# joesound212985/Deepfake-Detection-using-CLIP-Based-SigLIP-2-Vision-Transformers

Hardware: AMD Instinct MI355X
Metric: images/sec (train fwd+bwd) SigLIP-2-so400m@384 bf16 (higher is better)
Workload: dtype bf16; 1 GPU; so400m-patch14-384 encoder+pool-head train fwd+bwd, 384x384, per-GPU batch 128, seeded random weights; global_batch=128, parallelism=dp1

## Files before the change

### deepfake-detection-using-clip-based-siglip-2-vision-transformers_amd/csrc/attention.hip

```cpp
#include <stdlib.h>

#include "common.hip.h"
#include "kernels.h"

namespace sgl {

hipError_t attn_f32_fwd(const float*, const float*, const float*, float*, float*, int, int, int, int, int, int, hipStream_t);
hipError_t attn_f32_bwd(const float*, const float*, const float*, const float*, const float*, const float*, float*,
                        float*, int, int, int, int, int, int, hipStream_t);
hipError_t attn_ref_fwd(const float*, const float*, const float*, float*, float*, int, int, int, int, int, int, hipStream_t);
hipError_t attn_ref_bwd(const float*, const float*, const float*, const float*, const float*, const float*, float*,
                        float*, int, int, int, int, int, int, hipStream_t);

template <int DP>
struct AttnCfg {
  static constexpr int KS = DP / 16;
  static constexpr int DT = (DP + 31) / 32;
  static constexpr int CPR = DP / 8;
  static constexpr int RSTR = DP * 2 + 16;
  static constexpr int TSTR = 192;
  static constexpr int DSTR = 208;
};

__device__ __forceinline__ u32x4 a_ldg(__amdgpu_buffer_rsrc_t r, uint32_t off) {
// ... 336 lines not shown
      dP = MFMA32(da[ks], vfr[ks], dP);
    }
    if constexpr (C::KS == 5) {
      __builtin_amdgcn_sched_group_barrier(0x100, 4, 0);
#pragma unroll
      for (int i = 0; i < 6; ++i) {
        __builtin_amdgcn_sched_group_barrier(0x008, 1, 0);
        __builtin_amdgcn_sched_group_barrier(0x100, 1, 0);
      }
      __builtin_amdgcn_sched_group_barrier(0x008, 4, 0);
    }
    __builtin_amdgcn_sched_barrier(0);
    constexpr int NF = 2 * 2 * C::DT;
    lo_x8<T> fr[NF];
    auto frag = [&](int i) {
      const int which = i & 1, kk = (i >> 1) & 1, dt = i >> 2;
      return lds_trfrag<T>(which ? qimg : dimg, C::DSTR, kk, dt * 32, lane);
    };
    constexpr int PRE = NF < 2 ? NF : 2;
#pragma unroll
    for (int i = 0; i < PRE; ++i) fr[i] = frag(i);
    __builtin_amdgcn_sched_barrier(0);
#pragma unroll
    for (int g4 = 0; g4 < 4; ++g4) {
      const f32x4 A0 = *reinterpret_cast<const f32x4*>(ld + 2 * (8 * g4 + 4 * hh));
      const f32x4 A1 = *reinterpret_cast<const f32x4*>(ld + 2 * (8 * g4 + 4 * hh) + 4);
      const float L4[4] = {A0[0], A0[2], A1[0], A1[2]};
      const float D4[4] = {A0[1], A0[3], A1[1], A1[3]};
#pragma unroll
      for (int r3 = 0; r3 < 4; ++r3) {
        const int r = 4 * g4 + r3;
        const float p = fast_exp2(fmaf(S[r], c, L4[r3]));
        S[r] = p;
        dP[r] = p * fmaf(dP[r], scale, D4[r3]);
      }
    }
    lo_x8<T> pb[2], dsb[2];
    pb[0] = pack8<T>(S, 0);
    pb[1] = pack8<T>(S, 8);
    dsb[0] = pack8<T>(dP, 0);
    dsb[1] = pack8<T>(dP, 8);
    __builtin_amdgcn_sched_barrier(0);
#pragma unroll
    for (int i = 0; i < NF; ++i) {
      if (i + PRE < NF) fr[i + PRE] = frag(i + PRE);
      const int which = i & 1, kk = (i >> 1) & 1, dt = i >> 2;
      if (which) dk[dt] = MFMA32(fr[i], dsb[kk], dk[dt]);
      else dv[dt] = MFMA32(fr[i], pb[kk], dv[dt]);
      if (i % 3 == 1) issue1(i / 3, st_next);
      __builtin_amdgcn_sched_barrier(0);
    }
#pragma unroll
    for (int j = (NF + 1) / 3; j < 4; ++j) issue1(j, st_next);
  }
  asm volatile("s_waitcnt vmcnt(0)" ::: "memory");
  const int key = key0 + li;
  if (key < N) {
    T* krow = dqkv + ((size_t)b * N + key) * (3 * (size_t)D) + D + hd * dh;
    T* vrow = krow + D;
#pragma unroll
    for (int dt = 0; dt < C::DT; ++dt)
#pragma unroll
      for (int g4 = 0; g4 < 4; ++g4) {
        const int d = dt * 32 + 8 * g4 + 4 * hh;
        if (d < dh) {
          lo_x4<T> a, g;
#pragma unroll
          for (int r = 0; r < 4; ++r) {
            a[r] = (T)dk[dt][4 * g4 + r];
            g[r] = (T)dv[dt][4 * g4 + r];
          }
          *reinterpret_cast<lo_x4<T>*>(krow + d) = a;
          *reinterpret_cast<lo_x4<T>*>(vrow + d) = g;
        }
      }
  }
}

template <typename T, int DP, bool TOK>
__global__ __launch_bounds__(256, 2) void attn_bwd_q_kernel(const T* __restrict__ Q, const T* __restrict__ K,
                                                            const T* __restrict__ V, const T* __restrict__ O,
                                                            const T* __restrict__ dO, const float* __restrict__ lse,
                                                            float* __restrict__ aux, T* __restrict__ dqkv,
                                                            int B, int H, int N, int dh, int ld, float c, float scale) {
  using C = AttnCfg<DP>;
  constexpr int KT = 32;
  constexpr int SCK = C::DSTR / 16, SCV = C::RSTR / 16;
  constexpr int NIK = (KT * SCK + 63) / 64, NIV = (KT * SCV + 63) / 64;
  constexpr int KIMG = NIK * 1024, VIMG = NIV * 1024, STAGE = KIMG + VIMG;
  constexpr int NSLOT = NIK + NIV;
  static_assert(NSLOT <= 16, "at most four DMA slots per wave");
  constexpr float LOG2E = 1.4426950408889634f;
  extern __shared__ __attribute__((aligned(16))) char smem[];
  const int t = threadIdx.x, lane = t & 63;
  const int w = __builtin_amdgcn_readfirstlane(t >> 6);
  int bh, xb;
  if (!head_block((N + 127) / 128, B * H, bh, xb)) return;
  const int b = bh / H, hd = bh - b * H;
  const int D = H * dh;
  const int q0 = xb * 128 + w * 32;
  HeadSrc src = head_src(TOK ? ld : 0, b, hd, H, N, dh, DP);
  if constexpr (!TOK) {
    src.rowbytes = (uint32_t)DP * 2u;
    src.nc = (uint32_t)DP / 8u;
  }
  const __amdgpu_buffer_rsrc_t rq = make_rsrc(Q + src.base, src.bytes);
  const T* dOb = dO + (size_t)b * N * D + hd * dh;
  const __amdgpu_buffer_rsrc_t rdo = make_rsrc(dOb, (uint32_t)(((size_t)(N - 1) * D + dh) * 2));
  const u32x4 dk_ = att_desc(K + src.base, src.bytes);
  const u32x4 dv_ = att_desc(V + src.base, src.bytes);
  const uint32_t lds0 = (uint32_t)(size_t)((SGL_LDS char*)smem);

  const int li = lane & 31, hh = lane >> 5;
  const int q = q0 + li;
  lo_x8<T> qf[C::KS], dof[C::KS];
#pragma unroll
  for (int ks = 0; ks < C::KS; ++ks) {
    const int col = 16 * ks + 8 * hh;
    qf[ks] = as_x8<T>(a_ldg(rq, (q < N && (uint32_t)(col >> 3) < src.nc) ? (uint32_t)q * src.rowbytes + (uint32_t)col * 2u
                                                                           : SGL_OOB));
    dof[ks] = as_x8<T>(a_ldg(rdo, (q < N && col < dh) ? (uint32_t)(((size_t)q * D + col) * 2) : SGL_OOB));
  }
  float dl = 0.f;
  {
    const __amdgpu_buffer_rsrc_t ro = make_rsrc(O + (size_t)b * N * D + hd * dh, (uint32_t)(((size_t)(N - 1) * D + dh) * 2));
#pragma unroll
    for (int ks = 0; ks < C::KS; ++ks) {
      const int col = 16 * ks + 8 * hh;
      const lo_x8<T> of = as_x8<T>(a_ldg(ro, (q < N && col < dh) ? (uint32_t)(((size_t)q * D + col) * 2) : SGL_OOB));
#pragma unroll
      for (int j = 0; j < 8; ++j) dl = fmaf((float)of[j], (float)dof[ks][j], dl);
    }
    dl += __shfl_xor(dl, 32, 64);
  }
  const float Lq = (q < N) ? -lse[(size_t)bh * N + q] * LOG2E : -INFINITY;
  const float Dq = (q < N) ? -dl * scale : 0.f;
  if (q < N && hh == 0) *reinterpret_cast<float2*>(aux + 2 * ((size_t)bh * N + q)) = make_float2(Lq, Dq);

  uint32_t voff[4];
  u32x4 dsc[4];
  uint32_t ldst[4];
#pragma unroll
  for (int j = 0; j < 4; ++j) {
    const int sl = w + 4 * j;
    if (sl < NIK) {
      voff[j] = att_chunk_off(sl * 64 + lane, KT, SCK, (int)src.nc, src.rowbytes);
      dsc[j] = dk_;
      ldst[j] = (uint32_t)sl * 1024u;
    } else {
      voff[j] = att_chunk_off((sl - NIK) * 64 + lane, KT, SCV, (int)src.nc, src.rowbytes);
      dsc[j] = dv_;
      ldst[j] = (uint32_t)(KIMG + (sl - NIK) * 1024);
    }
  }
  auto issue1 = [&](int j, int stage) {
    if (w + 4 * j < NSLOT) att_dma16(dsc[j], lds0 + (uint32_t)(stage * STAGE) + ldst[j], voff[j]);
    voff[j] += (uint32_t)KT * src.rowbytes;
  };

  f32x16 dq[C::DT];
#pragma unroll
  for (int dt = 0; dt < C::DT; ++dt)
#pragma unroll
    for (int r = 0; r < 16; ++r) dq[dt][r] = 0.f;

  const int ntiles = (N + KT - 1) / KT;
#pragma unroll
// ... 5 lines not shown
#pragma unroll
  for (int j = 0; j < 4; ++j) issue1(j, 1);
  int st = 0;
  for (int kt = 0; kt < ntiles; ++kt) {
    const int nw = (NSLOT - w + 3) / 4;
    if (nw >= 4) SGL_ATT_WAIT_BARRIER(4);
    else if (nw == 3) SGL_ATT_WAIT_BARRIER(3);
    else if (nw == 2) SGL_ATT_WAIT_BARRIER(2);
    else SGL_ATT_WAIT_BARRIER(1);
    const int st_next = (st == 0) ? 2 : st - 1;
    const char* kimg = smem + st * STAGE;
    const char* vimg = kimg + KIMG;
    st = (st == 2) ? 0 : st + 1;
    f32x16 S, dP;
#pragma unroll
    for (int r = 0; r < 16; ++r) { S[r] = 0.f; dP[r] = 0.f; }
    lo_x8<T> ka[C::KS], va[C::KS];
#pragma unroll
    for (int ks = 0; ks < C::KS; ++ks) {
      ka[ks] = lds_row8<T>(kimg + li * C::DSTR + (16 * ks + 8 * hh) * 2);
      va[ks] = lds_row8<T>(vimg + li * C::RSTR + (16 * ks + 8 * hh) * 2);
    }
#pragma unroll
    for (int ks = 0; ks < C::KS; ++ks) {
      S = MFMA32(ka[ks], qf[ks], S);
      dP = MFMA32(va[ks], dof[ks], dP);
    }
    if constexpr (C::KS == 5) {
      __builtin_amdgcn_sched_group_barrier(0x100, 6, 0);
#pragma unroll
      for (int i = 0; i < 4; ++i) {
        __builtin_amdgcn_sched_group_barrier(0x008, 1, 0);
        __builtin_amdgcn_sched_group_barrier(0x100, 1, 0);
      }
      __builtin_amdgcn_sched_group_barrier(0x008, 6, 0);
    }
    __builtin_amdgcn_sched_barrier(0);
    lo_x8<T> kt_frag[C::DT][2];
#pragma unroll
    for (int dt = 0; dt < C::DT; ++dt)
#pragma unroll
      for (int kk = 0; kk < 2; ++kk) kt_frag[dt][kk] = lds_trfrag<T>(kimg, C::DSTR, kk, dt * 32, lane);
    __builtin_amdgcn_sched_barrier(0);
#pragma unroll
    for (int r = 0; r < 16; ++r) {
      const float p = fast_exp2(fmaf(S[r], c, Lq));
      dP[r] = p * fmaf(dP[r], scale, Dq);
    }
    if (kt == ntiles - 1) {
#pragma unroll
      for (int r = 0; r < 16; ++r) {
        const int key = kt * KT + (r & 3) + 8 * (r >> 2) + 4 * hh;
        if (key >= N) dP[r] = 0.f;
      }
    }
    lo_x8<T> dsb[2];
    dsb[0] = pack8<T>(dP, 0);
    dsb[1] = pack8<T>(dP, 8);
#pragma unroll
    for (int i = 0; i < 2 * C::DT; ++i) {
      dq[i >> 1] = MFMA32(kt_frag[i >> 1][i & 1], dsb[i & 1], dq[i >> 1]);
      if (i < 4) issue1(i, st_next);
      __builtin_amdgcn_sched_barrier(0);
    }
#pragma unroll
    for (int j = 2 * C::DT; j < 4; ++j) issue1(j, st_next);
  }
  asm volatile("s_waitcnt vmcnt(0)" ::: "memory");
  if (q < N) {
    T* qrow = dqkv + ((size_t)b * N + q) * (3 * (size_t)D) + hd * dh;
#pragma unroll
    for (int dt = 0; dt < C::DT; ++dt)
#pragma unroll
      for (int g4 = 0; g4 < 4; ++g4) {
        const int d = dt * 32 + 8 * g4 + 4 * hh;
        if (d < dh) {
          lo_x4<T> a;
#pragma unroll
          for (int r = 0; r < 4; ++r) a[r] = (T)dq[dt][4 * g4 + r];
          *reinterpret_cast<lo_x4<T>*>(qrow + d) = a;
        }
      }
  }
}

template <typename T, int DP>
static hipError_t fwd_launch(const T* q, const T* k, const T* v, T* out, float* lse, int B, int H, int N,
                             int dh, int ld, hipStream_t s) {
  using C = AttnCfg<DP>;
  constexpr int smem = 2 * (64 * C::RSTR + 64 * C::TSTR);
  const float scale = 1.0f / sqrtf((float)dh);
  if (ld > 0)
    hipLaunchKernelGGL((attn_fwd_kernel<T, DP, true>), head_grid((N + 127) / 128, B * H), dim3(256), smem, s, q, k, v, out, lse,
                       B, H, N, dh, ld, scale * 1.4426950408889634f, scale);
  else
    hipLaunchKernelGGL((attn_fwd_kernel<T, DP, false>), head_grid((N + 127) / 128, B * H), dim3(256), smem, s, q, k, v, out,
                       lse, B, H, N, dh, 0, scale * 1.4426950408889634f, scale);
  return hipGetLastError();
}

template <typename T, int DP>
static hipError_t bwd_launch(const T* q, const T* k, const T* v, const T* out, const T* dout,
                             const float* lse, T* dqkv, float* delta, int B, int H, int N, int dh, int ld,
                             hipStream_t s) {
  using C = AttnCfg<DP>;
  const float scale = 1.0f / sqrtf((float)dh);
  const float c = scale * 1.4426950408889634f;
  constexpr int smem_kv = 3 * (2 * ((32 * (C::DSTR / 16) + 63) / 64) * 1024 + 32 * 8);
  constexpr int smem_q = 3 * (((32 * (C::DSTR / 16) + 63) / 64) + ((32 * (C::RSTR / 16) + 63) / 64)) * 1024;
  const dim3 grid = head_grid((N + 127) / 128, B * H), block(256);
  if (ld > 0)
    hipLaunchKernelGGL((attn_bwd_q_kernel<T, DP, true>), grid, block, smem_q, s, q, k, v, out, dout, lse, delta, dqkv, B, H, N,
                       dh, ld, c, scale);
  else
    hipLaunchKernelGGL((attn_bwd_q_kernel<T, DP, false>), grid, block, smem_q, s, q, k, v, out, dout, lse, delta, dqkv, B, H, N,
                       dh, 0, c, scale);
  hipError_t e = hipGetLastError();
  if (e != hipSuccess) return e;
  if (ld > 0)
    hipLaunchKernelGGL((attn_bwd_kv_kernel<T, DP, true>), grid, block, smem_kv, s, q, k, v, dout, delta, dqkv, B, H, N, dh, ld, c,
                       scale);
  else
    hipLaunchKernelGGL((attn_bwd_kv_kernel<T, DP, false>), grid, block, smem_kv, s, q, k, v, dout, delta, dqkv, B, H, N, dh, 0,
                       c, scale);
  return hipGetLastError();
}

static bool attn_shape_ok(int N, int dh, int DP, int H, int ld) {
  if (dh % 8 || DP != ((dh + 15) / 16) * 16) return false;
  if (DP != 16 && DP != 32 && DP != 48 && DP != 64 && DP != 80 && DP != 96) return false;
  if (ld < 0 || (ld > 0 && (ld % 8 || ld < H * dh))) return false;
  if ((size_t)N * (ld > 0 ? ld : DP) * 2 >= (1ull << 31)) return false;
  if ((size_t)N * H * dh * 2 >= (1ull << 31)) return false;
  return true;
}

hipError_t attn_fwd(const void* q, const void* k, const void* v, int dtype, void* out, float* lse, int B, int H, int N,
                    int dh, int DP, int ld, hipStream_t s) {
  if (B * H == 0 || N == 0) return hipSuccess;
  if (dtype == DT_F32)
    return attn_ref_fwd((const float*)q, (const float*)k, (const float*)v, (float*)out, lse, B, H, N, dh, DP, ld, s);
  if (dtype == DT_F32_MFMA)
    return attn_f32_fwd((const float*)q, (const float*)k, (const float*)v, (float*)out, lse, B, H, N, dh, DP, ld, s);
  if (!attn_shape_ok(N, dh, DP, H, ld)) return hipErrorInvalidValue;
  if ((((uintptr_t)q) | ((uintptr_t)k) | ((uintptr_t)v)) & 15) return hipErrorInvalidValue;
#define SGL_F(T, DPV) \
  case DPV: return fwd_launch<T, DPV>((const T*)q, (const T*)k, (const T*)v, (T*)out, lse, B, H, N, dh, ld, s);
  if (dtype == DT_F16) {
    switch (DP) {
      SGL_F(f16, 16) SGL_F(f16, 32) SGL_F(f16, 48) SGL_F(f16, 64) SGL_F(f16, 80) SGL_F(f16, 96)
    }
    return hipErrorInvalidValue;
  }
  switch (DP) {
    SGL_F(bf16, 16) SGL_F(bf16, 32) SGL_F(bf16, 48) SGL_F(bf16, 64) SGL_F(bf16, 80) SGL_F(bf16, 96)
  }
#undef SGL_F
  return hipErrorInvalidValue;
}

hipError_t attn_bwd(const void* q, const void* k, const void* v, const void* out, const void* dout, const float* lse,
                    int dtype, void* dqkv, float* delta, float* , int B, int H, int N, int dh, int DP,
                    int ld, hipStream_t s) {
  if (B * H == 0 || N == 0) return hipSuccess;
  if (dtype == DT_F32)
    return attn_ref_bwd((const float*)q, (const float*)k, (const float*)v, (const float*)out, (const float*)dout, lse,
                        (float*)dqkv, delta, B, H, N, dh, DP, ld, s);
  if (dtype == DT_F32_MFMA)
    return attn_f32_bwd((const float*)q, (const float*)k, (const float*)v, (const float*)out, (const float*)dout, lse,
                        (float*)dqkv, delta, B, H, N, dh, DP, ld, s);
  if (!attn_shape_ok(N, dh, DP, H, ld)) return hipErrorInvalidValue;
  if ((((uintptr_t)q) | ((uintptr_t)k) | ((uintptr_t)v)) & 15) return hipErrorInvalidValue;
#define SGL_B(T, DPV)                                                                                  \
  case DPV:                                                                                            \
    return bwd_launch<T, DPV>((const T*)q, (const T*)k, (const T*)v, (const T*)out, (const T*)dout, lse, \
                              (T*)dqkv, delta, B, H, N, dh, ld, s);
  if (dtype == DT_F16) {
    switch (DP) {
      SGL_B(f16, 16) SGL_B(f16, 32) SGL_B(f16, 48) SGL_B(f16, 64) SGL_B(f16, 80) SGL_B(f16, 96)
    }
    return hipErrorInvalidValue;
  }
  switch (DP) {
    SGL_B(bf16, 16) SGL_B(bf16, 32) SGL_B(bf16, 48) SGL_B(bf16, 64) SGL_B(bf16, 80) SGL_B(bf16, 96)
  }
#undef SGL_B
  return hipErrorInvalidValue;
}

}
```

### deepfake-detection-using-clip-based-siglip-2-vision-transformers_amd/csrc/elementwise.hip

```cpp
#include "common.hip.h"
#include "shadow_tile.hip.h"
#include "kernels.h"

namespace sgl {

template <typename T>
__global__ __launch_bounds__(256) void im2col_kernel(const float* __restrict__ pix, int channels_last,
                                                     T* __restrict__ out, int B, int H, int W, int P, int gh, int gw,
                                                     int Kp) {
  const size_t total = (size_t)B * gh * gw * Kp;
  const int K = 3 * P * P;
  for (size_t idx = (size_t)blockIdx.x * 256 + threadIdx.x; idx < total; idx += (size_t)gridDim.x * 256) {
    const int k = (int)(idx % Kp);
    const size_t m = idx / Kp;
    float v = 0.f;
    if (k < K) {
      const int gx = (int)(m % gw);
      const int gy = (int)((m / gw) % gh);
      const int b = (int)(m / ((size_t)gw * gh));
      const int c = k / (P * P);
      const int r = k - c * P * P;
      const int ky = r / P, kx = r - ky * P;
      const int yy = gy * P + ky, xx = gx * P + kx;
      const size_t src = channels_last ? (((size_t)b * H + yy) * W + xx) * 3 + c
// ... 215 lines not shown
}
void cast_job_add_vec(CastJob& job, const float* src, int n, float* dst, int np) {
  job.vsrc[job.nvec] = src; job.vdst[job.nvec] = dst; job.vn[job.nvec] = n; job.vnp[job.nvec] = np;
  ++job.nvec;
}
hipError_t cast_job_run(const CastJob& job, int dst_dtype, hipStream_t s) {
  if (job.ntiles == 0 && job.nvec == 0) return hipSuccess;
  const dim3 grid((unsigned)(job.ntiles + (job.nvec ? 1 : 0)));
  if (dst_dtype == DT_BF16)
    hipLaunchKernelGGL(cast_job_kernel<bf16>, grid, dim3(256), 0, s, job);
  else if (dst_dtype == DT_F16)
    hipLaunchKernelGGL(cast_job_kernel<f16>, grid, dim3(256), 0, s, job);
  else
    hipLaunchKernelGGL(cast_job_kernel<float>, grid, dim3(256), 0, s, job);
  return hipGetLastError();
}

int colsum_chunks(int M) {
  int c = (M + 511) / 512;
  return c < 1 ? 1 : (c > 256 ? 256 : c);
}

template <typename T>
__global__ __launch_bounds__(256) void colsum_kernel(const T* __restrict__ in, int ld, int M, int N, int rows_per,
                                                     float* __restrict__ partial) {
  __shared__ float red[8][257];
  const int cg = threadIdx.x & 31, rl = threadIdx.x >> 5;
  const int col0 = blockIdx.x * 256 + cg * 8;
  const int r_begin = blockIdx.y * rows_per;
  const int r_end = (r_begin + rows_per < M) ? r_begin + rows_per : M;
  float acc[8] = {0, 0, 0, 0, 0, 0, 0, 0};
  if (col0 < N) {
    for (int r = r_begin + rl; r < r_end; r += 8) {
      float v[8];
      Vec<T, 8>::ld(in + (size_t)r * ld + col0, v);
#pragma unroll
      for (int j = 0; j < 8; ++j) acc[j] += v[j];
    }
  }
#pragma unroll
  for (int j = 0; j < 8; ++j) red[rl][cg * 8 + j] = acc[j];
  __syncthreads();
  const int c = threadIdx.x;
  if (blockIdx.x * 256 + c < N) {
    float s = 0.f;
#pragma unroll
    for (int r = 0; r < 8; ++r) s += red[r][c];
    partial[(size_t)blockIdx.y * N + blockIdx.x * 256 + c] = s;
  }
}

hipError_t colsum(const void* in, int dtype, int ld, int M, int N, int n_out, float* partial, float* out,
                  int accumulate, hipStream_t s) {
  if (N % 8 || ld % 8) return hipErrorInvalidValue;
  if (N == 0) return hipSuccess;
  const int chunks = colsum_chunks(M);
  const int rows_per = (M + chunks - 1) / chunks;
  dim3 grid((N + 255) / 256, chunks), block(256);
  if (dtype == DT_BF16)
    hipLaunchKernelGGL(colsum_kernel<bf16>, grid, block, 0, s, (const bf16*)in, ld, M, N, rows_per, partial);
  else if (dtype == DT_F16)
    hipLaunchKernelGGL(colsum_kernel<f16>, grid, block, 0, s, (const f16*)in, ld, M, N, rows_per, partial);
  else
    hipLaunchKernelGGL(colsum_kernel<float>, grid, block, 0, s, (const float*)in, ld, M, N, rows_per, partial);
  hipError_t e = hipGetLastError();
  if (e != hipSuccess) return e;
  return reduce_partials(partial, chunks, N, out, n_out < N ? n_out : N, accumulate, s);
}

__global__ __launch_bounds__(256) void batch_sum_kernel(const float* __restrict__ in, int B, size_t n,
                                                        float* __restrict__ out, int accumulate) {
  const size_t j = (size_t)blockIdx.x * 256 + threadIdx.x;
  if (j >= n) return;
  float s = 0.f;
  for (int b = 0; b < B; ++b) s += in[(size_t)b * n + j];
  out[j] = accumulate ? out[j] + s : s;
}
hipError_t batch_sum(const float* in, int B, size_t n, float* out, int accumulate, hipStream_t s) {
  if (n == 0) return hipSuccess;
  hipLaunchKernelGGL(batch_sum_kernel, dim3((unsigned)((n + 255) / 256)), dim3(256), 0, s, in, B, n, out, accumulate);
  return hipGetLastError();
}

constexpr int VECMAT_CHUNKS = 16;
__global__ __launch_bounds__(256) void vecmat_f32_kernel(const float* __restrict__ v, const float* __restrict__ W, int rows,
                                                         int cols, float* __restrict__ partial) {
  __shared__ float part[4][64];
  const int jj = threadIdx.x & 63, rg = threadIdx.x >> 6;
  const int j = blockIdx.x * 64 + jj;
  const int per = (rows + VECMAT_CHUNKS - 1) / VECMAT_CHUNKS;
  const int r0 = blockIdx.y * per, r1 = (r0 + per < rows) ? r0 + per : rows;
  float s = 0.f;
  if (j < cols)
    for (int i = r0 + rg; i < r1; i += 4) s = fmaf(v[i], W[(size_t)i * cols + j], s);
  part[rg][jj] = s;
  __syncthreads();
  if (rg == 0 && j < cols) partial[(size_t)blockIdx.y * cols + j] = (part[0][jj] + part[1][jj]) + (part[2][jj] + part[3][jj]);
}
hipError_t vecmat_f32(const float* v, const float* W, int rows, int cols, float* scratch, float* out, int accumulate,
                      hipStream_t s) {
  if (rows <= 0 || cols <= 0) return hipSuccess;
  hipLaunchKernelGGL(vecmat_f32_kernel, dim3((unsigned)((cols + 63) / 64), VECMAT_CHUNKS), dim3(256), 0, s, v, W, rows, cols,
                     scratch);
  hipError_t e = hipGetLastError();
  if (e != hipSuccess) return e;
  return reduce_partials(scratch, VECMAT_CHUNKS, cols, out, cols, accumulate, s);
}

__device__ __forceinline__ void cubic_coeffs(float t, float* w) {
  const float A = -0.75f;
  float x = t + 1.0f;
  w[0] = ((A * x - 5.0f * A) * x + 8.0f * A) * x - 4.0f * A;
  x = t;
  w[1] = ((A + 2.0f) * x - (A + 3.0f)) * x * x + 1.0f;
  x = 1.0f - t;
  w[2] = ((A + 2.0f) * x - (A + 3.0f)) * x * x + 1.0f;
  x = 2.0f - t;
  w[3] = ((A * x - 5.0f * A) * x + 8.0f * A) * x - 4.0f * A;
}
__device__ __forceinline__ void cubic_taps(int o, int n_in, int n_out, int* idx, float* w) {
  const float scale = (float)n_in / (float)n_out;
  const float src = scale * ((float)o + 0.5f) - 0.5f;
  const float fl = floorf(src);
  cubic_coeffs(src - fl, w);
  const int i0 = (int)fl;
#pragma unroll
  for (int k = 0; k < 4; ++k) {
    int i = i0 - 1 + k;
    idx[k] = i < 0 ? 0 : (i > n_in - 1 ? n_in - 1 : i);
  }
}

__global__ __launch_bounds__(256) void pos_resize_kernel(const float* __restrict__ table, int g0,
                                                         float* __restrict__ out, int gh, int gw, int D) {
  const size_t total = (size_t)gh * gw * D;
  const size_t idx = (size_t)blockIdx.x * 256 + threadIdx.x;
  if (idx >= total) return;
  const int d = (int)(idx % D);
  const int o = (int)(idx / D);
  const int oy = o / gw, ox = o - oy * gw;
  int iy[4], ix[4];
  float wy[4], wx[4];
  cubic_taps(oy, g0, gh, iy, wy);
  cubic_taps(ox, g0, gw, ix, wx);
  float acc = 0.f;
#pragma unroll
  for (int a = 0; a < 4; ++a) {
    float rowv = 0.f;
#pragma unroll
    for (int b = 0; b < 4; ++b) rowv += wx[b] * table[((size_t)iy[a] * g0 + ix[b]) * D + d];
    acc += wy[a] * rowv;
  }
  out[idx] = acc;
}
hipError_t pos_resize(const float* table, int g0, float* out, int gh, int gw, int D, hipStream_t s) {
  const size_t total = (size_t)gh * gw * D;
  if (total == 0) return hipSuccess;
  hipLaunchKernelGGL(pos_resize_kernel, dim3((unsigned)((total + 255) / 256)), dim3(256), 0, s, table, g0, out, gh, gw,
                     D);
  return hipGetLastError();
}

__device__ __forceinline__ void tap_range(int i, int g0, int gout, int& lo, int& hi) {
  const float inv = (float)gout / (float)g0;
  lo = (int)floorf(((float)i - 3.0f + 0.5f) * inv - 0.5f) - 1;
  hi = (int)ceilf(((float)i + 3.0f + 0.5f) * inv - 0.5f) + 1;
  if (i == 0) lo = 0;
  if (i == g0 - 1) hi = gout - 1;
  if (lo < 0) lo = 0;
  if (hi > gout - 1) hi = gout - 1;
}
__global__ __launch_bounds__(256) void pos_resize_bwd_kernel(const float* __restrict__ dout, int gh, int gw,
                                                             float* __restrict__ dtable, int g0, int D) {
  const size_t total = (size_t)g0 * g0 * D;
  const size_t idx = (size_t)blockIdx.x * 256 + threadIdx.x;
  if (idx >= total) return;
  const int d = (int)(idx % D);
  const int e = (int)(idx / D);
  const int ty = e / g0, tx = e - ty * g0;
  int ylo, yhi, xlo, xhi;
  tap_range(ty, g0, gh, ylo, yhi);
  tap_range(tx, g0, gw, xlo, xhi);
  float acc = 0.f;
  for (int oy = ylo; oy <= yhi; ++oy) {
    int iy[4];
    float wy[4];
    cubic_taps(oy, g0, gh, iy, wy);
// ... 299 lines not shown
```

### deepfake-detection-using-clip-based-siglip-2-vision-transformers_amd/csrc/encoder.hip

```cpp
#include <hip/hip_runtime.h>
#include <string.h>

#include <algorithm>
#include <new>
#include <vector>

#include "kernels.h"
#include "siglip_hip.h"

using namespace sgl;

namespace {

inline size_t align256(size_t x) { return (x + 255) & ~(size_t)255; }
inline char* at(void* base, size_t off) { return reinterpret_cast<char*>(base) + off; }
inline const char* at(const void* base, size_t off) { return reinterpret_cast<const char*>(base) + off; }
inline bool mfma16(int dt) { return dt == DT_BF16 || dt == DT_F16; }
inline int round_up(int x, int m) { return (x + m - 1) / m * m; }

struct Bump {
  size_t off = 0;
  size_t take(size_t bytes) {
    const size_t o = off;
    off += align256(bytes);
    return o;
  }
};

struct ShadowLayer {
  size_t wqkv, wqkv_t, wo, wo_t, w1, w1_t, w2, w2_t, bqkv, b1;
  size_t wqkv_s, wo_s, w1_s, w2_s;
};

}

struct sgl_ctx {
  sgl_config cfg;
  int D, I, Ip, L, H, dh, DP, P, K0, Kp, g0, dt;
  size_t es;
  int split = 0;
  int mx = 0;
  int Dp = 0;
  int recompute = 0;
  int last_hip = 0;
  size_t sh_wpatch = 0;
  std::vector<ShadowLayer> sh_layers;
  size_t sh_hwkv = 0, sh_hwkv_t = 0, sh_hwo = 0, sh_hwo_t = 0, sh_hw1 = 0, sh_hw1_t = 0, sh_hw2 = 0, sh_hw2_t = 0,
         sh_hb1 = 0;
  size_t sh_total = 0;
};

namespace {

constexpr int kMaxLayers = 128;

constexpr size_t kSplitWsBytes = (size_t)256 * 256 * 256 * 4;
static_assert(tn_plan_is(93312, 1152, 1152, kSplitWsBytes, 384, 12), "out_proj dW in the encoder's workspace");
static_assert(tn_plan_is(93312, 3456, 1152, kSplitWsBytes, 384, 4), "QKV dW in the encoder's workspace");

inline size_t head_bytes(const sgl_ctx* c, int B, int N) { return (size_t)B * c->H * N * c->DP * c->es; }

struct Layout {
  int B = 0, gh = 0, gw = 0, N = 0, M = 0;
  bool train = false;
  size_t a_im2col = 0, a_pos = 0;
  size_t a_layer0 = 0, a_layer_stride = 0;
  size_t r_stats1 = 0, r_h1 = 0, r_qkv = 0, r_attn = 0, r_lse = 0, r_xmid = 0, r_stats2 = 0, r_h2 = 0, r_u = 0, r_a = 0,
         r_attq = 0;
  size_t a_pstats = 0, a_lastlp = 0, a_kvh = 0, a_qp = 0, a_probs = 0, a_ao = 0, a_h0 = 0, a_hstats = 0, a_hl = 0, a_hu = 0,
         a_ha = 0;
  size_t a_spa = 0, a_spb = 0, w_spa = 0, w_spb = 0;
  size_t act_total = 0;
  size_t w_dx = 0, w_g = 0, w_du = 0, w_dh = 0, w_dqkv = 0, w_delta = 0, w_splitws = 0, w_lnpart = 0, w_cspart = 0,
         w_dlast = 0, w_gsum = 0, w_csum = 0;
  size_t w_hg = 0, w_hdu = 0, w_hdh = 0, w_hdao = 0, w_hdqpart = 0, w_hdqp = 0, w_hdh0 = 0;
  size_t ws_bwd_total = 0;
  size_t saved_total = 0, ws_total = 0, ws_act_off = 0;
  bool rc = false;
  size_t w_blk = 0;

  Layout() = default;
  Layout(const sgl_ctx* c, int B_, int Himg, int Wimg, bool train_) {
    B = B_;
    train = train_;
    rc = train && c->recompute;
    gh = Himg / c->P;
    gw = Wimg / c->P;
    N = gh * gw;
    M = B * N;
    const size_t es = c->es, D = c->D, Ip = c->Ip, Mz = (size_t)M;
    Bump a;
    a_im2col = a.take(Mz * c->Kp * es);
    a_pos = a.take((size_t)N * D * 4);
    Bump r;
    const size_t Dp = c->Dp;
    const bool mx = c->mx;
    r_stats1 = r.take(Mz * 2 * 4);
    r_h1 = r.take(mx ? Mz * Dp + Mz * Dp / 32 : Mz * D * es);
    r_qkv = r.take(3 * head_bytes(c, B, N));
    r_attn = r.take(Mz * D * es);
    r_lse = r.take((size_t)B * c->H * N * 4);
    r_xmid = r.take(Mz * D * 4);
    r_stats2 = r.take(Mz * 2 * 4);
    r_h2 = r.take(mx ? Mz * Dp + Mz * Dp / 32 : Mz * D * es);
    r_u = r.take(mx ? 0 : Mz * Ip * es);
    r_a = r.take(mx ? Mz * Ip + Mz * Ip / 32 : Mz * Ip * es);
    r_attq = r.take(mx ? Mz * Dp + Mz * Dp / 32 : 0);
    a_layer_stride = (train && !rc) ? r.off : 0;
    a_layer0 = a.take(rc ? 0 : train ? r.off * (size_t)c->L : r.off);
    a_pstats = a.take(Mz * 2 * 4);
    a_lastlp = a.take(Mz * D * es);
    a_kvh = a.take(2 * head_bytes(c, B, N));
    a_qp = a.take(D * 4);
    a_probs = a.take((size_t)B * c->H * N * 4);
    a_ao = a.take((size_t)B * D * es);
    a_h0 = a.take((size_t)B * D * 4);
    a_hstats = a.take((size_t)B * 2 * 4);
    a_hl = a.take((size_t)B * D * es);
    a_hu = a.take((size_t)B * Ip * es);
    a_ha = a.take((size_t)B * Ip * es);
    const size_t widest = std::max(Ip, 3 * D), Kp = (size_t)c->Kp;
    const size_t Wd = (size_t)round_up((int)std::max(widest, Kp), 8);
    const size_t sp_act = 3 * std::max(Mz, (size_t)B) * Wd * 2;
    const size_t sp_wgt = 3 * Wd * (size_t)round_up((int)std::max(D, Kp), 8) * 2;
    const size_t sp_bytes = std::max(sp_act, sp_wgt);
    if (c->split && !rc) {
      a_spa = a.take(sp_bytes);
      a_spb = a.take(sp_bytes);
    }
    act_total = a.off;

    Bump w;
    if (train) {
      w_dx = w.take(Mz * D * 4);
      w_g = w.take(Mz * D * es);
      w_du = w.take(Mz * Ip * es);
      w_dh = w.take(Mz * D * es);
      w_dqkv = w.take(Mz * 3 * D * es);
      w_delta = w.take((size_t)B * c->H * N * 8);
      w_splitws = w.take(kSplitWsBytes);
      w_lnpart = w.take((size_t)layernorm_bwd_blocks(M) * 3 * D * 4);
      w_gsum = w.take(D * 4);
      w_csum = w.take((size_t)((M + 127) / 128) * widest * 4);
      w_cspart = w.take((size_t)std::max(colsum_chunks(M), 16) * widest * 4);
      w_dlast = w.take(Mz * D * 4);
      w_hg = w.take((size_t)B * D * es);
      w_hdu = w.take((size_t)B * Ip * es);
      w_hdh = w.take((size_t)B * D * es);
      w_hdao = w.take((size_t)B * D * 4);
      w_hdqpart = w.take((size_t)B * D * 4);
      w_hdqp = w.take(D * 4);
      w_hdh0 = w.take((size_t)B * D * 4);
      if (c->split) {
        w_spa = w.take(sp_bytes);
        w_spb = w.take(sp_bytes);
      }
      if (rc) w_blk = w.take(r.off);
    }
    ws_bwd_total = w.off;
    if (train) {
      saved_total = act_total;
      ws_act_off = 0;
      ws_total = ws_bwd_total;
    } else {
      saved_total = 0;
      ws_act_off = ws_bwd_total;
      ws_total = ws_bwd_total + act_total;
    }
    if (ws_total == 0) ws_total = 256;
  }
  size_t layer_base(int l) const { return a_layer0 + a_layer_stride * (size_t)l; }
};

#define CK(expr)                        \
  do {                                  \
    hipError_t e_ = (expr);             \
    if (e_ != hipSuccess) {             \
      ctx->last_hip = (int)e_;          \
      return SGL_ERR_HIP;               \
    }                                   \
  } while (0)

#define RET(expr)                 \
  do {                            \
    int r_ = (expr);              \
    if (r_ != SGL_OK) return r_;  \
  } while (0)

EpiParams epi_store(void* out, int ldo) {
  EpiParams p;
  p.out = out;
  p.ldo = ldo;
  return p;
}
EpiParams epi_f32(float* out, int ldo, const float* bias = nullptr) {
  EpiParams p;
  p.out = out;
  p.ldo = ldo;
  p.bias = bias;
  return p;
}
EpiParams epi_f32_acc(float* out, int ldo, int accumulate) {
  EpiParams p;
  p.out = out;
  p.ldo = ldo;
  p.accumulate = accumulate;
  return p;
}
EpiParams epi_res_f32(float* out, const float* bias, const float* res, int ld) {
  EpiParams p;
  p.out = out;
  p.ldo = ld;
  p.bias = bias;
  p.res = res;
  p.ldr = ld;
  return p;
}
EpiParams epi_pos_f32(float* out, int ldo, const float* bias, const float* pos, int pos_rows) {
  EpiParams p;
  p.out = out;
  p.ldo = ldo;
  p.bias = bias;
  p.pos = pos;
  p.pos_rows = pos_rows;
  return p;
}
// ... 26 lines not shown
    p.colsum_ld = ld;
  }
  return p;
}

int tn_splits(int N1, int N2, int rows) {
  const int tiles = ((N1 + 127) / 128) * ((N2 + 127) / 128);
  return std::min({(512 + tiles - 1) / tiles, std::max(rows / 512, 1), 16});
}

struct Call {
  sgl_ctx* ctx = nullptr;
  Layout lay;
  hipStream_t s = nullptr;
  const void* shadow = nullptr;
  char* act = nullptr;
  void* ws = nullptr;
  void* sp_a = nullptr;
  void* sp_b = nullptr;

  char* wsp(size_t off) const { return at(ws, off); }
  float* wsf(size_t off) const { return reinterpret_cast<float*>(at(ws, off)); }
  float* actf(size_t off) const { return reinterpret_cast<float*>(act + off); }
  const char* sh(size_t off) const { return at(shadow, off); }
  const float* shf(size_t off) const { return reinterpret_cast<const float*>(at(shadow, off)); }
  size_t head_bytes() const { return ::head_bytes(ctx, lay.B, lay.N); }
  char* block(int l) const { return lay.rc ? wsp(lay.w_blk) : act + lay.layer_base(l); }

  EpiParams epi_qkv(void* out, const float* bias) const {
    EpiParams p;
    p.out = out;
    p.bias = bias;
    p.tokens = lay.N;
    p.heads = ctx->H;
    p.head_dim = ctx->dh;
    p.head_dim_pad = ctx->DP;
    p.batch = lay.B;
    return p;
  }

  hipError_t gemm_nt(const void* A, int lda, const void* B, int ldb, int M, int N, int K, int epi, int out_dt,
                     const EpiParams& p) const {
    if (ctx->dt == DT_BF16) return gemm_nt_bf16(A, lda, B, ldb, M, N, K, epi, out_dt, p, s);
    if (ctx->dt == DT_F16) return gemm_nt_f16(A, lda, B, ldb, M, N, K, epi, out_dt, p, s);
    if (ctx->split && M > 0 && N > 0) {
      const int Ks = round_up(K, 8);
      hipError_t e = split3_rows((const float*)A, M, K, lda, sp_a, Ks, 0, s);
      if (e != hipSuccess) return e;
      e = split3_rows((const float*)B, N, K, ldb, sp_b, Ks, 1, s);
      if (e != hipSuccess) return e;
      return gemm_nt_bf16(sp_a, 3 * Ks, sp_b, 3 * Ks, M, N, 3 * Ks, epi, out_dt, p, s);
    }
    return gemm_f32_generic((const float*)A, lda, 1, (const float*)B, ldb, 1, M, N, K, epi, out_dt, p, s);
  }

  hipError_t gemm_tn(const void* A, int lda, const void* B, int ldb, int Mred, int N1, int N2, float* out, int ldo,
                     int accumulate, bool split_slabs) const {
    const EpiParams p = epi_f32_acc(out, ldo, accumulate);
    float* slabs = split_slabs ? wsf(lay.w_splitws) : nullptr;
    const size_t slab_bytes = split_slabs ? kSplitWsBytes : 0;
    if (ctx->dt == DT_F16)
      return gemm_tn_f16(A, lda, B, ldb, Mred, N1, N2, tn_splits(N1, N2, Mred), p, s, slabs, slab_bytes);
    if (ctx->dt == DT_BF16)
      return gemm_tn_bf16(A, lda, B, ldb, Mred, N1, N2, tn_splits(N1, N2, Mred), p, s, slabs, slab_bytes);
    if (ctx->split && Mred > 0 && N1 > 0 && N2 > 0) {
      const int l1 = round_up(N1, 8), l2 = round_up(N2, 8);
      hipError_t e = split3_stack((const float*)A, Mred, N1, lda, sp_a, l1, 0, s);
      if (e != hipSuccess) return e;
      e = split3_stack((const float*)B, Mred, N2, ldb, sp_b, l2, 1, s);
      if (e != hipSuccess) return e;
      return gemm_tn_bf16(sp_a, l1, sp_b, l2, 3 * Mred, N1, N2, tn_splits(N1, N2, 3 * Mred), p, s, slabs, slab_bytes);
    }
    return gemm_f32_generic((const float*)A, 1, lda, (const float*)B, 1, ldb, N1, N2, Mred, EPI_F32, DT_F32, p, s);
  }

  int bias_grad(const void* in, int ld, int M, int N, int n_out, float* out, int accumulate) const {
    if (!out) return SGL_OK;
    CK(colsum(in, ctx->dt, ld, M, N, n_out, wsf(lay.w_cspart), out, accumulate, s));
    return SGL_OK;
  }

  int ln_backward(const void* dy, int dy_dt, const float* x, const float* stats, int rows, const float* gamma,
                  const float* dres, float* dx, void* dx_lp, float* dgamma, float* dbeta, int accumulate,
                  float* colsum_out = nullptr) const {
    const int D = ctx->D;
    const bool want = dgamma || dbeta || colsum_out;
    const int nblk = layernorm_bwd_blocks(rows);
    float* part = wsf(lay.w_lnpart);
    CK(layernorm_bwd(dy, dy_dt, D, x, stats, stats + rows, gamma, dres, dx, dx_lp, ctx->dt, want ? part : nullptr, nblk,
                     rows, D, s));
    CK(reduce_partials3(part, nblk, 3 * D, dgamma, dbeta, colsum_out, D, accumulate, accumulate, 0, s));
    return SGL_OK;
  }
};

int mx_block(const Call& c, const sgl_layer_weights& lw, const ShadowLayer& sl, char* lb, const float* x, float* xo) {
  sgl_ctx* ctx = c.ctx;
  const Layout& lay = c.lay;
  hipStream_t s = c.s;
  const int D = ctx->D, Ip = ctx->Ip, Dp = ctx->Dp, M = lay.M;
  const float eps = ctx->cfg.layer_norm_eps;
  const size_t Mz = (size_t)M;
  char* h1 = lb + lay.r_h1;
  char* q = lb + lay.r_qkv;
  char* aq = lb + lay.r_attq;
  float* xmid = reinterpret_cast<float*>(lb + lay.r_xmid);
  char* h2 = lb + lay.r_h2;
  char* ua = lb + lay.r_a;
  CK(layernorm_fwd_mx(x, lw.ln1_w, lw.ln1_b, h1, h1 + Mz * Dp, M, D, Dp, eps, s));
  CK(gemm_nt_mx(h1, h1 + Mz * Dp, c.sh(sl.wqkv), c.sh(sl.wqkv_s), M, 3 * D, Dp, EPI_QKV, c.epi_qkv(q, c.shf(sl.bqkv)),
                nullptr, s));
  CK(attn_fwd(q, q + c.head_bytes(), q + 2 * c.head_bytes(), DT_BF16, lb + lay.r_attn,
              reinterpret_cast<float*>(lb + lay.r_lse), lay.B, ctx->H, lay.N, ctx->dh, ctx->DP, 0, s));
  CK(quantize_mx(lb + lay.r_attn, DT_BF16, D, M, D, Dp, aq, aq + Mz * Dp, s));
  CK(gemm_nt_mx(aq, aq + Mz * Dp, c.sh(sl.wo), c.sh(sl.wo_s), M, D, Dp, EPI_RES_F32, epi_res_f32(xmid, lw.o_b, x, D),
                nullptr, s));
  CK(layernorm_fwd_mx(xmid, lw.ln2_w, lw.ln2_b, h2, h2 + Mz * Dp, M, D, Dp, eps, s));
  CK(gemm_nt_mx(h2, h2 + Mz * Dp, c.sh(sl.w1), c.sh(sl.w1_s), M, Ip, Dp, EPI_BIAS_GELU,
                epi_bias_gelu_mx(ua, Ip, c.shf(sl.b1)), ua + Mz * Ip, s));
  CK(gemm_nt_mx(ua, ua + Mz * Ip, c.sh(sl.w2), c.sh(sl.w2_s), M, D, Ip, EPI_RES_F32, epi_res_f32(xo, lw.fc2_b, xmid, D),
                nullptr, s));
  return SGL_OK;
}

int block_to_fc1(const Call& c, const sgl_layer_weights& lw, const ShadowLayer& sl, char* lb, const float* x, bool want_u) {
  sgl_ctx* ctx = c.ctx;
  const Layout& lay = c.lay;
  hipStream_t s = c.s;
  const int D = ctx->D, Ip = ctx->Ip, M = lay.M, dt = ctx->dt;
  const float eps = ctx->cfg.layer_norm_eps;
  float* st1 = reinterpret_cast<float*>(lb + lay.r_stats1);
  float* st2 = reinterpret_cast<float*>(lb + lay.r_stats2);
  char* q = lb + lay.r_qkv;
  float* xmid = reinterpret_cast<float*>(lb + lay.r_xmid);
  CK(layernorm_fwd(x, lw.ln1_w, lw.ln1_b, lb + lay.r_h1, dt, D, st1, st1 + M, M, D, eps, s));
  CK(c.gemm_nt(lb + lay.r_h1, D, c.sh(sl.wqkv), D, M, 3 * D, D, EPI_QKV, dt, c.epi_qkv(q, c.shf(sl.bqkv))));
  CK(attn_fwd(q, q + c.head_bytes(), q + 2 * c.head_bytes(), ctx->split ? DT_F32_MFMA : dt, lb + lay.r_attn,
              reinterpret_cast<float*>(lb + lay.r_lse), lay.B, ctx->H, lay.N, ctx->dh, ctx->DP, 0, s));
  CK(c.gemm_nt(lb + lay.r_attn, D, c.sh(sl.wo), D, M, D, D, EPI_RES_F32, DT_F32, epi_res_f32(xmid, lw.o_b, x, D)));
  CK(layernorm_fwd(xmid, lw.ln2_w, lw.ln2_b, lb + lay.r_h2, dt, D, st2, st2 + M, M, D, eps, s));
  CK(c.gemm_nt(lb + lay.r_h2, D, c.sh(sl.w1), D, M, Ip, D, EPI_BIAS_GELU, dt,
               epi_bias_gelu(want_u ? lb + lay.r_u : nullptr, lb + lay.r_a, Ip, c.shf(sl.b1), mfma16(dt))));
  return SGL_OK;
}

int embed_forward(const Call& c, const sgl_weights* w, const float* pixels, int channels_last, int H, int W, float* out) {
  sgl_ctx* ctx = c.ctx;
  const Layout& lay = c.lay;
  hipStream_t s = c.s;
  const int D = ctx->D, Kp = ctx->Kp, M = lay.M;
  char* cols = c.act + lay.a_im2col;
  if (channels_last == 2) {
    CK(hipMemcpyAsync(cols, pixels, (size_t)M * Kp * ctx->es, hipMemcpyDeviceToDevice, s));
  } else {
    CK(im2col(pixels, channels_last, cols, ctx->dt, lay.B, H, W, ctx->P, Kp, s));
  }
  const float* pos = w->pos;
  if (!(lay.gh == ctx->g0 && lay.gw == ctx->g0)) {
    float* pr = c.actf(lay.a_pos);
    CK(pos_resize(w->pos, ctx->g0, pr, lay.gh, lay.gw, D, s));
    pos = pr;
  }
  CK(c.gemm_nt(cols, Kp, c.sh(ctx->sh_wpatch), Kp, M, D, Kp, EPI_POS_F32, DT_F32,
               epi_pos_f32(out, D, w->patch_b, pos, lay.N)));
  return SGL_OK;
}

int head_forward(const Call& c, const sgl_weights* w, const float* last_hidden, float* pooled) {
  sgl_ctx* ctx = c.ctx;
  const Layout& lay = c.lay;
  hipStream_t s = c.s;
  const int D = ctx->D, Ip = ctx->Ip, M = lay.M, B = lay.B, dt = ctx->dt;
  char* act = c.act;
// ... 387 lines not shown
  float* pst = c.actf(lay.a_pstats);
  CK(layernorm_fwd(hs_slots[ctx->L], w->post_ln_w, w->post_ln_b, last_hidden, DT_F32, ctx->D, pst, pst + lay.M, lay.M,
                   ctx->D, ctx->cfg.layer_norm_eps, c.s));
  if (ctx->cfg.use_head && pooled) RET(head_forward(c, w, last_hidden, pooled));
  return SGL_OK;
}

namespace {

int head_backward(const Call& c, const sgl_weights* w, const sgl_grads* g, const float* d_pooled,
                  const float* d_last_hidden, float* dlast) {
  sgl_ctx* ctx = c.ctx;
  const Layout& lay = c.lay;
  hipStream_t s = c.s;
  const int D = ctx->D, I = ctx->I, Ip = ctx->Ip, M = lay.M, B = lay.B, dt = ctx->dt;
  const int acc = g->accumulate;
  const char* act = c.act;
  const char* kv = act + lay.a_kvh;
  const float* qp = c.actf(lay.a_qp);
  void* hg = c.wsp(lay.w_hg);
  void* hdu = c.wsp(lay.w_hdu);
  void* hdh = c.wsp(lay.w_hdh);
  float* hdao = c.wsf(lay.w_hdao);
  CK(cast_f32(d_pooled, hg, dt, (size_t)B * D, s));
  CK(c.gemm_nt(hg, D, c.sh(ctx->sh_hw2_t), D, B, Ip, D, EPI_GELU_BWD, dt, epi_gelu_bwd(hdu, act + lay.a_hu, Ip, 0)));
  if (g->head_fc2_w) CK(c.gemm_tn(hg, D, act + lay.a_ha, Ip, B, D, I, g->head_fc2_w, I, acc, false));
  RET(c.bias_grad(hg, D, B, D, D, g->head_fc2_b, acc));
  CK(c.gemm_nt(hdu, Ip, c.sh(ctx->sh_hw1_t), Ip, B, D, Ip, EPI_STORE, dt, epi_store(hdh, D)));
  if (g->head_fc1_w) CK(c.gemm_tn(hdu, Ip, act + lay.a_hl, D, B, I, D, g->head_fc1_w, D, acc, false));
  RET(c.bias_grad(hdu, Ip, B, Ip, I, g->head_fc1_b, acc));
  RET(c.ln_backward(hdh, dt, c.actf(lay.a_h0), c.actf(lay.a_hstats), B, w->head_ln_w, d_pooled, c.wsf(lay.w_hdh0), hg,
                    g->head_ln_w, g->head_ln_b, acc));
  CK(c.gemm_nt(hg, D, c.sh(ctx->sh_hwo_t), D, B, D, D, EPI_F32, DT_F32, epi_f32(hdao, D)));
  if (g->out_proj_w) CK(c.gemm_tn(hg, D, act + lay.a_ao, D, B, D, D, g->out_proj_w, D, acc, false));
  RET(c.bias_grad(hg, D, B, D, D, g->out_proj_b, acc));
  void* dkv = c.wsp(lay.w_dqkv);
  float* dqpart = c.wsf(lay.w_hdqpart);
  float* dqp = c.wsf(lay.w_hdqp);
  CK(pool_attn_bwd(qp, kv, kv + c.head_bytes(), dt, c.actf(lay.a_probs), hdao, dkv, dqpart, B, ctx->H, lay.N, ctx->dh,
                   ctx->DP, s));
  if (g->probe || g->in_proj_w || g->in_proj_b) {
    CK(batch_sum(dqpart, B, (size_t)D, dqp, 0, s));
    if (g->in_proj_w)
      CK(gemm_f32_generic(dqp, 1, 1, w->probe, 1, 1, D, D, 1, EPI_F32, DT_F32, epi_f32_acc(g->in_proj_w, D, acc), s));
    if (g->in_proj_b) CK(batch_sum(dqp, 1, (size_t)D, g->in_proj_b, acc, s));
    if (g->probe)
      CK(gemm_f32_generic(dqp, D, 1, w->in_proj_w, 1, D, 1, D, D, EPI_F32, DT_F32, epi_f32_acc(g->probe, D, acc), s));
  }
  if (d_last_hidden) CK(copy_f32(d_last_hidden, dlast, (size_t)M * D, s));
  CK(c.gemm_nt(dkv, 2 * D, c.sh(ctx->sh_hwkv_t), 2 * D, M, D, 2 * D, EPI_F32, DT_F32,
               epi_f32_acc(dlast, D, d_last_hidden ? 1 : 0)));
  if (g->in_proj_w)
    CK(c.gemm_tn(dkv, 2 * D, act + lay.a_lastlp, D, M, 2 * D, D, g->in_proj_w + (size_t)D * D, D, acc, true));
  if (g->in_proj_b) RET(c.bias_grad(dkv, 2 * D, M, 2 * D, 2 * D, g->in_proj_b + D, acc));
  return SGL_OK;
}

int zero_dead_grads(const Call& c, const sgl_grads* g, bool no_head_grad, bool no_post_ln_grad) {
  sgl_ctx* ctx = c.ctx;
  hipStream_t s = c.s;
  if (g->accumulate) return SGL_OK;
  auto zero = [&](float* p, size_t n) { return p ? hipMemsetAsync(p, 0, n * 4, s) : hipSuccess; };
  const size_t Dz = (size_t)ctx->D, Iz = (size_t)ctx->I;
  if (ctx->cfg.use_head && no_head_grad) {
    CK(zero(g->probe, Dz));
    CK(zero(g->in_proj_w, 3 * Dz * Dz));
    CK(zero(g->in_proj_b, 3 * Dz));
    CK(zero(g->out_proj_w, Dz * Dz));
    CK(zero(g->out_proj_b, Dz));
    CK(zero(g->head_ln_w, Dz));
    CK(zero(g->head_ln_b, Dz));
    CK(zero(g->head_fc1_w, Iz * Dz));
    CK(zero(g->head_fc1_b, Iz));
    CK(zero(g->head_fc2_w, Dz * Iz));
    CK(zero(g->head_fc2_b, Dz));
  }
  if (no_post_ln_grad) {
    CK(zero(g->post_ln_w, Dz));
    CK(zero(g->post_ln_b, Dz));
  }
  return SGL_OK;
}

int mlp_backward(const Call& c, const sgl_layer_weights& lw, const sgl_layer_grads& lg, const ShadowLayer& sl,
                 const char* lb, int acc) {
  sgl_ctx* ctx = c.ctx;
  const Layout& lay = c.lay;
  hipStream_t s = c.s;
  const int D = ctx->D, I = ctx->I, Ip = ctx->Ip, M = lay.M, dt = ctx->dt;
  float* dx = c.wsf(lay.w_dx);
  void* gbuf = c.wsp(lay.w_g);
  void* du = c.wsp(lay.w_du);
  void* dhb = c.wsp(lay.w_dh);
  float* gsum = c.wsf(lay.w_gsum);
  float* csum = c.wsf(lay.w_csum);
  const bool fuse_cs = mfma16(dt) && lg.fc1_b;
  if (fuse_cs) CK(hipMemsetAsync(csum, 0, (size_t)((M + 127) / 128) * Ip * 4, s));
  CK(c.gemm_nt(gbuf, D, c.sh(sl.w2_t), D, M, Ip, D, EPI_GELU_BWD, dt,
               epi_gelu_bwd(du, lb + lay.r_u, Ip, mfma16(dt), fuse_cs ? csum : nullptr)));
  if (lg.fc2_w) CK(c.gemm_tn(gbuf, D, lb + lay.r_a, Ip, M, D, I, lg.fc2_w, I, acc, true));
  if (lg.fc2_b) CK(batch_sum(gsum, 1, (size_t)D, lg.fc2_b, acc, s));
  CK(c.gemm_nt(du, Ip, c.sh(sl.w1_t), Ip, M, D, Ip, EPI_STORE, dt, epi_store(dhb, D)));
  if (lg.fc1_w) CK(c.gemm_tn(du, Ip, lb + lay.r_h2, D, M, I, D, lg.fc1_w, D, acc, true));
  if (fuse_cs)
    CK(reduce_partials(csum, (M + 127) / 128, Ip, lg.fc1_b, I, acc, s));
  else
    RET(c.bias_grad(du, Ip, M, Ip, I, lg.fc1_b, acc));
  RET(c.ln_backward(dhb, dt, reinterpret_cast<const float*>(lb + lay.r_xmid),
                    reinterpret_cast<const float*>(lb + lay.r_stats2), M, lw.ln2_w, dx, dx, gbuf, lg.ln2_w, lg.ln2_b, acc,
                    (lg.o_b || lg.v_b) ? gsum : nullptr));
  if (lg.o_b) CK(batch_sum(gsum, 1, (size_t)D, lg.o_b, acc, s));
  return SGL_OK;
}

int attn_backward(const Call& c, const sgl_layer_weights& lw, const sgl_layer_grads& lg, const ShadowLayer& sl,
                  const char* lb, int acc) {
  sgl_ctx* ctx = c.ctx;
  const Layout& lay = c.lay;
  hipStream_t s = c.s;
  const int D = ctx->D, M = lay.M, dt = ctx->dt;
  void* gbuf = c.wsp(lay.w_g);
  void* dattn = c.wsp(lay.w_dh);
  void* dqkv = c.wsp(lay.w_dqkv);
  float* gsum = c.wsf(lay.w_gsum);
  const char* q = lb + lay.r_qkv;
  CK(c.gemm_nt(gbuf, D, c.sh(sl.wo_t), D, M, D, D, EPI_STORE, dt, epi_store(dattn, D)));
  if (lg.o_w) CK(c.gemm_tn(gbuf, D, lb + lay.r_attn, D, M, D, D, lg.o_w, D, acc, true));
  CK(attn_bwd(q, q + c.head_bytes(), q + 2 * c.head_bytes(), lb + lay.r_attn, dattn,
              reinterpret_cast<const float*>(lb + lay.r_lse), ctx->split ? DT_F32_MFMA : dt, dqkv, c.wsf(lay.w_delta),
              nullptr, lay.B, ctx->H, lay.N, ctx->dh, ctx->DP, 0, s));
  float* gw[3] = {lg.q_w, lg.k_w, lg.v_w};
  float* gb[3] = {lg.q_b, lg.k_b, lg.v_b};
  const bool w_adj = gw[0] && gw[1] == gw[0] + (size_t)D * D && gw[2] == gw[1] + (size_t)D * D;
  if (w_adj) CK(c.gemm_tn(dqkv, 3 * D, lb + lay.r_h1, D, M, 3 * D, D, gw[0], D, acc, true));
  for (int j = 0; j < 3; ++j) {
    const char* aj = reinterpret_cast<const char*>(dqkv) + (size_t)j * D * ctx->es;
    if (!w_adj && gw[j]) CK(c.gemm_tn(aj, 3 * D, lb + lay.r_h1, D, M, D, D, gw[j], D, acc, true));
  }
  if (gb[0]) RET(c.bias_grad(dqkv, 3 * D, M, D, D, gb[0], acc));
  if (gb[1] && !acc) CK(hipMemsetAsync(gb[1], 0, (size_t)D * 4, s));
  if (gb[2]) CK(vecmat_f32(gsum, lw.o_w, D, D, c.wsf(lay.w_cspart), gb[2], acc, s));
  return SGL_OK;
}

int ln1_backward(const Call& c, const sgl_layer_weights& lw, const sgl_layer_grads& lg, const ShadowLayer& sl,
                 const char* lb, const float* x_in, int acc) {
  sgl_ctx* ctx = c.ctx;
  const Layout& lay = c.lay;
  const int D = ctx->D, M = lay.M, dt = ctx->dt;
  float* dx = c.wsf(lay.w_dx);
  void* dh1 = c.wsp(lay.w_dh);
  CK(c.gemm_nt(c.wsp(lay.w_dqkv), 3 * D, c.sh(sl.wqkv_t), 3 * D, M, D, 3 * D, EPI_STORE, dt, epi_store(dh1, D)));
  RET(c.ln_backward(dh1, dt, x_in, reinterpret_cast<const float*>(lb + lay.r_stats1), M, lw.ln1_w, dx, dx,
                    c.wsp(lay.w_g), lg.ln1_w, lg.ln1_b, acc, c.wsf(lay.w_gsum)));
  return SGL_OK;
}

}

int sgl_backward_begin(sgl_ctx* ctx, const sgl_weights* w, const void* shadow, const sgl_grads* g, int B, int H, int W,
                       const float* hidden_states, const float* d_last_hidden, const float* d_pooled,
                       const float* d_tap_last, const void* saved, size_t saved_bytes, void* ws, size_t ws_bytes,
                       sgl_stream stream) {
  if (!ctx || !hidden_states) return SGL_ERR_NULL;
  if (!train_shape_ok(ctx, B, H, W)) return SGL_ERR_BAD_SHAPE;
  const size_t stride = (size_t)B * (H / ctx->P) * (W / ctx->P) * ctx->D;
  return sgl_backward_begin_p(ctx, w, shadow, g, B, H, W, hidden_states + (size_t)ctx->L * stride, d_last_hidden, d_pooled,
                              d_tap_last, saved, saved_bytes, ws, ws_bytes, stream);
}

int sgl_backward_begin_p(sgl_ctx* ctx, const sgl_weights* w, const void* shadow, const sgl_grads* g, int B, int H, int W,
                         const float* hs_last, const float* d_last_hidden, const float* d_pooled,
                         const float* d_tap_last, const void* saved, size_t saved_bytes, void* ws, size_t ws_bytes,
                         sgl_stream stream) {
  if (!ctx || !w || !shadow || !g || !hs_last) return SGL_ERR_NULL;
  Call c;
  RET(begin_call(c, BACKWARD, ctx, shadow, B, H, W, saved, saved_bytes, ws, ws_bytes, stream));
  const Layout& lay = c.lay;
  hipStream_t s = c.s;
  const int D = ctx->D, M = lay.M;
  float* dx = c.wsf(lay.w_dx);
  void* gbuf = c.wsp(lay.w_g);
  float* gsum = c.wsf(lay.w_gsum);
  const float* dlast = d_last_hidden;
  if (ctx->cfg.use_head && d_pooled) {
    float* dlast_buf = c.wsf(lay.w_dlast);
    RET(head_backward(c, w, g, d_pooled, d_last_hidden, dlast_buf));
    dlast = dlast_buf;
  }
  RET(zero_dead_grads(c, g, !d_pooled, !dlast));
  if (dlast) {
    RET(c.ln_backward(dlast, DT_F32, hs_last, c.actf(lay.a_pstats), M, w->post_ln_w, d_tap_last, dx, gbuf, g->post_ln_w,
                      g->post_ln_b, g->accumulate, gsum));
  } else if (d_tap_last) {
    CK(copy_f32(d_tap_last, dx, (size_t)M * D, s));
    CK(cast_f32(d_tap_last, gbuf, ctx->dt, (size_t)M * D, s));
    CK(colsum(gbuf, ctx->dt, D, M, D, D, c.wsf(lay.w_cspart), gsum, 0, s));
  } else {
    CK(hipMemsetAsync(dx, 0, (size_t)M * D * 4, s));
    CK(hipMemsetAsync(gbuf, 0, (size_t)M * D * ctx->es, s));
    CK(hipMemsetAsync(gsum, 0, (size_t)D * 4, s));
  }
  return SGL_OK;
}

int sgl_backward_layer(sgl_ctx* ctx, const sgl_weights* w, const void* shadow, const sgl_grads* g, int layer, int B,
                       int H, int W, const float* hidden_states, const float* d_tap, int need_dx, const void* saved,
                       size_t saved_bytes, void* ws, size_t ws_bytes, sgl_stream stream) {
  if (!ctx || !hidden_states) return SGL_ERR_NULL;
  if (layer < 0 || layer >= ctx->L || !train_shape_ok(ctx, B, H, W)) return SGL_ERR_BAD_SHAPE;
  const size_t stride = (size_t)B * (H / ctx->P) * (W / ctx->P) * ctx->D;
  return sgl_backward_layer_p(ctx, w, shadow, g, layer, B, H, W, hidden_states + (size_t)layer * stride, d_tap, need_dx,
                              saved, saved_bytes, ws, ws_bytes, stream);
}

int sgl_backward_layer_p(sgl_ctx* ctx, const sgl_weights* w, const void* shadow, const sgl_grads* g, int layer, int B,
                         int H, int W, const float* hs_in, const float* d_tap, int need_dx, const void* saved,
                         size_t saved_bytes, void* ws, size_t ws_bytes, sgl_stream stream) {
  if (!ctx || !w || !shadow || !g || !hs_in || !g->layers || !w->layers) return SGL_ERR_NULL;
  if (layer < 0 || layer >= ctx->L) return SGL_ERR_BAD_SHAPE;
  Call c;
  RET(begin_call(c, BACKWARD, ctx, shadow, B, H, W, saved, saved_bytes, ws, ws_bytes, stream));
  const int acc = g->accumulate;
  const sgl_layer_weights& lw = w->layers[layer];
// ... 130 lines not shown
  return SGL_OK;
}

int sgl_op_layernorm_fwd_mx(const float* x, const float* gamma, const float* beta, void* q, void* scales, int M, int D,
                            int Kp, float eps, sgl_stream stream) {
  if (!x || !gamma || !beta || !q || !scales) return SGL_ERR_NULL;
  CKV(layernorm_fwd_mx(x, gamma, beta, q, scales, M, D, Kp, eps, (hipStream_t)stream));
  return SGL_OK;
}

int sgl_op_gemm_nt_mx(const void* A, const void* As, const void* B, const void* Bs, int M, int N, int Kp, int epi,
                      void* out, int ldo, void* out_scales, const float* bias, const float* res, int ldr, int tokens,
                      int heads, int head_dim, int head_dim_pad, int batch, sgl_stream stream) {
  if (!A || !As || !B || !Bs || !out || !bias) return SGL_ERR_NULL;
  EpiParams p;
  p.out = out; p.ldo = ldo; p.bias = bias; p.res = res; p.ldr = ldr;
  p.tokens = tokens > 0 ? tokens : 1; p.heads = heads > 0 ? heads : 1; p.head_dim = head_dim > 0 ? head_dim : 8;
  p.head_dim_pad = head_dim_pad > 0 ? head_dim_pad : 8; p.batch = batch > 0 ? batch : 1;
  CKV(gemm_nt_mx(A, As, B, Bs, M, N, Kp, epi, p, out_scales, (hipStream_t)stream));
  return SGL_OK;
}

int sgl_op_layernorm_bwd(const void* dy, int dy_dtype, const float* x, const float* mean, const float* rstd,
                         const float* gamma, const float* dres, float* dx, void* dx_lp, int lp_dtype, float* dgamma,
                         float* dbeta, float* scratch, size_t scratch_bytes, int M, int D, sgl_stream stream) {
  const int nblk = layernorm_bwd_blocks(M);
  if (scratch_bytes < (size_t)nblk * 3 * D * 4) return SGL_ERR_WORKSPACE;
  hipStream_t s = (hipStream_t)stream;
  CKV(layernorm_bwd(dy, dy_dtype, D, x, mean, rstd, gamma, dres, dx, dx_lp, lp_dtype, scratch, nblk, M, D, s));
  if (dgamma) CKV(reduce_partials(scratch, nblk, 3 * D, dgamma, D, 0, s));
  if (dbeta) CKV(reduce_partials(scratch + D, nblk, 3 * D, dbeta, D, 0, s));
  return SGL_OK;
}

int sgl_op_gemm_nt(int dtype, const void* A, int lda, const void* B, int ldb, int M, int N, int K, int epi, void* out,
                   int ldo, void* out2, int ldo2, const float* bias, const float* res, int ldr, const void* aux,
                   int ldaux, const float* pos, int pos_rows, int tokens, int heads, int head_dim, int head_dim_pad,
                   int batch, sgl_stream stream) {
  EpiParams p;
  p.out = out; p.ldo = ldo; p.out2 = out2; p.ldo2 = ldo2; p.bias = bias; p.res = res; p.ldr = ldr;
  p.aux = aux; p.ldaux = ldaux; p.pos = pos; p.pos_rows = pos_rows > 0 ? pos_rows : 1;
  p.tokens = tokens > 0 ? tokens : 1; p.heads = heads > 0 ? heads : 1; p.head_dim = head_dim > 0 ? head_dim : 8;
  p.head_dim_pad = head_dim_pad > 0 ? head_dim_pad : 8; p.batch = batch > 0 ? batch : 1;
  const bool f32_out = (epi == EPI_RES_F32 || epi == EPI_POS_F32 || epi == EPI_F32);
  const int out_dt = f32_out ? DT_F32 : dtype;
  if (dtype == DT_BF16)
    CKV(gemm_nt_bf16(A, lda, B, ldb, M, N, K, epi, out_dt, p, (hipStream_t)stream));
  else if (dtype == DT_F16)
    CKV(gemm_nt_f16(A, lda, B, ldb, M, N, K, epi, out_dt, p, (hipStream_t)stream));
  else
    CKV(gemm_f32_generic((const float*)A, lda, 1, (const float*)B, ldb, 1, M, N, K, epi, out_dt, p,
                         (hipStream_t)stream));
  return SGL_OK;
}

int sgl_op_gemm_tn(int dtype, const void* A, int lda, const void* B, int ldb, int Mred, int N1, int N2, int splits,
                   float* out, int ldo, int accumulate, sgl_stream stream) {
  return sgl_op_gemm_tn_ws(dtype, A, lda, B, ldb, Mred, N1, N2, splits, out, ldo, accumulate, nullptr, 0, stream);
}

int sgl_op_gemm_tn_ws(int dtype, const void* A, int lda, const void* B, int ldb, int Mred, int N1, int N2, int splits,
                      float* out, int ldo, int accumulate, float* scratch, size_t scratch_bytes, sgl_stream stream) {
  EpiParams p;
  p.out = out; p.ldo = ldo; p.accumulate = accumulate;
  if (dtype == DT_BF16)
    CKV(gemm_tn_bf16(A, lda, B, ldb, Mred, N1, N2, splits, p, (hipStream_t)stream, scratch, scratch_bytes));
  else if (dtype == DT_F16)
    CKV(gemm_tn_f16(A, lda, B, ldb, Mred, N1, N2, splits, p, (hipStream_t)stream, scratch, scratch_bytes));
  else
    CKV(gemm_f32_generic((const float*)A, 1, lda, (const float*)B, 1, ldb, N1, N2, Mred, EPI_F32, DT_F32, p,
                         (hipStream_t)stream));
  return SGL_OK;
}

int sgl_op_attn_fwd(int dtype, const void* q, const void* k, const void* v, void* out, float* lse, int B, int H, int N,
                    int head_dim, int head_dim_pad, int ld_qkv, sgl_stream stream) {
  CKV(attn_fwd(q, k, v, dtype, out, lse, B, H, N, head_dim, head_dim_pad, ld_qkv, (hipStream_t)stream));
  return SGL_OK;
}

int sgl_op_attn_bwd(int dtype, const void* q, const void* k, const void* v, const void* out, const void* dout,
                    const float* lse, void* dqkv, float* delta_scratch, int B, int H, int N, int head_dim,
                    int head_dim_pad, int ld_qkv, sgl_stream stream) {
  CKV(attn_bwd(q, k, v, out, dout, lse, dtype, dqkv, delta_scratch, nullptr, B, H, N, head_dim, head_dim_pad, ld_qkv,
               (hipStream_t)stream));
  return SGL_OK;
}

int sgl_op_colsum(int dtype, const void* in, int ld, int M, int N, float* out, int accumulate, float* scratch,
                  size_t scratch_bytes, sgl_stream stream) {
  if (scratch_bytes < (size_t)colsum_chunks(M) * N * 4) return SGL_ERR_WORKSPACE;
  CKV(colsum(in, dtype, ld, M, N, N, scratch, out, accumulate, (hipStream_t)stream));
  return SGL_OK;
}

int sgl_op_im2col(const float* pixels, int channels_last, void* out, int out_dtype, int B, int H, int W, int P, int Kp,
                  sgl_stream stream) {
  CKV(im2col(pixels, channels_last, out, out_dtype, B, H, W, P, Kp, (hipStream_t)stream));
  return SGL_OK;
}

int sgl_op_col2im(const float* d_cols, int B, int H, int W, int P, int Kp, float* d_pixels, int channels_last,
                  sgl_stream stream) {
  if (!d_cols || !d_pixels) return SGL_ERR_NULL;
  CKV(col2im(d_cols, B, H, W, P, Kp, d_pixels, channels_last, (hipStream_t)stream));
  return SGL_OK;
}

int sgl_op_pos_resize(const float* table, int native_grid, float* out, int gh, int gw, int D, sgl_stream stream) {
  CKV(pos_resize(table, native_grid, out, gh, gw, D, (hipStream_t)stream));
  return SGL_OK;
}

static bool lo_dtype_ok(int dt) { return dt == DT_F32 || dt == DT_BF16 || dt == DT_F16; }
static bool aligned16(const void* p) { return (((uintptr_t)p) & 15) == 0; }

int sgl_op_pool_attn_fwd(int dtype, const float* q, const void* K, const void* V, void* out, float* probs, int B, int H,
                         int N, int head_dim, int head_dim_pad, sgl_stream stream) {
  if (!q || !K || !V || !out || !probs) return SGL_ERR_NULL;
  if (B <= 0 || H <= 0 || N <= 0 || head_dim <= 0 || head_dim % 8 || head_dim_pad % 8 || head_dim > head_dim_pad)
    return SGL_ERR_BAD_SHAPE;
  if (!lo_dtype_ok(dtype) || !aligned16(K) || !aligned16(V)) return SGL_ERR_UNSUPPORTED;
  CKV(pool_attn_fwd(q, K, V, dtype, out, probs, B, H, N, head_dim, head_dim_pad, (hipStream_t)stream));
  return SGL_OK;
}

int sgl_op_pool_attn_bwd(int dtype, const float* q, const void* K, const void* V, const float* probs, const float* dout,
                         void* dkv, float* dq_partial, int B, int H, int N, int head_dim, int head_dim_pad,
                         sgl_stream stream) {
  if (!q || !K || !V || !probs || !dout || !dkv || !dq_partial) return SGL_ERR_NULL;
  if (B <= 0 || H <= 0 || N <= 0 || head_dim <= 0 || head_dim % 8 || head_dim_pad % 8 || head_dim > head_dim_pad)
    return SGL_ERR_BAD_SHAPE;
  if (!lo_dtype_ok(dtype) || !aligned16(K) || !aligned16(V) || !aligned16(dkv)) return SGL_ERR_UNSUPPORTED;
  CKV(pool_attn_bwd(q, K, V, dtype, probs, dout, dkv, dq_partial, B, H, N, head_dim, head_dim_pad, (hipStream_t)stream));
  return SGL_OK;
}

int sgl_op_pos_resize_bwd(const float* dout, int gh, int gw, float* dtable, int native_grid, int D, sgl_stream stream) {
  if (!dout || !dtable) return SGL_ERR_NULL;
  if (gh <= 0 || gw <= 0 || native_grid <= 0 || D <= 0) return SGL_ERR_BAD_SHAPE;
  CKV(pos_resize_bwd(dout, gh, gw, dtable, native_grid, D, (hipStream_t)stream));
  return SGL_OK;
}

int sgl_op_cast_pad(const float* src, int R, int C, int lds, void* dst, int dst_dtype, int Rp, int Cp, int ldd,
                    sgl_stream stream) {
  if (!src || !dst) return SGL_ERR_NULL;
  if (R < 0 || C < 0 || Rp < R || Cp < C || lds < C || ldd < Cp) return SGL_ERR_BAD_SHAPE;
  if (!lo_dtype_ok(dst_dtype)) return SGL_ERR_UNSUPPORTED;
  CKV(cast_pad(src, R, C, lds, dst, dst_dtype, Rp, Cp, ldd, (hipStream_t)stream));
  return SGL_OK;
}

int sgl_op_cast_job(const sgl_cast_mat* mats, int nmat, const sgl_cast_vec* vecs, int nvec, int dst_dtype,
                    sgl_stream stream) {
  if ((nmat > 0 && !mats) || (nvec > 0 && !vecs)) return SGL_ERR_NULL;
  if (nmat < 0 || nmat > 6 || nvec < 0 || nvec > 4) return SGL_ERR_BAD_SHAPE;
  for (int k = 0; k < nmat; ++k)
    if (!mats[k].src || (!mats[k].dst && !mats[k].dst_t)) return SGL_ERR_NULL;
  for (int k = 0; k < nvec; ++k)
    if (!vecs[k].src || !vecs[k].dst) return SGL_ERR_NULL;
  for (int k = 0; k < nmat; ++k) {
    const sgl_cast_mat& m = mats[k];
    if (m.R <= 0 || m.C <= 0 || m.Rp < m.R || m.Cp < m.C || m.lds < m.C || (m.dst && m.ldd < m.Cp) ||
        (m.dst_t && m.ldt < m.Rp))
      return SGL_ERR_BAD_SHAPE;
  }
  for (int k = 0; k < nvec; ++k)
    if (vecs[k].n < 0 || vecs[k].np < vecs[k].n) return SGL_ERR_BAD_SHAPE;
// ... 79 lines not shown
```

### deepfake-detection-using-clip-based-siglip-2-vision-transformers_amd/csrc/epilogue.hip.h

```cpp
#pragma once
#include <type_traits>

#include "common.hip.h"
#include "kernels.h"

namespace sgl {

template <int NV>
__device__ __forceinline__ void epi_res_f32(float* v, const float* bias, const float* r, float* dst) {
#pragma unroll
  for (int j = 0; j < NV; ++j) v[j] = r[j] + (v[j] + bias[j]);
  Vec<float, NV>::st_nt(dst, v);
}
template <typename TOut, int NV>
__device__ __forceinline__ void epi_bias_gelu(const EpiParams& p, float* v, const float* bias, TOut* dst_u, TOut* dst_act) {
  float a[NV];
  if (p.out && p.gelu_grad_form) {
#pragma unroll
    for (int j = 0; j < NV; ++j) gelu_tanh_both(v[j] + bias[j], a[j], v[j]);
  } else {
#pragma unroll
    for (int j = 0; j < NV; ++j) {
      v[j] += bias[j];
      a[j] = gelu_tanh(v[j]);
    }
  }
  if (p.out) Vec<TOut, NV>::st_nt(dst_u, v);
  Vec<TOut, NV>::st_nt(dst_act, a);
}
__device__ __forceinline__ void qkv_split_row(int row, int tokens, int& b, int& n) {
  b = (int)((float)row * __builtin_amdgcn_rcpf((float)tokens));
  n = row - b * tokens;
  if (n < 0) { b -= 1; n += tokens; }
  else if (n >= tokens) { b += 1; n -= tokens; }
}
template <typename TOut, int NV>
__device__ __forceinline__ void epi_qkv(float* v, const float* bias, TOut* dst, int pad_chunks) {
#pragma unroll
  for (int j = 0; j < NV; ++j) v[j] += bias[j];
  Vec<TOut, NV>::st_nt(dst, v);
  if (pad_chunks) {
    float z[NV];
#pragma unroll
    for (int j = 0; j < NV; ++j) z[j] = 0.f;
    for (int k = 1; k <= pad_chunks; ++k) Vec<TOut, NV>::st_nt(dst + k * NV, z);
  }
}
template <typename TOut, int NV>
__device__ __forceinline__ void epi_gelu_bwd(const EpiParams& p, float* v, const float* u, TOut* dst) {
  if (p.gelu_grad_form) {
#pragma unroll
    for (int j = 0; j < NV; ++j) v[j] *= u[j];
  } else {
#pragma unroll
    for (int j = 0; j < NV; ++j) v[j] *= gelu_tanh_grad(u[j]);
  }
  Vec<TOut, NV>::st_nt(dst, v);
}

__device__ __forceinline__ void lds_barrier() {
  asm volatile("s_waitcnt lgkmcnt(0)" ::: "memory");
  __builtin_amdgcn_s_barrier();
  asm volatile("" ::: "memory");
}

template <int NT, int BN, int NV>
__device__ __forceinline__ void epi_colsum_fold(float* ct, const float (&csum)[NV], int t, int m0, int n0, int N,
                                                const EpiParams& p) {
  constexpr int CPR = BN / NV, GROUPS = NT / CPR;
  static_assert(NT % CPR == 0 && BN <= NT, "one fixed column set per thread, one thread per column");
  if (!p.colsum) return;
  lds_barrier();
#pragma unroll
  for (int j = 0; j < NV; ++j) ct[(t / CPR) * BN + (t % CPR) * NV + j] = csum[j];
  lds_barrier();
  if (t < BN && n0 + t < N) {
    float s = 0.f;
#pragma unroll
    for (int gI = 0; gI < GROUPS; ++gI) s += ct[gI * BN + t];
    if (p.colsum_ld > 0)
      p.colsum[(size_t)(m0 >> 7) * p.colsum_ld + n0 + t] = s;
    else
      atomicAdd(p.colsum + n0 + t, s);
  }
}

template <int EPI, typename TOut, int NV>
__device__ __forceinline__ void epi_apply(const EpiParams& p, int row, int col, int N, float* v) {
  if constexpr (EPI == EPI_STORE) {
#pragma unroll
    for (int j = 0; j < NV; ++j) v[j] *= p.alpha;
    if (p.bias) {
      float b[NV];
      Vec<float, NV>::ld(p.bias + col, b);
#pragma unroll
      for (int j = 0; j < NV; ++j) v[j] += b[j];
    }
    Vec<TOut, NV>::st_nt(reinterpret_cast<TOut*>(p.out) + (size_t)row * p.ldo + col, v);
  } else if constexpr (EPI == EPI_BIAS_GELU) {
    float b[NV];
    Vec<float, NV>::ld(p.bias + col, b);
    epi_bias_gelu<TOut, NV>(p, v, b, reinterpret_cast<TOut*>(p.out) + (size_t)row * p.ldo + col,
                            reinterpret_cast<TOut*>(p.out2) + (size_t)row * p.ldo2 + col);
  } else if constexpr (EPI == EPI_RES_F32) {
    float b[NV], r[NV];
    Vec<float, NV>::ld(p.bias + col, b);
    Vec<float, NV>::ld(p.res + (size_t)row * p.ldr + col, r);
    epi_res_f32<NV>(v, b, r, reinterpret_cast<float*>(p.out) + (size_t)row * p.ldo + col);
  } else if constexpr (EPI == EPI_QKV) {
    const int dm = p.heads * p.head_dim;
    const int which = col / dm;
    const int hc = col - which * dm;
    const int h = hc / p.head_dim;
    const int d = hc - h * p.head_dim;
    int b, n;
    qkv_split_row(row, p.tokens, b, n);
    float bb[NV];
    Vec<float, NV>::ld(p.bias + col, bb);
    TOut* dst = reinterpret_cast<TOut*>(p.out) +
                ((((size_t)which * p.batch + b) * p.heads + h) * p.tokens + n) * p.head_dim_pad + d;
    epi_qkv<TOut, NV>(v, bb, dst, (d + NV == p.head_dim) ? (p.head_dim_pad - p.head_dim) / NV : 0);
  } else if constexpr (EPI == EPI_GELU_BWD) {
    float u[NV];
    Vec<TOut, NV>::ld(reinterpret_cast<const TOut*>(p.aux) + (size_t)row * p.ldaux + col, u);
    epi_gelu_bwd<TOut, NV>(p, v, u, reinterpret_cast<TOut*>(p.out) + (size_t)row * p.ldo + col);
  } else if constexpr (EPI == EPI_POS_F32) {
    float b[NV], e[NV];
    Vec<float, NV>::ld(p.bias + col, b);
    Vec<float, NV>::ld(p.pos + (size_t)(row % p.pos_rows) * N + col, e);
#pragma unroll
    for (int j = 0; j < NV; ++j) v[j] = (v[j] + b[j]) + e[j];
    Vec<float, NV>::st(reinterpret_cast<float*>(p.out) + (size_t)row * p.ldo + col, v);
  } else {
    float* dst = reinterpret_cast<float*>(p.out) + (size_t)row * p.ldo + col;
    const int nv = (col + NV <= N) ? NV : (N - col);
#pragma unroll
    for (int j = 0; j < NV; ++j) v[j] *= p.alpha;
    if (p.bias) {
      for (int j = 0; j < nv; ++j) v[j] += p.bias[col + j];
    }
    if (p.atomic) {
      for (int j = 0; j < nv; ++j) atomicAdd(dst + j, v[j]);
    } else if (nv == NV && (p.ldo % NV) == 0) {
      if (p.accumulate) {
        float o[NV];
        Vec<float, NV>::ld(dst, o);
#pragma unroll
        for (int j = 0; j < NV; ++j) v[j] += o[j];
      }
      Vec<float, NV>::st(dst, v);
    } else {
      for (int j = 0; j < nv; ++j) dst[j] = p.accumulate ? dst[j] + v[j] : v[j];
    }
  }
}

template <int EPI, typename TOut>
struct EpiTag {
  static constexpr int epi = EPI;
  using out = TOut;
};
template <typename TLo = bf16, typename Launch>
hipError_t dispatch_epilogue(int epi, int out_dtype, Launch&& launch) {
  const bool b16 = out_dtype == (std::is_same<TLo, f16>::value ? DT_F16 : DT_BF16);
  switch (epi) {
// ... 13 lines not shown
```

### deepfake-detection-using-clip-based-siglip-2-vision-transformers_amd/csrc/gemm_bf16.hip

```cpp
#include <stdlib.h>

#include "common.hip.h"
#include "epilogue.hip.h"
#include "kernels.h"

namespace sgl {

constexpr int G_BM = 128, G_BN = 128, G_BK = 64;
constexpr int G_STAGE = (G_BM + G_BN) * G_BK * 2;
constexpr int G_CT_LD = 132;
constexpr int G_LDS = (2 * G_STAGE > G_BM * G_CT_LD * 4) ? 2 * G_STAGE : G_BM * G_CT_LD * 4;

__device__ __forceinline__ u32x4 ldg128(__amdgpu_buffer_rsrc_t r, uint32_t voff) {
  return __builtin_amdgcn_raw_buffer_load_b128(r, voff, 0, 0);
}

template <int EPI, typename TOut>
__device__ __forceinline__ void store_tile(char* smem, f32x4 (&acc)[4][4], int wr, int wc, int lane, int t, int m0,
                                           int n0, int M, int N, const EpiParams& p) {
  float* ct = reinterpret_cast<float*>(smem);
  __syncthreads();
  const int g = lane >> 4, c16 = lane & 15;
#pragma unroll
  for (int i = 0; i < 4; ++i)
#pragma unroll
    for (int j = 0; j < 4; ++j)
#pragma unroll
      for (int r = 0; r < 4; ++r)
        ct[(wr * 64 + i * 16 + g * 4 + r) * G_CT_LD + wc * 64 + j * 16 + c16] = acc[i][j][r];
  __syncthreads();
  if constexpr (EPI == EPI_F32) {
    if (p.atomic) {
      float* outp = reinterpret_cast<float*>(p.out);
      const int w = t >> 6;
#pragma unroll 4
      for (int rr = 0; rr < 32; ++rr) {
        const int row = w + rr * 4;
        const int grow = m0 + row;
        if (grow >= M) continue;
#pragma unroll
        for (int h = 0; h < 2; ++h) {
          const int col = lane + 64 * h;
          if (n0 + col < N) atomicAdd(outp + (size_t)grow * p.ldo + n0 + col, ct[row * G_CT_LD + col] * p.alpha);
        }
      }
      return;
    }
  }
  constexpr int NV = (sizeof(TOut) == 4) ? 4 : 8;
  constexpr int CPR = G_BN / NV;
  float csum[NV];
#pragma unroll
  for (int j = 0; j < NV; ++j) csum[j] = 0.f;
#pragma unroll
  for (int q = 0; q < (G_BM * CPR) / 256; ++q) {
    const int c = t + q * 256;
    const int row = c / CPR, col = (c % CPR) * NV;
    const int grow = m0 + row, gcol = n0 + col;
    if (grow < M && gcol < N) {
      float v[NV];
      Vec<float, NV>::ld(ct + row * G_CT_LD + col, v);
      epi_apply<EPI, TOut, NV>(p, grow, gcol, N, v);
      if constexpr (EPI == EPI_GELU_BWD) {
#pragma unroll
        for (int j = 0; j < NV; ++j) csum[j] += v[j];
      }
    }
  }
  if constexpr (EPI == EPI_GELU_BWD) epi_colsum_fold<256, G_BN, NV>(ct, csum, t, m0, n0, N, p);
}

template <int EPI, typename TOut, typename TIn>
__global__ __launch_bounds__(256, 2) void gemm_nt_kernel(const TIn* __restrict__ A, int lda,
                                                         const TIn* __restrict__ B, int ldb, int M, int N, int K,
                                                         EpiParams p) {
  extern __shared__ __attribute__((aligned(16))) char smem[];
  const int t = threadIdx.x, lane = t & 63, wave = t >> 6;
  const int wr = wave >> 1, wc = wave & 1;
  const int tiles_n = (N + G_BN - 1) / G_BN;
  const int tile_m = blockIdx.x / tiles_n, tile_n = blockIdx.x - tile_m * tiles_n;
  const int m0 = tile_m * G_BM, n0 = tile_n * G_BN;
  const int rows_a = (M - m0 < G_BM) ? M - m0 : G_BM;
  const int rows_b = (N - n0 < G_BN) ? N - n0 : G_BN;
  const __amdgpu_buffer_rsrc_t ra = make_rsrc(A + (size_t)m0 * lda, (uint32_t)(((size_t)(rows_a - 1) * lda + K) * 2));
  const __amdgpu_buffer_rsrc_t rb = make_rsrc(B + (size_t)n0 * ldb, (uint32_t)(((size_t)(rows_b - 1) * ldb + K) * 2));

  const int srow = t >> 3, skc = t & 7;
  uint32_t a_off[4], b_off[4], l_off[4];
#pragma unroll
  for (int q = 0; q < 4; ++q) {
    const int row = srow + q * 32;
    a_off[q] = (row < rows_a) ? (uint32_t)(row * lda + skc * 8) * 2u : SGL_OOB;
    b_off[q] = (row < rows_b) ? (uint32_t)(row * ldb + skc * 8) * 2u : SGL_OOB;
    l_off[q] = (uint32_t)(row * 128 + ((skc ^ (row & 7)) << 4));
  }
  const int frow = lane & 15, fg = lane >> 4;
  uint32_t fa_row[4], fb_row[4];
#pragma unroll
  for (int i = 0; i < 4; ++i) {
    fa_row[i] = (uint32_t)((wr * 64 + i * 16 + frow) * 128);
    fb_row[i] = (uint32_t)(G_BM * 128 + (wc * 64 + i * 16 + frow) * 128);
  }
  const int fsw = frow & 7;

  f32x4 acc[4][4];
#pragma unroll
  for (int i = 0; i < 4; ++i)
#pragma unroll
    for (int j = 0; j < 4; ++j) acc[i][j] = f32x4{0.f, 0.f, 0.f, 0.f};

  const int nk = (K + G_BK - 1) / G_BK;
  u32x4 sa[4], sb[4];
  auto load_tile = [&](int kt) {
    const int k0 = kt * G_BK;
    const bool kok = (k0 + skc * 8) < K;
#pragma unroll
    for (int q = 0; q < 4; ++q) {
      sa[q] = ldg128(ra, kok ? a_off[q] + (uint32_t)k0 * 2u : SGL_OOB);
      sb[q] = ldg128(rb, kok ? b_off[q] + (uint32_t)k0 * 2u : SGL_OOB);
    }
  };
  auto store_stage = [&](int stage) {
    char* base = smem + stage * G_STAGE;
#pragma unroll
    for (int q = 0; q < 4; ++q) {
      *reinterpret_cast<u32x4*>(base + l_off[q]) = sa[q];
      *reinterpret_cast<u32x4*>(base + G_BM * 128 + l_off[q]) = sb[q];
    }
  };

  load_tile(0);
  store_stage(0);
  __syncthreads();
  for (int kt = 0; kt < nk; ++kt) {
    const int cur = kt & 1;
    if (kt + 1 < nk) load_tile(kt + 1);
    const char* base = smem + cur * G_STAGE;
#pragma unroll
    for (int s = 0; s < 2; ++s) {
      const uint32_t coff = (uint32_t)(((4 * s + fg) ^ fsw) << 4);
      lo_x8<TIn> af[4], bfr[4];
#pragma unroll
      for (int i = 0; i < 4; ++i) {
        af[i] = *reinterpret_cast<const lo_x8<TIn>*>(base + fa_row[i] + coff);
        bfr[i] = *reinterpret_cast<const lo_x8<TIn>*>(base + fb_row[i] + coff);
      }
#pragma unroll
      for (int i = 0; i < 4; ++i)
#pragma unroll
        for (int j = 0; j < 4; ++j)
          acc[i][j] = mfma_16x16x32(af[i], bfr[j], acc[i][j]);
    }
// ... 220 lines not shown
```

### deepfake-detection-using-clip-based-siglip-2-vision-transformers_amd/csrc/gemm_bf16_v2.hip

```cpp
#include <stdlib.h>
#ifdef SGL_TIMELINE
#include <stdio.h>
#include <string.h>
#endif

#include "common.hip.h"
#include "epilogue.hip.h"
#include "kernels.h"

namespace sgl {

constexpr int T_BK = 64;

template <int BM_, int BN_, int MI_, int MJ_>
struct NtTileShape {
  static constexpr int BM = BM_, BN = BN_, MI = MI_, MJ = MJ_;
  static constexpr int WM = 16 * MI, WN = 16 * MJ;
  static constexpr int NWR = BM / WM, NWC = BN / WN;
  static constexpr int OPA = BM * T_BK * 2;
  static constexpr int STAGE = (BM + BN) * T_BK * 2;
  static constexpr int LDS = 2 * STAGE;
  static constexpr int PA = BM / 128, PB = BN / 64, NI = 2 * PA + PB;
  static constexpr int CT_LD = BN + 4;
  static_assert(NWR * WM == BM && NWC * WN == BN && NWR * NWC == 8, "8 waves = 512 threads cover the tile");
// ... 79 lines not shown
        const void* src = (EPI == EPI_RES_F32)
                              ? (const void*)(p.res + (size_t)grow * p.ldr + gcol[h])
                              : (const void*)(reinterpret_cast<const TOut*>(p.aux) + (size_t)grow * p.ldaux + gcol[h]);
        dst[q] = (grow < M && col_ok[h]) ? *reinterpret_cast<const PreT*>(src) : PreT{0u, 0u, 0u, 0u};
      }
    }
  };
  load_pre(0, pre[0]);
#pragma unroll
  for (int pass = 0; pass < NPASS; ++pass) {
    if (pass + 1 < NPASS) load_pre(pass + 1, pre[(pass + 1) & 1]);
    lds_barrier();
#pragma unroll
    for (int i2 = 0; i2 < BLK; ++i2)
#pragma unroll
      for (int j = 0; j < G::MJ; ++j)
#pragma unroll
        for (int r = 0; r < 4; ++r)
          ct[(wr * WR_ROWS + i2 * 16 + g * 4 + r) * CT_LD + wc * G::WN + j * 16 + c16] = acc[BLK * pass + i2][j][r];
    lds_barrier();
    if constexpr (EPI == EPI_F32) {
      if (p.atomic) {
        float* outp = reinterpret_cast<float*>(p.out);
        const int w = t >> 6;
#pragma unroll 2
        for (int rr = 0; rr < 8; ++rr) {
          const int row = w + rr * 8;
          const int grow = grow_of(pass, row);
          if (grow >= M) continue;
#pragma unroll
          for (int h = 0; h < G::BN / 64; ++h) {
            const int col = lane + 64 * h;
            if (n0 + col < N) atomicAdd(outp + (size_t)grow * p.ldo + n0 + col, ct[row * CT_LD + col] * p.alpha);
          }
        }
        continue;
      }
    }
#pragma unroll
    for (int q = 0; q < QN; ++q) {
      const int h = q % P;
      const int row = (t + 512 * q) / CPR;
      const int grow = grow_of(pass, row);
      if (grow < M && col_ok[h]) {
        float v[NV];
        Vec<float, NV>::ld(ct + row * CT_LD + tcol[h], v);
        if constexpr (EPI == EPI_RES_F32) {
          const f32x4 r = __builtin_bit_cast(f32x4, pre[pass & 1][q]);
          float rf[NV];
#pragma unroll
          for (int j = 0; j < NV; ++j) rf[j] = r[j];
          epi_res_f32<NV>(v, bias[h], rf, reinterpret_cast<float*>(p.out) + (size_t)grow * p.ldo + gcol[h]);
        } else if constexpr (EPI == EPI_BIAS_GELU) {
          epi_bias_gelu<TOut, NV>(p, v, bias[h], reinterpret_cast<TOut*>(p.out) + (size_t)grow * p.ldo + gcol[h],
                                  reinterpret_cast<TOut*>(p.out2) + (size_t)grow * p.ldo2 + gcol[h]);
        } else if constexpr (EPI == EPI_QKV) {
          int b, n;
          qkv_split_row(grow, p.tokens, b, n);
          epi_qkv<TOut, NV>(v, bias[h],
                            reinterpret_cast<TOut*>(p.out) + qkv_c0[h] + ((size_t)b * p.heads * p.tokens + n) * p.head_dim_pad,
                            qkv_pad[h]);
        } else if constexpr (EPI == EPI_GELU_BWD) {
          float u[NV];
          if constexpr (NV == 8) {
            const lo_x8<TOut> ub = __builtin_bit_cast(lo_x8<TOut>, pre[pass & 1][q]);
#pragma unroll
            for (int j = 0; j < NV; ++j) u[j] = (float)ub[j];
          } else {
            const f32x4 uf = __builtin_bit_cast(f32x4, pre[pass & 1][q]);
#pragma unroll
            for (int j = 0; j < NV; ++j) u[j] = uf[j];
          }
          epi_gelu_bwd<TOut, NV>(p, v, u, reinterpret_cast<TOut*>(p.out) + (size_t)grow * p.ldo + gcol[h]);
#pragma unroll
          for (int j = 0; j < NV; ++j) csum[j] += v[j];
        } else {
          epi_apply<EPI, TOut, NV>(p, grow, gcol[h], N, v);
        }
      }
    }
  }
  if constexpr (EPI == EPI_GELU_BWD) {
    static_assert(P == 1, "the bias-gradient fold needs one column set per thread");
    epi_colsum_fold<512, G::BN, NV>(ct, csum, t, m0, n0, N, p);
  }
}

__device__ __forceinline__ int unit_of_block(int bid, int per) { return (bid & 7) * per + (bid >> 3); }

__device__ __forceinline__ void tile_of_unit(int u, int tiles_m, int tiles_n, int& tile_m, int& tile_n, int bh = 8) {
  const int band = u / (bh * tiles_n);
  const int rows = (tiles_m - band * bh < bh) ? tiles_m - band * bh : bh;
  const int r = u - band * bh * tiles_n;
  tile_n = r / rows;
  tile_m = band * bh + (r - tile_n * rows);
}

__device__ __forceinline__ bool tile_of_local(int xcd, int v, int tiles_m, int tiles_n, int cgw, int& tm, int& tn) {
  const int r_lo = (xcd * tiles_m) >> 3, r_hi = ((xcd + 1) * tiles_m) >> 3;
  const int R = r_hi - r_lo;
  if (v >= R * tiles_n) return false;
  const int full = R * cgw;
  const int g = v / full, rem = v - g * full;
  const int w = (tiles_n - g * cgw < cgw) ? tiles_n - g * cgw : cgw;
  const int r = rem / w;
  tm = r_lo + r;
  tn = g * cgw + (rem - r * w);
  return true;
}

__device__ __forceinline__ void pp_dma16(u32x4 desc, uint32_t lds_addr, uint32_t voff) {
  asm volatile("s_mov_b32 m0, %0\n\ts_nop 0\n\tbuffer_load_dwordx4 %1, %2, 0 offen lds"
               :: "s"(lds_addr), "v"(voff), "s"(desc) : "memory");
}
__device__ __forceinline__ u32x4 pp_desc(const void* base, uint32_t bytes) {
  const uint64_t q = (uint64_t)base;
  u32x4 d = {(uint32_t)q, (uint32_t)(q >> 32) & 0xffffu, bytes, 0x00020000u};
  return d;
}
__device__ __forceinline__ u32x4 pp_desc_sgpr(u32x4 d) {
  return u32x4{(uint32_t)__builtin_amdgcn_readfirstlane((int)d[0]), (uint32_t)__builtin_amdgcn_readfirstlane((int)d[1]),
               (uint32_t)__builtin_amdgcn_readfirstlane((int)d[2]), (uint32_t)__builtin_amdgcn_readfirstlane((int)d[3])};
}
template <int NI>
__device__ __forceinline__ void pp_end_read() {
  asm volatile("s_waitcnt vmcnt(%0) lgkmcnt(0)" :: "n"(NI) : "memory");
  __builtin_amdgcn_sched_barrier(0);
  __builtin_amdgcn_s_barrier();
  __builtin_amdgcn_sched_barrier(0);
}
#define SGL_PP_END_MFMA()                 \
  do {                                    \
    __builtin_amdgcn_sched_barrier(0);    \
    __builtin_amdgcn_s_barrier();         \
    __builtin_amdgcn_sched_barrier(0);    \
  } while (0)

#ifdef SGL_TIMELINE
__device__ unsigned long long g_nt6_tl[4];
__device__ unsigned long long g_tn6_tl[12];
#define SGL_TL_STAMP(v) const unsigned long long v = __builtin_readcyclecounter()
#else
#define SGL_TL_STAMP(v)
#endif

template <typename G, int EPI, typename TOut, typename TIn>
__global__ __launch_bounds__(512, 2) void gemm_nt6_kernel(const TIn* __restrict__ A, int lda,
                                                          const TIn* __restrict__ B, int ldb, int M, int N, int K,
                                                          int tiles_m, int tiles_n, int band_h, EpiParams p) {
  extern __shared__ __attribute__((aligned(16))) char smem[];
  SGL_TL_STAMP(tl0);
  const int ntiles = tiles_m * tiles_n;
  int tile_m, tile_n;
  if (band_h < 0) {
    if (!tile_of_local(blockIdx.x & 7, blockIdx.x >> 3, tiles_m, tiles_n, -band_h, tile_m, tile_n)) return;
  } else {
    const int unit = unit_of_block(blockIdx.x, (ntiles + 7) >> 3);
    if (unit >= ntiles) return;
    tile_of_unit(unit, tiles_m, tiles_n, tile_m, tile_n, band_h);
  }
  constexpr int MI = G::MI, MJ = G::MJ, HI = MI / 2, PA = G::PA, PB = G::PB, NI = G::NI;
  const int t = threadIdx.x, lane = t & 63;
  const int w = __builtin_amdgcn_readfirstlane(t >> 6);
  const int wr = G::wr(w), wc = G::wc(w), grp = w >> 2;
  const int m0 = tile_m * G::BM, n0 = tile_n * G::BN;
  const int rows_a = (M - m0 < G::BM) ? M - m0 : G::BM;
  const int rows_b = (N - n0 < G::BN) ? N - n0 : G::BN;
// ... 366 lines not shown
```

### deepfake-detection-using-clip-based-siglip-2-vision-transformers_amd/csrc/kernels.h

```cpp
#pragma once
#include <hip/hip_runtime.h>
#include <stddef.h>
#include <stdint.h>

#include "siglip_hip.h"

namespace sgl {

enum DType : int {
  DT_F32 = 0,
  DT_BF16 = 1,
  DT_F32_MFMA = 2,
  DT_F16 = 3,
};
static inline size_t dtype_size(int dt) { return (dt == DT_BF16 || dt == DT_F16) ? 2 : 4; }

template <auto Kernel>
hipError_t set_max_dynamic_lds_once(int bytes) {
  static bool done = false;
  if (done) return hipSuccess;
  const hipError_t e =
      hipFuncSetAttribute(reinterpret_cast<const void*>(Kernel), hipFuncAttributeMaxDynamicSharedMemorySize, bytes);
  done = e == hipSuccess;
  return e;
}

static inline bool view_box_ok(const sgl_view& r, int B, int Hs, int Ws) {
  return r.src >= 0 && r.src < B && r.x0 >= 0 && r.x0 < r.x1 && r.x1 <= Ws && r.y0 >= 0 && r.y0 < r.y1 && r.y1 <= Hs;
}

enum Epi : int {
  EPI_STORE = 0,
  EPI_BIAS_GELU = 1,
  EPI_RES_F32 = 2,
  EPI_QKV = 3,
  EPI_GELU_BWD = 4,
  EPI_POS_F32 = 5,
  EPI_F32 = 6,
};

struct EpiParams {
  void* out = nullptr;   int ldo = 0;
  void* out2 = nullptr;  int ldo2 = 0;
  const float* bias = nullptr;
  const float* res = nullptr;  int ldr = 0;
  const void* aux = nullptr;   int ldaux = 0;
  const float* pos = nullptr;  int pos_rows = 1;
  int tokens = 1, heads = 1, head_dim = 8, head_dim_pad = 8, batch = 1;
  float alpha = 1.0f;
  int accumulate = 0;
  int atomic = 0;
  float* colsum = nullptr;
  int colsum_ld = 0;
  int gelu_grad_form = 0;
  size_t split_stride = 0;
};

hipError_t quantize_mx(const void* x, int x_dtype, int ldx, int M, int K, int Kp, void* q, void* sc, hipStream_t s);
hipError_t layernorm_fwd_mx(const float* x, const float* gamma, const float* beta, void* q, void* sc, int M, int D, int Kp,
                            float eps, hipStream_t s);
hipError_t gemm_nt_mx(const void* A, const void* As, const void* B, const void* Bs, int M, int N, int Kp, int epi,
                      const EpiParams& p, void* out_sc, hipStream_t s);

hipError_t layernorm_fwd(const float* x, const float* gamma, const float* beta, void* y, int y_dtype, int ldy,
                         float* mean, float* rstd, int M, int D, float eps, hipStream_t s);
int layernorm_bwd_blocks(int M);
hipError_t layernorm_bwd(const void* dy, int dy_dtype, int lddy, const float* x, const float* mean,
                         const float* rstd, const float* gamma, const float* dres, float* dx, void* dx_lp,
                         int lp_dtype, float* partial, int nblk, int M, int D, hipStream_t s);
hipError_t reduce_partials(const float* partial, int nblk, int stride, float* out, int n, int accumulate,
                           hipStream_t s);
hipError_t reduce_partials3(const float* partial, int nblk, int stride, float* o0, float* o1, float* o2, int n, int a0,
                            int a1, int a2, hipStream_t s);

hipError_t im2col(const float* pix, int channels_last, void* out, int out_dtype, int B, int H, int W, int P,
                  int Kp, hipStream_t s);
hipError_t col2im(const float* d_cols, int B, int H, int W, int P, int Kp, float* d_pixels, int channels_last,
                  hipStream_t s);
hipError_t cast_pad(const float* src, int R, int C, int lds_, void* dst, int dst_dtype, int Rp, int Cp, int ldd,
                    hipStream_t s);
struct CastMat {
  const float* src;
  void* dst;
  void* dst_t;
  int R, C, lds, Rp, Cp, ldd, ldt, tiles_c, tile0;
};
struct CastJob {
  CastMat m[6];
  const float* vsrc[4];
  float* vdst[4];
  int vn[4], vnp[4];
  int nmat = 0, nvec = 0, ntiles = 0;
};
void cast_job_add(CastJob& job, const float* src, int R, int C, int lds_, void* dst, int Rp, int Cp, int ldd, void* dst_t,
                  int ldt);
void cast_job_add_vec(CastJob& job, const float* src, int n, float* dst, int np);
hipError_t cast_job_run(const CastJob& job, int dst_dtype, hipStream_t s);
hipError_t split3_rows(const float* src, int R, int C, int ld, void* dst, int Cs, int b_side, hipStream_t s);
hipError_t split3_stack(const float* src, int R, int C, int ld, void* dst, int Cs, int b_side, hipStream_t s);
int colsum_chunks(int M);
hipError_t colsum(const void* in, int dtype, int ld, int M, int N, int n_out, float* partial ,
                  float* out, int accumulate, hipStream_t s);
hipError_t batch_sum(const float* in, int B, size_t n, float* out, int accumulate, hipStream_t s);
hipError_t vecmat_f32(const float* v, const float* W, int rows, int cols, float* scratch, float* out, int accumulate,
                      hipStream_t s);
hipError_t pos_resize(const float* table, int g0, float* out, int gh, int gw, int D, hipStream_t s);
hipError_t pos_resize_bwd(const float* dout, int gh, int gw, float* dtable, int g0, int D, hipStream_t s);
hipError_t copy_f32(const float* src, float* dst, size_t n, hipStream_t s);
hipError_t cast_f32(const float* src, void* dst, int dst_dtype, size_t n, hipStream_t s);
hipError_t add_f32(const float* a, const float* b, float* out, size_t n, hipStream_t s);
static inline size_t pool_attn_lds_floats(int N, int DP, int backward) {
  const size_t part = (size_t)N * (DP / 8) > (size_t)256 * 8 ? (size_t)N * (DP / 8) : (size_t)256 * 8;
  return part + (backward ? 2 : 1) * (size_t)N + 8;
}
static inline int pool_attn_max_tokens(int DP, int backward) {
  return (int)((64 * 1024 / sizeof(float) - 8) / (size_t)(DP / 8 + (backward ? 2 : 1)));
}
hipError_t pool_attn_fwd(const float* q, const void* K, const void* V, int dtype, void* out ,
                         float* probs , int B, int H, int N, int dh, int DP, hipStream_t s);
hipError_t pool_attn_bwd(const float* q, const void* K, const void* V, int dtype, const float* probs,
                         const float* dout , void* dkv ,
                         float* dq_partial , int B, int H, int N, int dh, int DP, hipStream_t s);

hipError_t gemm_f32_generic(const float* A, long sam, long sak, const float* B, long sbn, long sbk, int M, int N,
                            int K, int epi, int out_dtype, const EpiParams& p, hipStream_t s);

hipError_t gemm_nt_bf16(const void* A, int lda, const void* B, int ldb, int M, int N, int K, int epi,
                        int out_dtype, const EpiParams& p, hipStream_t s);
hipError_t reduce_splits(const float* ws, int splits, size_t stride, int N1, int N2, float* out, int ldo, int accumulate,
                         hipStream_t s);
hipError_t gemm_tn_bf16(const void* A, int lda, const void* B, int ldb, int Mred, int N1, int N2, int splits,
                        const EpiParams& p, hipStream_t s, float* split_ws = nullptr, size_t split_ws_bytes = 0);
hipError_t gemm_nt_f16(const void* A, int lda, const void* B, int ldb, int M, int N, int K, int epi, int out_dtype,
                       const EpiParams& p, hipStream_t s);
hipError_t gemm_tn_f16(const void* A, int lda, const void* B, int ldb, int Mred, int N1, int N2, int splits,
                       const EpiParams& p, hipStream_t s, float* split_ws = nullptr, size_t split_ws_bytes = 0);
template <typename TIn>
hipError_t gemm_nt256(const void* A, int lda, const void* B, int ldb, int M, int N, int K, int epi, int out_dtype,
                      const EpiParams& p, hipStream_t s);
template <typename TIn>
hipError_t gemm_nt384(const void* A, int lda, const void* B, int ldb, int M, int N, int K, int epi, int out_dtype,
                      const EpiParams& p, hipStream_t s);
template <typename TIn>
hipError_t gemm_tn256(const void* A, int lda, const void* B, int ldb, int Mred, int N1, int N2, int m_per, int splits,
                      const EpiParams& p, hipStream_t s);
template <typename TIn>
hipError_t gemm_tn384(const void* A, int lda, const void* B, int ldb, int Mred, int N1, int N2, int m_per, int splits,
                      const EpiParams& p, hipStream_t s);

struct TnPlan {
  int tile, splits, m_per;
};
constexpr TnPlan tn_plan(int Mred, int N1, int N2, size_t ws_bytes, int tile = 0) {
  TnPlan best = {0, 0, 0};
  long best_cost = 0;
  for (int g = 0; g < 2; ++g) {
    const int bm = g ? 384 : 256, bn = g ? 192 : 256, area8 = g ? 9 : 8;
    if (tile != 0 && tile != bm) continue;
    const int tiles = ((N1 + bm - 1) / bm) * ((N2 + bn - 1) / bn);
    for (int sp = 1; sp == 1 || (tiles * sp <= 256 && Mred / sp >= 1024); ++sp) {
      if (sp > 1 && (size_t)sp * N1 * N2 * sizeof(float) > ws_bytes) break;
      const int m_per = ((Mred + sp - 1) / sp + 63) / 64 * 64;
      const long cost = (long)area8 * m_per;
      if (best.tile == 0 || cost < best_cost) {
        best = {bm, (Mred + m_per - 1) / m_per, m_per};
        best_cost = cost;
      }
    }
  }
  return best;
}
constexpr bool tn_plan_is(int Mred, int N1, int N2, size_t ws_bytes, int tile, int splits) {
  const TnPlan p = tn_plan(Mred, N1, N2, ws_bytes);
  return (tile == 0 || p.tile == tile) && p.splits == splits;
}
constexpr size_t kTnSlabBytes = (size_t)256 * 384 * 192 * 4;
static_assert(tn_plan_is(93312, 1152, 1152, kTnSlabBytes, 384, 14), "out_proj dW");
static_assert(tn_plan_is(93312, 3456, 1152, kTnSlabBytes, 384, 4), "QKV dW");
static_assert(tn_plan_is(93312, 4304, 1152, kTnSlabBytes, 256, 3), "fc1 dW");
static_assert(tn_plan_is(93312, 1152, 4304, kTnSlabBytes, 256, 3), "fc2 dW");
static_assert(tn_plan_is(4133, 520, 1152, kTnSlabBytes, 0, 4) && tn_plan(4133, 520, 1152, kTnSlabBytes).m_per == 1088, "digest case");
static_assert(tn_plan_is(2048, 512, 512, kTnSlabBytes, 256, 2) && tn_plan(2048, 512, 512, kTnSlabBytes).m_per == 1024, "digest case");

hipError_t attn_fwd(const void* q, const void* k, const void* v, int dtype, void* out, float* lse, int B, int H,
                    int N, int dh, int DP, int ld_qkv, hipStream_t s);
hipError_t attn_bwd(const void* q, const void* k, const void* v, const void* out, const void* dout,
                    const float* lse, int dtype, void* dqkv, float* delta, float* reserved, int B, int H, int N,
                    int dh, int DP, int ld_qkv, hipStream_t s);

}
```

### deepfake-detection-using-clip-based-siglip-2-vision-transformers_amd/csrc/layernorm.hip

```cpp
#include "common.hip.h"
#include "kernels.h"

namespace sgl {

constexpr int LN_MAXV_MAX = 8;

template <typename TOut, int LN_MAXV>
__global__ __launch_bounds__(256) void ln_fwd_kernel(const float* __restrict__ x, const float* __restrict__ gamma,
                                                     const float* __restrict__ beta, TOut* __restrict__ y, int ldy,
                                                     float* __restrict__ mean, float* __restrict__ rstd, int M, int D,
                                                     float eps) {
  const int lane = lane_id();
  const int nv = D >> 2;
  const int stride = gridDim.x * 4;
  int row = blockIdx.x * 4 + wave_id();
  if (row >= M) return;
  f32x4 v[LN_MAXV], nx[LN_MAXV];
#pragma unroll
  for (int i = 0; i < LN_MAXV; ++i) {
    const int c = lane + i * 64;
    const f32x4 z = {0.f, 0.f, 0.f, 0.f};
    v[i] = (c < nv) ? __builtin_nontemporal_load(reinterpret_cast<const f32x4*>(x + (size_t)row * D) + c) : z;
    nx[i] = z;
  }
// ... 136 lines not shown
        const f32x4 gm = reinterpret_cast<const f32x4*>(gsm)[c];
        float o[4];
#pragma unroll
        for (int j = 0; j < 4; ++j) {
          const float h = (xv[i][j] - mu) * rs;
          const float g = (float)dv[i][j] * gm[j];
          o[j] = rs * (g - c1 - h * c2);
        }
        if (rr) {
#pragma unroll
          for (int j = 0; j < 4; ++j) o[j] += rv[i][j];
        }
        Vec<float, 4>::st_nt(dxr + c * 4, o);
#pragma unroll
        for (int j = 0; j < 4; ++j) ds[i][j] += o[j];
        if (dx_lp) Vec<TLp, 4>::st_nt(dx_lp + (size_t)row * D + c * 4, o);
      }
    }
  }
  if (!partial) return;
  float* mine = ln_smem + (size_t)w * D;
  float* out = partial + (size_t)blockIdx.x * 3 * D;
#pragma unroll
  for (int ph = 0; ph < 3; ++ph) {
#pragma unroll
    for (int i = 0; i < LN_MAXV; ++i) {
      const int c = lane + i * 64;
      if (c < nv) reinterpret_cast<f32x4*>(mine)[c] = (ph == 0) ? dg[i] : ((ph == 1) ? db[i] : ds[i]);
    }
    __syncthreads();
    for (int j = threadIdx.x; j < D; j += 256)
      out[ph * D + j] = (ln_smem[j] + ln_smem[D + j]) + (ln_smem[2 * D + j] + ln_smem[3 * D + j]);
    __syncthreads();
  }
}

int layernorm_bwd_blocks(int M) {
  int b = (M + 3) / 4;
  return b < 1 ? 1 : (b > 768 ? 768 : b);
}

template <typename TDy, typename TLp>
static hipError_t ln_bwd_launch2(const void* dy, int lddy, const float* x, const float* mean, const float* rstd,
                                 const float* gamma, const float* dres, float* dx, void* dx_lp, float* partial,
                                 int nblk, int M, int D, hipStream_t s) {
  dim3 grid(nblk), block(256);
  const size_t smem = (size_t)5 * D * sizeof(float);
#define SGL_LNB(V)                                                                                                  \
  hipLaunchKernelGGL((ln_bwd_kernel<TDy, TLp, V>), grid, block, smem, s, (const TDy*)dy, lddy, x, mean, rstd, gamma, \
                     dres, dx, (TLp*)dx_lp, partial, M, D)
  if (D <= 512)
    SGL_LNB(2);
  else if (D <= 1280)
    SGL_LNB(5);
  else
    SGL_LNB(8);
#undef SGL_LNB
  return hipGetLastError();
}

template <typename TDy>
static hipError_t ln_bwd_launch(const void* dy, int lddy, const float* x, const float* mean, const float* rstd,
                                const float* gamma, const float* dres, float* dx, void* dx_lp, int lp_dtype,
                                float* partial, int nblk, int M, int D, hipStream_t s) {
  if (lp_dtype == DT_BF16)
    return ln_bwd_launch2<TDy, bf16>(dy, lddy, x, mean, rstd, gamma, dres, dx, dx_lp, partial, nblk, M, D, s);
  if (lp_dtype == DT_F16)
    return ln_bwd_launch2<TDy, f16>(dy, lddy, x, mean, rstd, gamma, dres, dx, dx_lp, partial, nblk, M, D, s);
  return ln_bwd_launch2<TDy, float>(dy, lddy, x, mean, rstd, gamma, dres, dx, dx_lp, partial, nblk, M, D, s);
}

hipError_t layernorm_bwd(const void* dy, int dy_dtype, int lddy, const float* x, const float* mean,
                         const float* rstd, const float* gamma, const float* dres, float* dx, void* dx_lp,
                         int lp_dtype, float* partial, int nblk, int M, int D, hipStream_t s) {
  if (D % 4 || D > 64 * 4 * LN_MAXV_MAX || lddy % 4) return hipErrorInvalidValue;
  if (M == 0) return hipSuccess;
  if (dy_dtype == DT_BF16)
    return ln_bwd_launch<bf16>(dy, lddy, x, mean, rstd, gamma, dres, dx, dx_lp, lp_dtype, partial, nblk, M, D, s);
  if (dy_dtype == DT_F16)
    return ln_bwd_launch<f16>(dy, lddy, x, mean, rstd, gamma, dres, dx, dx_lp, lp_dtype, partial, nblk, M, D, s);
  return ln_bwd_launch<float>(dy, lddy, x, mean, rstd, gamma, dres, dx, dx_lp, lp_dtype, partial, nblk, M, D, s);
}

__global__ __launch_bounds__(256) void reduce_partials_kernel(const float* __restrict__ partial, int nblk, int stride,
                                                              float* __restrict__ out, int n, int accumulate) {
  __shared__ float red[8][33];
  const int c = threadIdx.x & 31, g = threadIdx.x >> 5;
  const int j = blockIdx.x * 32 + c;
  float s0 = 0.f, s1 = 0.f;
  if (j < n) {
    int b = g;
    for (; b + 8 < nblk; b += 16) {
      s0 += partial[(size_t)b * stride + j];
      s1 += partial[(size_t)(b + 8) * stride + j];
    }
    if (b < nblk) s0 += partial[(size_t)b * stride + j];
  }
  red[g][c] = s0 + s1;
  __syncthreads();
  if (g == 0 && j < n) {
    float r = 0.f;
#pragma unroll
    for (int k = 0; k < 8; ++k) r += red[k][c];
    out[j] = accumulate ? out[j] + r : r;
  }
}

__global__ __launch_bounds__(256) void reduce_partials3_kernel(const float* __restrict__ partial, int nblk, int stride,
                                                               float* __restrict__ o0, float* __restrict__ o1,
                                                               float* __restrict__ o2, int n, int a0, int a1, int a2) {
  __shared__ float red[8][33];
  const int c = threadIdx.x & 31, g = threadIdx.x >> 5;
  const int j = blockIdx.x * 32 + c;
  const int which = j / n, jj = j - which * n;
  float* o = which == 0 ? o0 : (which == 1 ? o1 : o2);
  const int acc = which == 0 ? a0 : (which == 1 ? a1 : a2);
  const bool live = (j < 3 * n) && o;
  float s0 = 0.f, s1 = 0.f, s2 = 0.f, s3 = 0.f;
  if (live) {
    int b = g;
    for (; b + 24 < nblk; b += 32) {
      s0 += partial[(size_t)b * stride + j];
      s1 += partial[(size_t)(b + 8) * stride + j];
      s2 += partial[(size_t)(b + 16) * stride + j];
      s3 += partial[(size_t)(b + 24) * stride + j];
    }
    for (; b < nblk; b += 8) s0 += partial[(size_t)b * stride + j];
  }
  red[g][c] = (s0 + s1) + (s2 + s3);
  __syncthreads();
  if (g == 0 && live) {
    float r = 0.f;
#pragma unroll
    for (int k = 0; k < 8; ++k) r += red[k][c];
    o[jj] = acc ? o[jj] + r : r;
  }
}

hipError_t reduce_partials3(const float* partial, int nblk, int stride, float* o0, float* o1, float* o2, int n, int a0,
                            int a1, int a2, hipStream_t s) {
  if (n == 0 || (!o0 && !o1 && !o2)) return hipSuccess;
  hipLaunchKernelGGL(reduce_partials3_kernel, dim3((3 * n + 31) / 32), dim3(256), 0, s, partial, nblk, stride, o0, o1,
                     o2, n, a0, a1, a2);
  return hipGetLastError();
}

hipError_t reduce_partials(const float* partial, int nblk, int stride, float* out, int n, int accumulate,
                           hipStream_t s) {
  if (n == 0) return hipSuccess;
  hipLaunchKernelGGL(reduce_partials_kernel, dim3((n + 31) / 32), dim3(256), 0, s, partial, nblk, stride, out, n,
                     accumulate);
  return hipGetLastError();
}

}
```

### deepfake-detection-using-clip-based-siglip-2-vision-transformers_amd/lib.py

```python
from __future__ import annotations

import ctypes as C
import os
import re

_HERE = os.path.dirname(os.path.abspath(__file__))
LIB_PATH = os.environ.get("SGL_LIB_PATH") or os.path.join(_HERE, "libsiglip_hip.so")
HEADER_PATH = os.path.join(os.path.dirname(_HERE), "include", "siglip_hip.h")

SGL_DTYPE_F32, SGL_DTYPE_BF16, SGL_DTYPE_BF16X3, SGL_DTYPE_F16, SGL_DTYPE_MXFP8 = 0, 1, 2, 3, 5
SGL_DTYPE_U8 = 6
SEG_EVAL_AUC_BINS = 4096
SGL_RECOMPUTE_NONE, SGL_RECOMPUTE_BLOCKS = 0, 1
EPI_STORE, EPI_BIAS_GELU, EPI_RES_F32, EPI_QKV, EPI_GELU_BWD, EPI_POS_F32, EPI_F32 = range(7)
STATUS = {0: "ok", -1: "bad shape", -2: "unsupported configuration", -3: "buffer too small", -4: "HIP error",
          -5: "null pointer"}

_fp = C.c_void_p


class SglConfig(C.Structure):
    _fields_ = [("hidden_size", C.c_int), ("intermediate_size", C.c_int), ("num_layers", C.c_int),
                ("num_heads", C.c_int), ("patch_size", C.c_int), ("native_grid", C.c_int),
                ("layer_norm_eps", C.c_float), ("compute_dtype", C.c_int), ("use_head", C.c_int)]


LAYER_FIELDS = ["ln1_w", "ln1_b", "q_w", "q_b", "k_w", "k_b", "v_w", "v_b", "o_w", "o_b", "ln2_w", "ln2_b",
                "fc1_w", "fc1_b", "fc2_w", "fc2_b"]
HEAD_FIELDS = ["probe", "in_proj_w", "in_proj_b", "out_proj_w", "out_proj_b", "head_ln_w", "head_ln_b",
               "head_fc1_w", "head_fc1_b", "head_fc2_w", "head_fc2_b"]


class SglLayerPtrs(C.Structure):
    _fields_ = [(n, _fp) for n in LAYER_FIELDS]


class SglWeights(C.Structure):
    _fields_ = ([("patch_w", _fp), ("patch_b", _fp), ("pos", _fp), ("layers", C.POINTER(SglLayerPtrs)),
                 ("post_ln_w", _fp), ("post_ln_b", _fp)] + [(n, _fp) for n in HEAD_FIELDS])


class SglGrads(C.Structure):
    _fields_ = ([("patch_w", _fp), ("patch_b", _fp), ("pos", _fp), ("layers", C.POINTER(SglLayerPtrs)),
                 ("post_ln_w", _fp), ("post_ln_b", _fp)] + [(n, _fp) for n in HEAD_FIELDS] +
                [("accumulate", C.c_int)])


class SglAdamwTensor(C.Structure):
    _fields_ = [("p", _fp), ("g", _fp), ("m", _fp), ("v", _fp), ("n", C.c_uint64), ("lr", C.c_float),
                ("weight_decay", C.c_float)]


class SglAdamwAux(C.Structure):
    _fields_ = [("dst", _fp), ("dst_t", _fp), ("dst_f32", _fp), ("ema", _fp), ("ld", C.c_int), ("ld_t", C.c_int),
                ("rows", C.c_int), ("cols", C.c_int), ("row0", C.c_int), ("dtype", C.c_int), ("group", C.c_int),
                ("reserved", C.c_int)]


class SglCastMat(C.Structure):
    _fields_ = [("src", _fp), ("dst", _fp), ("dst_t", _fp)] + [(n, C.c_int) for n in ("R", "C", "lds", "Rp", "Cp", "ldd",
                                                                                    "ldt")]


class SglCastVec(C.Structure):
    _fields_ = [("src", _fp), ("dst", _fp), ("n", C.c_int), ("np", C.c_int)]


class SglView(C.Structure):
    _fields_ = [(n, C.c_int32) for n in ("src", "x0", "y0", "x1", "y1", "turns", "keep_canvas", "flip")]


_lib = None


def declared_symbols() -> list[str]:
    with open(HEADER_PATH) as f:
        text = f.read()
    text = re.sub(r"/\*.*?\*/", "", text, flags=re.S)
    return sorted(set(re.findall(r"\b(sgl_[a-z0-9_]+)\s*\(", text)))


def _sig(lib, name, restype, argtypes):
    fn = getattr(lib, name)
    fn.restype = restype
    fn.argtypes = argtypes
    return fn


def load():
    global _lib
    if _lib is not None:
        return _lib
    if not os.path.exists(LIB_PATH):
        raise RuntimeError(
            f"{LIB_PATH} not found: build it with `python -c 'import __graft_entry__ as g; g.build()'` "
            "(hipcc --offload-arch=gfx950).  There is no CPU fallback for the encoder path.")
    lib = C.CDLL(LIB_PATH)
    missing = [s for s in declared_symbols() if not hasattr(lib, s)]
    if missing:
        raise RuntimeError(f"{LIB_PATH} lacks symbols declared in siglip_hip.h: {missing}")
    i, sz, f = C.c_int, C.c_size_t, C.c_float
    psz = C.POINTER(C.c_size_t)
    _sig(lib, "sgl_abi_version", i, [])
    _sig(lib, "sgl_status_string", C.c_char_p, [i])
    _sig(lib, "sgl_create", C.c_void_p, [C.POINTER(SglConfig)])
    _sig(lib, "sgl_create_ex", C.c_void_p, [C.POINTER(SglConfig), i])
    _sig(lib, "sgl_destroy", None, [C.c_void_p])
    _sig(lib, "sgl_last_hip_error", i, [C.c_void_p])
    _sig(lib, "sgl_query_sizes", i, [C.c_void_p, i, i, i, i, psz, psz, psz])
    _sig(lib, "sgl_prepare_weights", i, [C.c_void_p, C.POINTER(SglWeights), _fp, sz, _fp])
    _sig(lib, "sgl_prepare_weights_dirty", i, [C.c_void_p, C.POINTER(SglWeights), _fp, sz, C.c_char_p, i, _fp])
    _sig(lib, "sgl_forward", i, [C.c_void_p, C.POINTER(SglWeights), _fp, _fp, i, i, i, i, i, _fp, i, _fp, _fp, _fp, sz,
                                 _fp, sz, _fp])
    _sig(lib, "sgl_forward_ex", i, [C.c_void_p, C.POINTER(SglWeights), _fp, _fp, i, i, i, i, i, _fp, i, _fp, _fp, _fp, sz,
                                    _fp, sz, i, _fp])
    _sig(lib, "sgl_forward_slots", i, [C.c_void_p, C.POINTER(SglWeights), _fp, _fp, i, i, i, i, i, C.POINTER(_fp), _fp, _fp,
                                       _fp, sz, _fp, sz, i, _fp])
    _sig(lib, "sgl_backward_begin_p", i, [C.c_void_p, C.POINTER(SglWeights), _fp, C.POINTER(SglGrads), i, i, i, _fp, _fp,
                                          _fp, _fp, _fp, sz, _fp, sz, _fp])
    _sig(lib, "sgl_backward_layer_p", i, [C.c_void_p, C.POINTER(SglWeights), _fp, C.POINTER(SglGrads), i, i, i, i, _fp,
                                          _fp, i, _fp, sz, _fp, sz, _fp])
    _sig(lib, "sgl_backward_begin", i, [C.c_void_p, C.POINTER(SglWeights), _fp, C.POINTER(SglGrads), i, i, i, _fp, _fp,
                                        _fp, _fp, _fp, sz, _fp, sz, _fp])
    _sig(lib, "sgl_backward_layer", i, [C.c_void_p, C.POINTER(SglWeights), _fp, C.POINTER(SglGrads), i, i, i, i, _fp,
                                        _fp, i, _fp, sz, _fp, sz, _fp])
    _sig(lib, "sgl_backward_embed", i, [C.c_void_p, C.POINTER(SglWeights), C.POINTER(SglGrads), i, i, i, i, _fp, sz,
                                        _fp, sz, _fp])
    _sig(lib, "sgl_query_input_grad_bytes", i, [C.c_void_p, i, i, i, psz])
    _sig(lib, "sgl_backward_embed_px", i, [C.c_void_p, C.POINTER(SglWeights), C.POINTER(SglGrads), i, i, i, i, _fp, i, _fp,
                                           sz, _fp, sz, _fp, sz, _fp])
    _sig(lib, "sgl_backward", i, [C.c_void_p, C.POINTER(SglWeights), _fp, C.POINTER(SglGrads), i, i, i, i, _fp,
                                  C.POINTER(_fp), _fp, _fp, i, i, _fp, sz, _fp, sz, _fp])
    _sig(lib, "sgl_op_layernorm_fwd", i, [_fp, _fp, _fp, _fp, i, _fp, _fp, i, i, f, _fp])
    _sig(lib, "sgl_op_layernorm_bwd", i, [_fp, i, _fp, _fp, _fp, _fp, _fp, _fp, _fp, i, _fp, _fp, _fp, sz, i, i, _fp])
    _sig(lib, "sgl_op_gemm_nt", i, [i, _fp, i, _fp, i, i, i, i, i, _fp, i, _fp, i, _fp, _fp, i, _fp, i, _fp, i, i, i,
                                    i, i, i, _fp])
    _sig(lib, "sgl_op_quantize_mxfp8", i, [_fp, i, i, i, i, i, _fp, _fp, _fp])
    _sig(lib, "sgl_op_layernorm_fwd_mx", i, [_fp, _fp, _fp, _fp, _fp, i, i, i, f, _fp])
    _sig(lib, "sgl_op_gemm_nt_mx", i, [_fp, _fp, _fp, _fp, i, i, i, i, _fp, i, _fp, _fp, _fp, i, i, i, i, i, i, _fp])
    _sig(lib, "sgl_op_gemm_tn", i, [i, _fp, i, _fp, i, i, i, i, i, _fp, i, i, _fp])
    _sig(lib, "sgl_op_gemm_tn_ws", i, [i, _fp, i, _fp, i, i, i, i, i, _fp, i, i, _fp, sz, _fp])
    _sig(lib, "sgl_op_attn_fwd", i, [i, _fp, _fp, _fp, _fp, _fp, i, i, i, i, i, i, _fp])
    _sig(lib, "sgl_op_attn_bwd", i, [i, _fp, _fp, _fp, _fp, _fp, _fp, _fp, _fp, i, i, i, i, i, i, _fp])
    _sig(lib, "sgl_op_colsum", i, [i, _fp, i, i, i, _fp, i, _fp, sz, _fp])
    _sig(lib, "sgl_op_im2col", i, [_fp, i, _fp, i, i, i, i, i, i, _fp])
    _sig(lib, "sgl_op_col2im", i, [_fp, i, i, i, i, i, _fp, i, _fp])
    _sig(lib, "sgl_op_pos_resize", i, [_fp, i, _fp, i, i, i, _fp])
    _sig(lib, "sgl_op_pool_attn_fwd", i, [i, _fp, _fp, _fp, _fp, _fp, i, i, i, i, i, _fp])
    _sig(lib, "sgl_op_pool_attn_bwd", i, [i, _fp, _fp, _fp, _fp, _fp, _fp, _fp, i, i, i, i, i, _fp])
    _sig(lib, "sgl_op_pos_resize_bwd", i, [_fp, i, i, _fp, i, i, _fp])
    _sig(lib, "sgl_op_cast_pad", i, [_fp, i, i, i, _fp, i, i, i, i, _fp])
    _sig(lib, "sgl_op_cast_job", i, [C.POINTER(SglCastMat), i, C.POINTER(SglCastVec), i, i, _fp])
    _sig(lib, "sgl_op_split3", i, [_fp, i, i, i, _fp, i, i, i, _fp])
    _sig(lib, "sgl_op_batch_sum", i, [_fp, i, sz, _fp, i, _fp])
    _sig(lib, "sgl_op_vecmat", i, [_fp, _fp, i, i, _fp, sz, _fp, i, _fp])
    _sig(lib, "sgl_op_reduce_partials", i, [_fp, i, i, _fp, i, i, _fp])
    _sig(lib, "sgl_op_reduce_partials3", i, [_fp, i, i, _fp, _fp, _fp, i, i, i, i, _fp])
    _sig(lib, "sgl_op_reduce_splits", i, [_fp, i, sz, i, i, _fp, i, i, _fp])
    _sig(lib, "sgl_op_add_f32", i, [_fp, _fp, _fp, sz, _fp])
    _sig(lib, "sgl_op_cast_f32", i, [_fp, _fp, i, sz, _fp])
    i64 = C.c_int64
    _sig(lib, "sgl_adamw_plan", i64, [C.POINTER(C.c_uint64), i, C.POINTER(C.c_int32), i64])
    _sig(lib, "sgl_op_grad_norm", i, [_fp, _fp, i64, f, _fp, _fp, _fp])
    _sig(lib, "sgl_op_adamw", i, [_fp, _fp, i64, C.c_double, C.c_double, C.c_double, i, _fp, _fp])
    _sig(lib, "sgl_op_ema", i, [_fp, _fp, i64, C.c_double, _fp])
    _sig(lib, "sgl_adamw_bind_shadows", i, [C.c_void_p, C.POINTER(SglWeights), _fp, C.POINTER(SglAdamwTensor),
                                            C.POINTER(SglAdamwAux), i])
    _sig(lib, "sgl_op_grad_norm_scaled", i, [_fp, _fp, i64, f, f, _fp, _fp, _fp])
    _sig(lib, "sgl_op_adamw_ex", i, [_fp, _fp, _fp, i64, C.c_double, C.c_double, C.c_double, i, _fp,
                                     C.POINTER(C.c_float), i, C.c_double, _fp])
    _sig(lib, "sgl_op_dwconv3x3", i, [_fp, i, _fp, _fp, _fp, i, i, i, i, i, _fp])
    _sig(lib, "sgl_op_dwconv3x3_wgrad_scratch_bytes", sz, [i, i, i, i])
    _sig(lib, "sgl_op_dwconv3x3_wgrad", i, [_fp, _fp, i, _fp, i, _fp, sz, i, i, i, i, _fp])
    _sig(lib, "sgl_op_preprocess", i, [_fp, i, i, i, i, _fp, i, i, i, i, i, f, f, _fp, f, _fp])
    _sig(lib, "sgl_op_preprocess_bwd_scratch_bytes", sz, [i, i, i, i])
    _sig(lib, "sgl_op_preprocess_bwd", i, [_fp, i, i, i, i, f, _fp, f, _fp, _fp, sz, _fp])
    _sig(lib, "sgl_op_preprocess_aug", i, [_fp, i, i, i, i, _fp, i, i, i, i, i, f, f, _fp, _fp, _fp])
    _sig(lib, "sgl_op_preprocess_aug_bwd_scratch_bytes", sz, [i, i, i, i])
    _sig(lib, "sgl_op_preprocess_aug_bwd", i, [_fp, _fp, i, i, i, i, i, f, _fp, _fp, _fp, sz, _fp])
    _sig(lib, "sgl_op_preprocess_views_scratch_bytes", sz, [i, i])
    _sig(lib, "sgl_op_preprocess_views", i, [_fp, i, i, i, i, C.POINTER(SglView), i, _fp, i, i, i, i, i, f, f, _fp, sz,
                                             _fp])
    _sig(lib, "sgl_op_preprocess_views_bwd_scratch_bytes", sz, [C.POINTER(SglView), i, i])
    _sig(lib, "sgl_op_preprocess_views_bwd", i, [_fp, i, i, i, C.POINTER(SglView), i, i, f, _fp, _fp, sz, _fp])
    _sig(lib, "sgl_op_freq_features_scratch_bytes", sz, [i, i, i])
    _sig(lib, "sgl_op_freq_features", i, [_fp, i, i, i, C.POINTER(SglView), i, _fp, _fp, i, _fp, _fp, sz, _fp])
    _sig(lib, "sgl_op_l2norm_tmean_fwd", i, [_fp, _fp, _fp, i, i, i, _fp])
    _sig(lib, "sgl_op_l2norm_tmean_bwd", i, [_fp, _fp, _fp, _fp, i, i, i, _fp])
    _sig(lib, "sgl_op_gate_mul", i, [_fp, _fp, _fp, sz, i, _fp])
    _sig(lib, "sgl_op_gate_mul_bwd", i, [_fp, _fp, _fp, _fp, _fp, sz, i, _fp])
    _sig(lib, "sgl_op_seg_loss_chunks", i, [i])
    _sig(lib, "sgl_op_seg_loss_fwd", i, [_fp, _fp, _fp, i, i, i, _fp])
    _sig(lib, "sgl_op_seg_loss_bwd", i, [_fp, _fp, _fp, _fp, _fp, i, i, i, f, _fp])
    _sig(lib, "sgl_op_seg_eval_auc_bins", i, [])
    _sig(lib, "sgl_op_seg_eval", i, [_fp, _fp, i, _fp, _fp, i, _fp, _fp, i, i, i, _fp])
    _lib = lib
    return lib


class SglError(RuntimeError):
    pass


def check(status: int, what: str, ctx=None):
    if status == 0:
        return
    msg = STATUS.get(status, f"status {status}")
    if status == -4 and ctx is not None and _lib is not None:
        msg += f" (hipError_t {_lib.sgl_last_hip_error(ctx)})"
    raise SglError(f"{what}: {msg}")


def ptr(t) -> int | None:
    return None if t is None else t.data_ptr()


def current_stream_handle(device) -> int:
    import torch
    return torch.cuda.current_stream(device).cuda_stream


def call(symbol: str, device, *args) -> None:
    import torch
    fn = getattr(load(), symbol)
    with torch.cuda.device(device):
        status = fn(*args, current_stream_handle(device))
# ... 10 lines not shown
```

### include/siglip_hip.h

```cpp
#ifndef SIGLIP_HIP_H
#define SIGLIP_HIP_H
#include <stddef.h>
#include <stdint.h>

#ifdef __cplusplus
extern "C" {
#endif

typedef struct sgl_ctx sgl_ctx;
typedef void* sgl_stream;

enum { SGL_DTYPE_F32 = 0, SGL_DTYPE_BF16 = 1, SGL_DTYPE_BF16X3 = 2, SGL_DTYPE_F16 = 3, SGL_DTYPE_MXFP8 = 5 };
enum { SGL_DTYPE_U8 = 6 };

typedef enum {
  SGL_OK = 0,
  SGL_ERR_BAD_SHAPE = -1,
  SGL_ERR_UNSUPPORTED = -2,
  SGL_ERR_WORKSPACE = -3,
  SGL_ERR_HIP = -4,
  SGL_ERR_NULL = -5
} sgl_status;

typedef struct {
// ... 44 lines not shown
} sgl_grads;

sgl_ctx* sgl_create(const sgl_config* cfg);
enum { SGL_RECOMPUTE_NONE = 0, SGL_RECOMPUTE_BLOCKS = 1 };
sgl_ctx* sgl_create_ex(const sgl_config* cfg, int recompute);
void sgl_destroy(sgl_ctx* ctx);
int sgl_last_hip_error(const sgl_ctx* ctx);
const char* sgl_status_string(int status);
int sgl_abi_version(void);

int sgl_query_sizes(const sgl_ctx* ctx, int B, int H, int W, int train, size_t* shadow_bytes, size_t* saved_bytes,
                    size_t* ws_bytes);

int sgl_prepare_weights(sgl_ctx* ctx, const sgl_weights* w, void* shadow, size_t shadow_bytes, sgl_stream stream);
int sgl_prepare_weights_dirty(sgl_ctx* ctx, const sgl_weights* w, void* shadow, size_t shadow_bytes,
                              const unsigned char* layer_dirty, int globals_dirty, sgl_stream stream);

int sgl_forward(sgl_ctx* ctx, const sgl_weights* w, const void* shadow, const float* pixels, int channels_last, int B,
                int H, int W, int interpolate_pos, float* hidden_states, int hs_slots, float* last_hidden,
                float* pooled, void* saved, size_t saved_bytes, void* ws, size_t ws_bytes, sgl_stream stream);
int sgl_forward_ex(sgl_ctx* ctx, const sgl_weights* w, const void* shadow, const float* pixels, int channels_last, int B,
                   int H, int W, int interpolate_pos, float* hidden_states, int hs_slots, float* last_hidden,
                   float* pooled, void* saved, size_t saved_bytes, void* ws, size_t ws_bytes, int first_trainable_block,
                   sgl_stream stream);

int sgl_forward_slots(sgl_ctx* ctx, const sgl_weights* w, const void* shadow, const float* pixels, int channels_last,
                      int B, int H, int W, int interpolate_pos, float* const* hs_slots, float* last_hidden,
                      float* pooled, void* saved, size_t saved_bytes, void* ws, size_t ws_bytes,
                      int first_trainable_block, sgl_stream stream);

int sgl_backward_begin(sgl_ctx* ctx, const sgl_weights* w, const void* shadow, const sgl_grads* g, int B, int H, int W,
                       const float* hidden_states, const float* d_last_hidden, const float* d_pooled,
                       const float* d_tap_last, const void* saved, size_t saved_bytes, void* ws, size_t ws_bytes,
                       sgl_stream stream);
int sgl_backward_layer(sgl_ctx* ctx, const sgl_weights* w, const void* shadow, const sgl_grads* g, int layer, int B,
                       int H, int W, const float* hidden_states, const float* d_tap, int need_dx, const void* saved,
                       size_t saved_bytes, void* ws, size_t ws_bytes, sgl_stream stream);
int sgl_backward_begin_p(sgl_ctx* ctx, const sgl_weights* w, const void* shadow, const sgl_grads* g, int B, int H, int W,
                         const float* hs_last, const float* d_last_hidden, const float* d_pooled,
                         const float* d_tap_last, const void* saved, size_t saved_bytes, void* ws, size_t ws_bytes,
                         sgl_stream stream);
int sgl_backward_layer_p(sgl_ctx* ctx, const sgl_weights* w, const void* shadow, const sgl_grads* g, int layer, int B,
                         int H, int W, const float* hs_in, const float* d_tap, int need_dx, const void* saved,
                         size_t saved_bytes, void* ws, size_t ws_bytes, sgl_stream stream);
int sgl_backward_embed(sgl_ctx* ctx, const sgl_weights* w, const sgl_grads* g, int B, int H, int W, int interpolate_pos,
                       const void* saved, size_t saved_bytes, void* ws, size_t ws_bytes, sgl_stream stream);
int sgl_query_input_grad_bytes(const sgl_ctx* ctx, int B, int H, int W, size_t* scratch_bytes);
int sgl_backward_embed_px(sgl_ctx* ctx, const sgl_weights* w, const sgl_grads* g, int B, int H, int W,
                          int interpolate_pos, float* d_pixels, int channels_last, void* px_scratch,
                          size_t px_scratch_bytes, const void* saved, size_t saved_bytes, void* ws, size_t ws_bytes,
                          sgl_stream stream);
int sgl_backward(sgl_ctx* ctx, const sgl_weights* w, const void* shadow, const sgl_grads* g, int B, int H, int W,
                 int interpolate_pos, const float* hidden_states, const float* const* d_taps,
                 const float* d_last_hidden, const float* d_pooled, int first_trainable_block, int train_embeddings,
                 const void* saved, size_t saved_bytes, void* ws, size_t ws_bytes, sgl_stream stream);

int sgl_op_layernorm_fwd(const float* x, const float* gamma, const float* beta, void* y, int y_dtype, float* mean,
                         float* rstd, int M, int D, float eps, sgl_stream stream);
int sgl_op_layernorm_bwd(const void* dy, int dy_dtype, const float* x, const float* mean, const float* rstd,
                         const float* gamma, const float* dres, float* dx, void* dx_lp, int lp_dtype, float* dgamma,
                         float* dbeta, float* scratch, size_t scratch_bytes, int M, int D, sgl_stream stream);
enum { SGL_EPI_STORE = 0, SGL_EPI_BIAS_GELU = 1, SGL_EPI_RES_F32 = 2, SGL_EPI_QKV = 3, SGL_EPI_GELU_BWD = 4,
       SGL_EPI_POS_F32 = 5, SGL_EPI_F32 = 6 };
int sgl_op_gemm_nt(int dtype, const void* A, int lda, const void* B, int ldb, int M, int N, int K, int epi, void* out,
                   int ldo, void* out2, int ldo2, const float* bias, const float* res, int ldr, const void* aux,
                   int ldaux, const float* pos, int pos_rows, int tokens, int heads, int head_dim, int head_dim_pad,
                   int batch, sgl_stream stream);
int sgl_op_quantize_mxfp8(const void* x, int x_dtype, int ldx, int M, int K, int Kp, void* q, void* scales,
                          sgl_stream stream);
int sgl_op_layernorm_fwd_mx(const float* x, const float* gamma, const float* beta, void* q, void* scales, int M, int D,
                            int Kp, float eps, sgl_stream stream);
int sgl_op_gemm_nt_mx(const void* A, const void* As, const void* B, const void* Bs, int M, int N, int Kp, int epi,
                      void* out, int ldo, void* out_scales, const float* bias, const float* res, int ldr, int tokens,
                      int heads, int head_dim, int head_dim_pad, int batch, sgl_stream stream);
int sgl_op_gemm_tn(int dtype, const void* A, int lda, const void* B, int ldb, int Mred, int N1, int N2, int splits,
                   float* out, int ldo, int accumulate, sgl_stream stream);
int sgl_op_gemm_tn_ws(int dtype, const void* A, int lda, const void* B, int ldb, int Mred, int N1, int N2, int splits,
                      float* out, int ldo, int accumulate, float* scratch, size_t scratch_bytes, sgl_stream stream);
int sgl_op_attn_fwd(int dtype, const void* q, const void* k, const void* v, void* out, float* lse, int B, int H, int N,
                    int head_dim, int head_dim_pad, int ld_qkv, sgl_stream stream);
int sgl_op_attn_bwd(int dtype, const void* q, const void* k, const void* v, const void* out, const void* dout,
                    const float* lse, void* dqkv, float* delta_scratch, int B, int H, int N, int head_dim,
                    int head_dim_pad, int ld_qkv, sgl_stream stream);
int sgl_op_colsum(int dtype, const void* in, int ld, int M, int N, float* out, int accumulate, float* scratch,
                  size_t scratch_bytes, sgl_stream stream);
int sgl_op_im2col(const float* pixels, int channels_last, void* out, int out_dtype, int B, int H, int W, int P, int Kp,
                  sgl_stream stream);
int sgl_op_col2im(const float* d_cols, int B, int H, int W, int P, int Kp, float* d_pixels, int channels_last,
                  sgl_stream stream);
int sgl_op_pos_resize(const float* table, int native_grid, float* out, int gh, int gw, int D, sgl_stream stream);

int sgl_op_pool_attn_fwd(int dtype, const float* q, const void* K, const void* V, void* out, float* probs, int B, int H,
                         int N, int head_dim, int head_dim_pad, sgl_stream stream);
int sgl_op_pool_attn_bwd(int dtype, const float* q, const void* K, const void* V, const float* probs, const float* dout,
                         void* dkv, float* dq_partial, int B, int H, int N, int head_dim, int head_dim_pad,
                         sgl_stream stream);
int sgl_op_pos_resize_bwd(const float* dout, int gh, int gw, float* dtable, int native_grid, int D, sgl_stream stream);
int sgl_op_cast_pad(const float* src, int R, int C, int lds, void* dst, int dst_dtype, int Rp, int Cp, int ldd,
                    sgl_stream stream);
typedef struct {
  const float* src;
  void* dst;
  void* dst_t;
  int R, C, lds, Rp, Cp, ldd, ldt;
} sgl_cast_mat;
typedef struct {
  const float* src;
  float* dst;
  int n, np;
} sgl_cast_vec;
int sgl_op_cast_job(const sgl_cast_mat* mats, int nmat, const sgl_cast_vec* vecs, int nvec, int dst_dtype,
                    sgl_stream stream);
int sgl_op_split3(const float* src, int R, int C, int ld, void* dst, int Cs, int b_side, int stacked, sgl_stream stream);
int sgl_op_batch_sum(const float* in, int B, size_t n, float* out, int accumulate, sgl_stream stream);
int sgl_op_vecmat(const float* v, const float* W, int rows, int cols, float* scratch, size_t scratch_bytes, float* out,
                  int accumulate, sgl_stream stream);
int sgl_op_reduce_partials(const float* partial, int nblk, int stride, float* out, int n, int accumulate,
                           sgl_stream stream);
int sgl_op_reduce_partials3(const float* partial, int nblk, int stride, float* out0, float* out1, float* out2, int n,
                            int accumulate0, int accumulate1, int accumulate2, sgl_stream stream);
int sgl_op_reduce_splits(const float* ws, int splits, size_t stride, int N1, int N2, float* out, int ldo, int accumulate,
                         sgl_stream stream);
int sgl_op_add_f32(const float* a, const float* b, float* out, size_t n, sgl_stream stream);
int sgl_op_cast_f32(const float* src, void* dst, int dst_dtype, size_t n, sgl_stream stream);

int sgl_op_dwconv3x3(const void* x, int dtype, const float* w9, const float* bias, void* y, int B, int gh, int gw, int E,
                     int flip, sgl_stream stream);
size_t sgl_op_dwconv3x3_wgrad_scratch_bytes(int B, int gh, int gw, int E);
int sgl_op_dwconv3x3_wgrad(const void* x, const void* dy, int dtype, float* dw10, int accumulate, float* scratch,
                           size_t scratch_bytes, int B, int gh, int gw, int E, sgl_stream stream);

int sgl_op_preprocess(const void* src, int src_is_u8_nhwc, int B, int Hs, int Ws, void* out, int out_dtype, int S, int P,
                      int Kp, int patch_major, float mean, float std, const int* mix_index, float lam,
                      sgl_stream stream);
size_t sgl_op_preprocess_bwd_scratch_bytes(int B, int Hs, int Ws, int S);
int sgl_op_preprocess_bwd(const float* d_out, int B, int Hs, int Ws, int S, float std, const int* mix_index, float lam,
                          float* d_src, void* scratch, size_t scratch_bytes, sgl_stream stream);

typedef struct sgl_view {
  int32_t src, x0, y0, x1, y1, turns, keep_canvas, flip;
} sgl_view;
size_t sgl_op_preprocess_views_scratch_bytes(int V, int S);
int sgl_op_preprocess_views(const void* src, int src_is_u8_nhwc, int B, int Hs, int Ws, const sgl_view* views, int V,
                            void* out, int out_dtype, int S, int P, int Kp, int patch_major, float mean, float std,
                            void* scratch, size_t scratch_bytes, sgl_stream stream);
size_t sgl_op_preprocess_views_bwd_scratch_bytes(const sgl_view* views, int V, int S);
int sgl_op_preprocess_views_bwd(const float* d_out, int B, int Hs, int Ws, const sgl_view* views, int V, int S, float std,
                                float* d_src, void* scratch, size_t scratch_bytes, sgl_stream stream);

size_t sgl_op_freq_features_scratch_bytes(int V, int Hs, int Ws);
int sgl_op_freq_features(const void* src_u8_nhwc, int B, int Hs, int Ws, const sgl_view* views, int V,
                         const unsigned char* geometry, float* out , int standardize,
                         unsigned char* gray_out , void* scratch, size_t scratch_bytes,
                         sgl_stream stream);

typedef struct sgl_aug_sample {
  float flip, cos_a, sin_a, brightness, contrast, saturation, hue;
  int order[4];
  int reserved;
} sgl_aug_sample;
int sgl_op_preprocess_aug(const void* src, int src_is_u8_nhwc, int B, int Hs, int Ws, void* out, int out_dtype, int S,
                          int P, int Kp, int patch_major, float mean, float std, const sgl_aug_sample* aug,
                          float* grey_mean, sgl_stream stream);
size_t sgl_op_preprocess_aug_bwd_scratch_bytes(int B, int Hs, int Ws, int S);
int sgl_op_preprocess_aug_bwd(const float* d_out, const void* src, int src_is_u8_nhwc, int B, int Hs, int Ws, int S,
                              float std, const sgl_aug_sample* aug, float* d_src, void* scratch, size_t scratch_bytes,
                              sgl_stream stream);

int sgl_op_l2norm_tmean_fwd(const float* f, float* out, float* inv_norm, int B, int T, int D, sgl_stream stream);
int sgl_op_l2norm_tmean_bwd(const float* f, const float* inv_norm, const float* dout, float* df, int B, int T, int D,
                            sgl_stream stream);

int sgl_op_gate_mul(const void* g, const void* x, void* y, size_t n, int dtype, sgl_stream stream);
int sgl_op_gate_mul_bwd(const void* dy, const void* g, const void* x, void* dg, void* dx, size_t n, int dtype,
                        sgl_stream stream);
int sgl_op_seg_loss_chunks(int S);
int sgl_op_seg_loss_fwd(const float* logits_lr, const float* targets, float* partial, int B, int g, int S,
                        sgl_stream stream);
int sgl_op_seg_loss_bwd(const float* logits_lr, const float* targets, const float* sums, const float* coef,
                        float* dlogits_lr, int B, int g, int S, float eps, sgl_stream stream);

#define SGL_SEG_EVAL_AUC_BINS 4096
int sgl_op_seg_eval_auc_bins(void);
int sgl_op_seg_eval(const float* logits_lr, const void* targets, int target_dtype, const uint8_t* sel, const float* cuts,
                    int K, int32_t* hist, unsigned long long* auc_hist, int B, int g, int S, sgl_stream stream);

typedef struct {
  float* p;
  const float* g;
  float* m;
  float* v;
  uint64_t n;
  float lr, weight_decay;
} sgl_adamw_tensor;
int64_t sgl_adamw_plan(const uint64_t* numel, int ntensors, int32_t* blockmap, int64_t capacity_pairs);
int sgl_op_grad_norm(const sgl_adamw_tensor* table, const int32_t* blockmap, int64_t nblocks, float max_norm,
                     float* partials, float* norm_and_coef, sgl_stream stream);
int sgl_op_adamw(const sgl_adamw_tensor* table, const int32_t* blockmap, int64_t nblocks, double beta1, double beta2,
                 double eps, int step, const float* norm_and_coef, sgl_stream stream);
typedef struct {
  void* dst;
  void* dst_t;
  float* dst_f32;
// ... 18 lines not shown
```

Before: 435.3 images/sec.

## Fuse q-bias gradient into attention backward and batch bias-grad reductions into one fold kernel

The attention dQ backward kernel now also produces per-128-row column partial sums of dQ, so the separate bias_grad pass that re-read dqkv for the q bias is skipped. Several small reduce/zero/batch_sum launches in the MLP and attention backward paths are merged into one multi-job fold kernel, and the csum memset is dropped. The aim is to cut extra memory passes and kernel launch overhead per layer. The cost is added LDS work and barriers at the end of the dQ kernel, plus more complex bookkeeping in the fold kernel.

After: 437.0 images/sec, median of 6. Within noise of the previous version (+0.4%).

```diff
diff --git a/deepfake-detection-using-clip-based-siglip-2-vision-transformers_amd/csrc/attention.hip b/deepfake-detection-using-clip-based-siglip-2-vision-transformers_amd/csrc/attention.hip
--- a/deepfake-detection-using-clip-based-siglip-2-vision-transformers_amd/csrc/attention.hip
+++ b/deepfake-detection-using-clip-based-siglip-2-vision-transformers_amd/csrc/attention.hip
@@ -442,7 +442,8 @@
                                                             const T* __restrict__ V, const T* __restrict__ O,
                                                             const T* __restrict__ dO, const float* __restrict__ lse,
                                                             float* __restrict__ aux, T* __restrict__ dqkv,
-                                                            int B, int H, int N, int dh, int ld, float c, float scale) {
+                                                            int B, int H, int N, int dh, int ld, float c, float scale,
+                                                            float* __restrict__ qsum, int qld) {
   using C = AttnCfg<DP>;
   constexpr int KT = 32;
   constexpr int SCK = C::DSTR / 16, SCV = C::RSTR / 16;
@@ -614,6 +615,42 @@
         }
       }
   }
+  if (qsum) {
+    constexpr int TS = 36, ND = C::DT * 32;
+    static_assert((4 * 32 * TS + 8 * ND) * 4 <= 3 * STAGE, "the fold images fit in the tile stages");
+    float* img = reinterpret_cast<float*>(smem) + w * (32 * TS);
+    float* part = reinterpret_cast<float*>(smem) + 4 * 32 * TS;
+    asm volatile("s_waitcnt lgkmcnt(0)" ::: "memory");
+    __builtin_amdgcn_s_barrier();
+    asm volatile("" ::: "memory");
+#pragma unroll
+    for (int dt = 0; dt < C::DT; ++dt) {
+#pragma unroll
+      for (int g4 = 0; g4 < 4; ++g4) {
+        f32x4 v;
+#pragma unroll
+        for (int r = 0; r < 4; ++r) {
+          const int d = dt * 32 + 8 * g4 + 4 * hh + r;
+          v[r] = (q < N && d < dh) ? (float)(T)dq[dt][4 * g4 + r] : 0.f;
+        }
+        *reinterpret_cast<f32x4*>(img + li * TS + 8 * g4 + 4 * hh) = v;
+      }
+      asm volatile("s_waitcnt lgkmcnt(0)" ::: "memory");
+      float sum = 0.f;
+#pragma unroll
+      for (int k = 0; k < 16; ++k) sum += img[(2 * k + hh) * TS + li];
+      part[(w * 2 + hh) * ND + dt * 32 + li] = sum;
+      asm volatile("s_waitcnt lgkmcnt(0)" ::: "memory");
+    }
+    __builtin_amdgcn_s_barrier();
+    asm volatile("" ::: "memory");
+    if (t < ND && t < dh) {
+      float r = 0.f;
+#pragma unroll
+      for (int k = 0; k < 8; ++k) r += part[k * ND + t];
+      qsum[((size_t)b * ((N + 127) / 128) + xb) * qld + hd * dh + t] = r;
+    }
+  }
 }
 
 template <typename T, int DP>
@@ -633,8 +670,8 @@
 
 template <typename T, int DP>
 static hipError_t bwd_launch(const T* q, const T* k, const T* v, const T* out, const T* dout,
-                             const float* lse, T* dqkv, float* delta, int B, int H, int N, int dh, int ld,
-                             hipStream_t s) {
+                             const float* lse, T* dqkv, float* delta, float* qsum, int qld, int B, int H, int N,
+                             int dh, int ld, hipStream_t s) {
   using C = AttnCfg<DP>;
   const float scale = 1.0f / sqrtf((float)dh);
   const float c = scale * 1.4426950408889634f;
@@ -643,10 +680,10 @@
   const dim3 grid = head_grid((N + 127) / 128, B * H), block(256);
   if (ld > 0)
     hipLaunchKernelGGL((attn_bwd_q_kernel<T, DP, true>), grid, block, smem_q, s, q, k, v, out, dout, lse, delta, dqkv, B, H, N,
-                       dh, ld, c, scale);
+                       dh, ld, c, scale, qsum, qld);
   else
     hipLaunchKernelGGL((attn_bwd_q_kernel<T, DP, false>), grid, block, smem_q, s, q, k, v, out, dout, lse, delta, dqkv, B, H, N,
-                       dh, 0, c, scale);
+                       dh, 0, c, scale, qsum, qld);
   hipError_t e = hipGetLastError();
   if (e != hipSuccess) return e;
   if (ld > 0)
@@ -692,9 +729,10 @@
 }
 
 hipError_t attn_bwd(const void* q, const void* k, const void* v, const void* out, const void* dout, const float* lse,
-                    int dtype, void* dqkv, float* delta, float* , int B, int H, int N, int dh, int DP,
+                    int dtype, void* dqkv, float* delta, float* qsum, int qld, int B, int H, int N, int dh, int DP,
                     int ld, hipStream_t s) {
   if (B * H == 0 || N == 0) return hipSuccess;
+  if (qsum && dtype != DT_BF16 && dtype != DT_F16) return hipErrorInvalidValue;
   if (dtype == DT_F32)
     return attn_ref_bwd((const float*)q, (const float*)k, (const float*)v, (const float*)out, (const float*)dout, lse,
                         (float*)dqkv, delta, B, H, N, dh, DP, ld, s);
@@ -703,10 +741,11 @@
                         (float*)dqkv, delta, B, H, N, dh, DP, ld, s);
   if (!attn_shape_ok(N, dh, DP, H, ld)) return hipErrorInvalidValue;
   if ((((uintptr_t)q) | ((uintptr_t)k) | ((uintptr_t)v)) & 15) return hipErrorInvalidValue;
+  if (qsum && qld < H * dh) return hipErrorInvalidValue;
 #define SGL_B(T, DPV)                                                                                  \
   case DPV:                                                                                            \
     return bwd_launch<T, DPV>((const T*)q, (const T*)k, (const T*)v, (const T*)out, (const T*)dout, lse, \
-                              (T*)dqkv, delta, B, H, N, dh, ld, s);
+                              (T*)dqkv, delta, qsum, qld, B, H, N, dh, ld, s);
   if (dtype == DT_F16) {
     switch (DP) {
       SGL_B(f16, 16) SGL_B(f16, 32) SGL_B(f16, 48) SGL_B(f16, 64) SGL_B(f16, 80) SGL_B(f16, 96)
diff --git a/deepfake-detection-using-clip-based-siglip-2-vision-transformers_amd/csrc/elementwise.hip b/deepfake-detection-using-clip-based-siglip-2-vision-transformers_amd/csrc/elementwise.hip
--- a/deepfake-detection-using-clip-based-siglip-2-vision-transformers_amd/csrc/elementwise.hip
+++ b/deepfake-detection-using-clip-based-siglip-2-vision-transformers_amd/csrc/elementwise.hip
@@ -321,7 +321,7 @@
   return hipGetLastError();
 }
 
-constexpr int VECMAT_CHUNKS = 16;
+constexpr int VECMAT_CHUNKS = kVecmatChunks;
 __global__ __launch_bounds__(256) void vecmat_f32_kernel(const float* __restrict__ v, const float* __restrict__ W, int rows,
                                                          int cols, float* __restrict__ partial) {
   __shared__ float part[4][64];
@@ -336,12 +336,16 @@
   __syncthreads();
   if (rg == 0 && j < cols) partial[(size_t)blockIdx.y * cols + j] = (part[0][jj] + part[1][jj]) + (part[2][jj] + part[3][jj]);
 }
+hipError_t vecmat_f32_chunks(const float* v, const float* W, int rows, int cols, float* scratch, hipStream_t s) {
+  if (rows <= 0 || cols <= 0) return hipErrorInvalidValue;
+  hipLaunchKernelGGL(vecmat_f32_kernel, dim3((unsigned)((cols + 63) / 64), VECMAT_CHUNKS), dim3(256), 0, s, v, W, rows, cols,
+                     scratch);
+  return hipGetLastError();
+}
 hipError_t vecmat_f32(const float* v, const float* W, int rows, int cols, float* scratch, float* out, int accumulate,
                       hipStream_t s) {
   if (rows <= 0 || cols <= 0) return hipSuccess;
-  hipLaunchKernelGGL(vecmat_f32_kernel, dim3((unsigned)((cols + 63) / 64), VECMAT_CHUNKS), dim3(256), 0, s, v, W, rows, cols,
-                     scratch);
-  hipError_t e = hipGetLastError();
+  hipError_t e = vecmat_f32_chunks(v, W, rows, cols, scratch, s);
   if (e != hipSuccess) return e;
   return reduce_partials(scratch, VECMAT_CHUNKS, cols, out, cols, accumulate, s);
 }
diff --git a/deepfake-detection-using-clip-based-siglip-2-vision-transformers_amd/csrc/encoder.hip b/deepfake-detection-using-clip-based-siglip-2-vision-transformers_amd/csrc/encoder.hip
--- a/deepfake-detection-using-clip-based-siglip-2-vision-transformers_amd/csrc/encoder.hip
+++ b/deepfake-detection-using-clip-based-siglip-2-vision-transformers_amd/csrc/encoder.hip
@@ -1,7 +1,9 @@
 #include <hip/hip_runtime.h>
+#include <stdlib.h>
 #include <string.h>
 
 #include <algorithm>
+#include <atomic>
 #include <new>
 #include <vector>
 
@@ -17,6 +19,12 @@
 inline const char* at(const void* base, size_t off) { return reinterpret_cast<const char*>(base) + off; }
 inline bool mfma16(int dt) { return dt == DT_BF16 || dt == DT_F16; }
 inline int round_up(int x, int m) { return (x + m - 1) / m * m; }
+
+std::atomic<unsigned long long> g_qsum_fused{0}, g_qsum_fallback{0};
+inline bool qsum_forced_off() {
+  const char* e = getenv("SGL_QSUM");
+  return e && e[0] == '0';
+}
 
 struct Bump {
   size_t off = 0;
@@ -74,6 +82,7 @@
   size_t w_dx = 0, w_g = 0, w_du = 0, w_dh = 0, w_dqkv = 0, w_delta = 0, w_splitws = 0, w_lnpart = 0, w_cspart = 0,
          w_dlast = 0, w_gsum = 0, w_csum = 0;
   size_t w_hg = 0, w_hdu = 0, w_hdh = 0, w_hdao = 0, w_hdqpart = 0, w_hdqp = 0, w_hdh0 = 0;
+  size_t n_csum = 0;
   size_t ws_bwd_total = 0;
   size_t saved_total = 0, ws_total = 0, ws_act_off = 0;
   bool rc = false;
@@ -141,7 +150,8 @@
       w_splitws = w.take(kSplitWsBytes);
       w_lnpart = w.take((size_t)layernorm_bwd_blocks(M) * 3 * D * 4);
       w_gsum = w.take(D * 4);
-      w_csum = w.take((size_t)((M + 127) / 128) * widest * 4);
+      n_csum = (size_t)((M + 127) / 128) * widest;
+      w_csum = w.take(n_csum * 4);
       w_cspart = w.take((size_t)std::max(colsum_chunks(M), 16) * widest * 4);
       w_dlast = w.take(Mz * D * 4);
       w_hg = w.take((size_t)B * D * es);
@@ -334,13 +344,20 @@
 
   int ln_backward(const void* dy, int dy_dt, const float* x, const float* stats, int rows, const float* gamma,
                   const float* dres, float* dx, void* dx_lp, float* dgamma, float* dbeta, int accumulate,
-                  float* colsum_out = nullptr) const {
+                  float* colsum_out = nullptr, FoldJob* fold = nullptr) const {
     const int D = ctx->D;
     const bool want = dgamma || dbeta || colsum_out;
     const int nblk = layernorm_bwd_blocks(rows);
     float* part = wsf(lay.w_lnpart);
     CK(layernorm_bwd(dy, dy_dt, D, x, stats, stats + rows, gamma, dres, dx, dx_lp, ctx->dt, want ? part : nullptr, nblk,
                      rows, D, s));
+    if (fold) {
+      *fold = FoldJob{};
+      fold->partial = part; fold->nblk = nblk; fold->stride = 3 * D; fold->n = D; fold->nout = 3;
+      fold->out[0] = dgamma; fold->out[1] = dbeta; fold->out[2] = colsum_out;
+      fold->acc[0] = fold->acc[1] = accumulate;
+      return SGL_OK;
+    }
     CK(reduce_partials3(part, nblk, 3 * D, dgamma, dbeta, colsum_out, D, accumulate, accumulate, 0, s));
     return SGL_OK;
   }
@@ -894,6 +911,10 @@
   return SGL_OK;
 }
 
+inline hipError_t fold_add(FoldJobs& jobs, const FoldJob& j) {
+  return fold_jobs_add(jobs, j) ? hipSuccess : hipErrorInvalidValue;
+}
+
 int mlp_backward(const Call& c, const sgl_layer_weights& lw, const sgl_layer_grads& lg, const ShadowLayer& sl,
                  const char* lb, int acc) {
   sgl_ctx* ctx = c.ctx;
@@ -907,21 +928,35 @@
   float* gsum = c.wsf(lay.w_gsum);
   float* csum = c.wsf(lay.w_csum);
   const bool fuse_cs = mfma16(dt) && lg.fc1_b;
-  if (fuse_cs) CK(hipMemsetAsync(csum, 0, (size_t)((M + 127) / 128) * Ip * 4, s));
   CK(c.gemm_nt(gbuf, D, c.sh(sl.w2_t), D, M, Ip, D, EPI_GELU_BWD, dt,
                epi_gelu_bwd(du, lb + lay.r_u, Ip, mfma16(dt), fuse_cs ? csum : nullptr)));
   if (lg.fc2_w) CK(c.gemm_tn(gbuf, D, lb + lay.r_a, Ip, M, D, I, lg.fc2_w, I, acc, true));
-  if (lg.fc2_b) CK(batch_sum(gsum, 1, (size_t)D, lg.fc2_b, acc, s));
   CK(c.gemm_nt(du, Ip, c.sh(sl.w1_t), Ip, M, D, Ip, EPI_STORE, dt, epi_store(dhb, D)));
   if (lg.fc1_w) CK(c.gemm_tn(du, Ip, lb + lay.r_h2, D, M, I, D, lg.fc1_w, D, acc, true));
-  if (fuse_cs)
-    CK(reduce_partials(csum, (M + 127) / 128, Ip, lg.fc1_b, I, acc, s));
-  else
-    RET(c.bias_grad(du, Ip, M, Ip, I, lg.fc1_b, acc));
+  if (!fuse_cs) RET(c.bias_grad(du, Ip, M, Ip, I, lg.fc1_b, acc));
+  const bool new_gsum = lg.o_b || lg.v_b;
+  FoldJob ln2;
   RET(c.ln_backward(dhb, dt, reinterpret_cast<const float*>(lb + lay.r_xmid),
                     reinterpret_cast<const float*>(lb + lay.r_stats2), M, lw.ln2_w, dx, dx, gbuf, lg.ln2_w, lg.ln2_b, acc,
-                    (lg.o_b || lg.v_b) ? gsum : nullptr));
-  if (lg.o_b) CK(batch_sum(gsum, 1, (size_t)D, lg.o_b, acc, s));
+                    new_gsum ? gsum : nullptr, &ln2));
+  FoldJobs jobs;
+  if (fuse_cs) {
+    FoldJob j;
+    j.partial = csum; j.nblk = (M + 127) / 128; j.stride = Ip; j.n = I;
+    j.out[0] = lg.fc1_b; j.acc[0] = acc;
+    CK(fold_add(jobs, j));
+  }
+  if (new_gsum) {
+    ln2.prev = lg.fc2_b; ln2.prev_acc = acc;
+    ln2.extra[0] = lg.o_b; ln2.extra_acc[0] = acc;
+  } else if (lg.fc2_b) {
+    FoldJob j;
+    j.partial = gsum; j.nblk = 1; j.stride = D; j.n = D;
+    j.out[0] = lg.fc2_b; j.acc[0] = acc;
+    CK(fold_add(jobs, j));
+  }
+  CK(fold_add(jobs, ln2));
+  CK(fold_jobs_run(jobs, s));
   return SGL_OK;
 }
 
@@ -938,20 +973,43 @@
   const char* q = lb + lay.r_qkv;
   CK(c.gemm_nt(gbuf, D, c.sh(sl.wo_t), D, M, D, D, EPI_STORE, dt, epi_store(dattn, D)));
   if (lg.o_w) CK(c.gemm_tn(gbuf, D, lb + lay.r_attn, D, M, D, D, lg.o_w, D, acc, true));
+  float* gw[3] = {lg.q_w, lg.k_w, lg.v_w};
+  float* gb[3] = {lg.q_b, lg.k_b, lg.v_b};
+  const int qrows = lay.B * ((lay.N + 127) / 128);
+  const bool q_fused = gb[0] && mfma16(dt) && !ctx->split && (size_t)qrows * D <= lay.n_csum && !qsum_forced_off();
+  float* qpart = c.wsf(lay.w_csum);
+  if (gb[0]) (q_fused ? g_qsum_fused : g_qsum_fallback).fetch_add(1, std::memory_order_relaxed);
   CK(attn_bwd(q, q + c.head_bytes(), q + 2 * c.head_bytes(), lb + lay.r_attn, dattn,
               reinterpret_cast<const float*>(lb + lay.r_lse), ctx->split ? DT_F32_MFMA : dt, dqkv, c.wsf(lay.w_delta),
-              nullptr, lay.B, ctx->H, lay.N, ctx->dh, ctx->DP, 0, s));
-  float* gw[3] = {lg.q_w, lg.k_w, lg.v_w};
-  float* gb[3] = {lg.q_b, lg.k_b, lg.v_b};
+              q_fused ? qpart : nullptr, D, lay.B, ctx->H, lay.N, ctx->dh, ctx->DP, 0, s));
   const bool w_adj = gw[0] && gw[1] == gw[0] + (size_t)D * D && gw[2] == gw[1] + (size_t)D * D;
   if (w_adj) CK(c.gemm_tn(dqkv, 3 * D, lb + lay.r_h1, D, M, 3 * D, D, gw[0], D, acc, true));
   for (int j = 0; j < 3; ++j) {
     const char* aj = reinterpret_cast<const char*>(dqkv) + (size_t)j * D * ctx->es;
     if (!w_adj && gw[j]) CK(c.gemm_tn(aj, 3 * D, lb + lay.r_h1, D, M, D, D, gw[j], D, acc, true));
   }
-  if (gb[0]) RET(c.bias_grad(dqkv, 3 * D, M, D, D, gb[0], acc));
-  if (gb[1] && !acc) CK(hipMemsetAsync(gb[1], 0, (size_t)D * 4, s));
-  if (gb[2]) CK(vecmat_f32(gsum, lw.o_w, D, D, c.wsf(lay.w_cspart), gb[2], acc, s));
+  if (gb[0] && !q_fused) RET(c.bias_grad(dqkv, 3 * D, M, D, D, gb[0], acc));
+  FoldJobs jobs;
+  if (q_fused) {
+    FoldJob j;
+    j.partial = qpart; j.nblk = qrows; j.stride = D; j.n = D;
+    j.out[0] = gb[0]; j.acc[0] = acc;
+    CK(fold_add(jobs, j));
+  }
+  if (gb[2]) {
+    float* chunks = c.wsf(lay.w_cspart);
+    CK(vecmat_f32_chunks(gsum, lw.o_w, D, D, chunks, s));
+    FoldJob j;
+    j.partial = chunks; j.nblk = kVecmatChunks; j.stride = D; j.n = D;
+    j.out[0] = gb[2]; j.acc[0] = acc;
+    CK(fold_add(jobs, j));
+  }
+  if (gb[1] && !acc) {
+    FoldJob j;
+    j.zero = gb[1]; j.nzero = D;
+    CK(fold_add(jobs, j));
+  }
+  CK(fold_jobs_run(jobs, s));
   return SGL_OK;
 }
 
@@ -1248,9 +1306,46 @@
 int sgl_op_attn_bwd(int dtype, const void* q, const void* k, const void* v, const void* out, const void* dout,
                     const float* lse, void* dqkv, float* delta_scratch, int B, int H, int N, int head_dim,
                     int head_dim_pad, int ld_qkv, sgl_stream stream) {
-  CKV(attn_bwd(q, k, v, out, dout, lse, dtype, dqkv, delta_scratch, nullptr, B, H, N, head_dim, head_dim_pad, ld_qkv,
+  CKV(attn_bwd(q, k, v, out, dout, lse, dtype, dqkv, delta_scratch, nullptr, 0, B, H, N, head_dim, head_dim_pad, ld_qkv,
                (hipStream_t)stream));
   return SGL_OK;
+}
+
+int sgl_op_attn_bwd_qsum(int dtype, const void* q, const void* k, const void* v, const void* out, const void* dout,
+                         const float* lse, void* dqkv, float* delta_scratch, int B, int H, int N, int head_dim,
+                         int head_dim_pad, int ld_qkv, float* qsum, int qsum_ld, sgl_stream stream) {
+  if (!qsum) return SGL_ERR_NULL;
+  if (B < 0 || H < 0 || N < 0 || head_dim <= 0 || qsum_ld < H * head_dim) return SGL_ERR_BAD_SHAPE;
+  CKV(attn_bwd(q, k, v, out, dout, lse, dtype, dqkv, delta_scratch, qsum, qsum_ld, B, H, N, head_dim, head_dim_pad,
+               ld_qkv, (hipStream_t)stream));
+  return SGL_OK;
+}
+
+int sgl_op_fold_jobs(const sgl_fold_job* jobs, int njobs, sgl_stream stream) {
+  if (njobs < 0 || njobs > 4) return SGL_ERR_BAD_SHAPE;
+  if (njobs > 0 && !jobs) return SGL_ERR_NULL;
+  FoldJobs table;
+  for (int k = 0; k < njobs; ++k) {
+    const sgl_fold_job& u = jobs[k];
+    if (u.nout != 1 && u.nout != 3) return SGL_ERR_BAD_SHAPE;
+    if (u.partial && (u.nblk < 0 || u.n < 0 || u.stride < u.nout * u.n)) return SGL_ERR_BAD_SHAPE;
+    if (u.nzero < 0 || (u.nzero > 0 && !u.zero)) return SGL_ERR_BAD_SHAPE;
+    if ((u.prev || u.extra[0] || u.extra[1]) && !(u.partial && u.out[u.nout - 1])) return SGL_ERR_NULL;
+    FoldJob j;
+    j.partial = u.partial; j.nblk = u.nblk; j.stride = u.stride; j.n = u.n; j.nout = u.nout;
+    for (int i = 0; i < 3; ++i) { j.out[i] = i < u.nout ? u.out[i] : nullptr; j.acc[i] = u.acc[i]; }
+    j.prev = u.prev; j.prev_acc = u.prev_acc;
+    for (int i = 0; i < 2; ++i) { j.extra[i] = u.extra[i]; j.extra_acc[i] = u.extra_acc[i]; }
+    j.zero = u.zero; j.nzero = u.nzero;
+    if (!fold_jobs_add(table, j)) return SGL_ERR_BAD_SHAPE;
+  }
+  CKV(fold_jobs_run(table, (hipStream_t)stream));
+  return SGL_OK;
+}
+
+void sgl_debug_qsum_counts(unsigned long long* fused, unsigned long long* fallback) {
+  if (fused) *fused = g_qsum_fused.load(std::memory_order_relaxed);
+  if (fallback) *fallback = g_qsum_fallback.load(std::memory_order_relaxed);
 }
 
 int sgl_op_colsum(int dtype, const void* in, int ld, int M, int N, float* out, int accumulate, float* scratch,
diff --git a/deepfake-detection-using-clip-based-siglip-2-vision-transformers_amd/csrc/epilogue.hip.h b/deepfake-detection-using-clip-based-siglip-2-vision-transformers_amd/csrc/epilogue.hip.h
--- a/deepfake-detection-using-clip-based-siglip-2-vision-transformers_amd/csrc/epilogue.hip.h
+++ b/deepfake-detection-using-clip-based-siglip-2-vision-transformers_amd/csrc/epilogue.hip.h
@@ -64,11 +64,12 @@
   asm volatile("" ::: "memory");
 }
 
-template <int NT, int BN, int NV>
-__device__ __forceinline__ void epi_colsum_fold(float* ct, const float (&csum)[NV], int t, int m0, int n0, int N,
+template <int NT, int BM, int BN, int NV>
+__device__ __forceinline__ void epi_colsum_fold(float* ct, const float (&csum)[NV], int t, int m0, int n0, int M, int N,
                                                 const EpiParams& p) {
   constexpr int CPR = BN / NV, GROUPS = NT / CPR;
   static_assert(NT % CPR == 0 && BN <= NT, "one fixed column set per thread, one thread per column");
+  static_assert(BM == 128 || BM == 256, "one or two 128-row blocks per tile");
   if (!p.colsum) return;
   lds_barrier();
 #pragma unroll
@@ -78,9 +79,10 @@
     float s = 0.f;
 #pragma unroll
     for (int gI = 0; gI < GROUPS; ++gI) s += ct[gI * BN + t];
-    if (p.colsum_ld > 0)
+    if (p.colsum_ld > 0) {
       p.colsum[(size_t)(m0 >> 7) * p.colsum_ld + n0 + t] = s;
-    else
+      if (BM == 256 && m0 + 128 < M) p.colsum[(size_t)((m0 >> 7) + 1) * p.colsum_ld + n0 + t] = 0.f;
+    } else
       atomicAdd(p.colsum + n0 + t, s);
   }
 }
diff --git a/deepfake-detection-using-clip-based-siglip-2-vision-transformers_amd/csrc/gemm_bf16.hip b/deepfake-detection-using-clip-based-siglip-2-vision-transformers_amd/csrc/gemm_bf16.hip
--- a/deepfake-detection-using-clip-based-siglip-2-vision-transformers_amd/csrc/gemm_bf16.hip
+++ b/deepfake-detection-using-clip-based-siglip-2-vision-transformers_amd/csrc/gemm_bf16.hip
@@ -67,7 +67,7 @@
       }
     }
   }
-  if constexpr (EPI == EPI_GELU_BWD) epi_colsum_fold<256, G_BN, NV>(ct, csum, t, m0, n0, N, p);
+  if constexpr (EPI == EPI_GELU_BWD) epi_colsum_fold<256, G_BM, G_BN, NV>(ct, csum, t, m0, n0, M, N, p);
 }
 
 template <int EPI, typename TOut, typename TIn>
diff --git a/deepfake-detection-using-clip-based-siglip-2-vision-transformers_amd/csrc/gemm_bf16_v2.hip b/deepfake-detection-using-clip-based-siglip-2-vision-transformers_amd/csrc/gemm_bf16_v2.hip
--- a/deepfake-detection-using-clip-based-siglip-2-vision-transformers_amd/csrc/gemm_bf16_v2.hip
+++ b/deepfake-detection-using-clip-based-siglip-2-vision-transformers_amd/csrc/gemm_bf16_v2.hip
@@ -185,7 +185,7 @@
   }
   if constexpr (EPI == EPI_GELU_BWD) {
     static_assert(P == 1, "the bias-gradient fold needs one column set per thread");
-    epi_colsum_fold<512, G::BN, NV>(ct, csum, t, m0, n0, N, p);
+    epi_colsum_fold<512, G::BM, G::BN, NV>(ct, csum, t, m0, n0, M, N, p);
   }
 }
 
diff --git a/deepfake-detection-using-clip-based-siglip-2-vision-transformers_amd/csrc/kernels.h b/deepfake-detection-using-clip-based-siglip-2-vision-transformers_amd/csrc/kernels.h
--- a/deepfake-detection-using-clip-based-siglip-2-vision-transformers_amd/csrc/kernels.h
+++ b/deepfake-detection-using-clip-based-siglip-2-vision-transformers_amd/csrc/kernels.h
@@ -72,6 +72,24 @@
                            hipStream_t s);
 hipError_t reduce_partials3(const float* partial, int nblk, int stride, float* o0, float* o1, float* o2, int n, int a0,
                             int a1, int a2, hipStream_t s);
+struct FoldJob {
+  const float* partial = nullptr;
+  int nblk = 0, stride = 0, n = 0, nout = 1;
+  float* out[3] = {nullptr, nullptr, nullptr};
+  int acc[3] = {0, 0, 0};
+  float* prev = nullptr;
+  float* extra[2] = {nullptr, nullptr};
+  int prev_acc = 0, extra_acc[2] = {0, 0};
+  float* zero = nullptr;
+  int nzero = 0;
+  int block0 = 0, colblocks = 0;
+};
+struct FoldJobs {
+  FoldJob j[4];
+  int njobs = 0, nblocks = 0;
+};
+bool fold_jobs_add(FoldJobs& jobs, const FoldJob& job);
+hipError_t fold_jobs_run(const FoldJobs& jobs, hipStream_t s);
 
 hipError_t im2col(const float* pix, int channels_last, void* out, int out_dtype, int B, int H, int W, int P,
                   int Kp, hipStream_t s);
@@ -104,6 +122,8 @@
 hipError_t batch_sum(const float* in, int B, size_t n, float* out, int accumulate, hipStream_t s);
 hipError_t vecmat_f32(const float* v, const float* W, int rows, int cols, float* scratch, float* out, int accumulate,
                       hipStream_t s);
+constexpr int kVecmatChunks = 16;
+hipError_t vecmat_f32_chunks(const float* v, const float* W, int rows, int cols, float* scratch, hipStream_t s);
 hipError_t pos_resize(const float* table, int g0, float* out, int gh, int gw, int D, hipStream_t s);
 hipError_t pos_resize_bwd(const float* dout, int gh, int gw, float* dtable, int g0, int D, hipStream_t s);
 hipError_t copy_f32(const float* src, float* dst, size_t n, hipStream_t s);
@@ -185,7 +205,7 @@
 hipError_t attn_fwd(const void* q, const void* k, const void* v, int dtype, void* out, float* lse, int B, int H,
                     int N, int dh, int DP, int ld_qkv, hipStream_t s);
 hipError_t attn_bwd(const void* q, const void* k, const void* v, const void* out, const void* dout,
-                    const float* lse, int dtype, void* dqkv, float* delta, float* reserved, int B, int H, int N,
-                    int dh, int DP, int ld_qkv, hipStream_t s);
-
-}
+                    const float* lse, int dtype, void* dqkv, float* delta, float* qsum, int qsum_ld, int B, int H,
+                    int N, int dh, int DP, int ld_qkv, hipStream_t s);
+
+}
diff --git a/deepfake-detection-using-clip-based-siglip-2-vision-transformers_amd/csrc/layernorm.hip b/deepfake-detection-using-clip-based-siglip-2-vision-transformers_amd/csrc/layernorm.hip
--- a/deepfake-detection-using-clip-based-siglip-2-vision-transformers_amd/csrc/layernorm.hip
+++ b/deepfake-detection-using-clip-based-siglip-2-vision-transformers_amd/csrc/layernorm.hip
@@ -242,26 +242,46 @@
   return ln_bwd_launch<float>(dy, lddy, x, mean, rstd, gamma, dres, dx, dx_lp, lp_dtype, partial, nblk, M, D, s);
 }
 
+__device__ __forceinline__ float fold_rows_x2(const float* __restrict__ partial, int nblk, int stride, int j, int g) {
+  float s0 = 0.f, s1 = 0.f;
+  int b = g;
+#pragma unroll 8
+  for (; b + 8 < nblk; b += 16) {
+    s0 += partial[(size_t)b * stride + j];
+    s1 += partial[(size_t)(b + 8) * stride + j];
+  }
+  if (b < nblk) s0 += partial[(size_t)b * stride + j];
+  return s0 + s1;
+}
+__device__ __forceinline__ float fold_rows_x4(const float* __restrict__ partial, int nblk, int stride, int j, int g) {
+  float s0 = 0.f, s1 = 0.f, s2 = 0.f, s3 = 0.f;
+  int b = g;
+#pragma unroll 4
+  for (; b + 24 < nblk; b += 32) {
+    s0 += partial[(size_t)b * stride + j];
+    s1 += partial[(size_t)(b + 8) * stride + j];
+    s2 += partial[(size_t)(b + 16) * stride + j];
+    s3 += partial[(size_t)(b + 24) * stride + j];
+  }
+  for (; b < nblk; b += 8) s0 += partial[(size_t)b * stride + j];
+  return (s0 + s1) + (s2 + s3);
+}
+__device__ __forceinline__ float fold_groups(const float (*red)[33], int c) {
+  float r = 0.f;
+#pragma unroll
+  for (int k = 0; k < 8; ++k) r += red[k][c];
+  return r;
+}
+
 __global__ __launch_bounds__(256) void reduce_partials_kernel(const float* __restrict__ partial, int nblk, int stride,
                                                               float* __restrict__ out, int n, int accumulate) {
   __shared__ float red[8][33];
   const int c = threadIdx.x & 31, g = threadIdx.x >> 5;
   const int j = blockIdx.x * 32 + c;
-  float s0 = 0.f, s1 = 0.f;
-  if (j < n) {
-    int b = g;
-    for (; b + 8 < nblk; b += 16) {
-      s0 += partial[(size_t)b * stride + j];
-      s1 += partial[(size_t)(b + 8) * stride + j];
-    }
-    if (b < nblk) s0 += partial[(size_t)b * stride + j];
-  }
-  red[g][c] = s0 + s1;
+  red[g][c] = (j < n) ? fold_rows_x2(partial, nblk, stride, j, g) : 0.f;
   __syncthreads();
   if (g == 0 && j < n) {
-    float r = 0.f;
-#pragma unroll
-    for (int k = 0; k < 8; ++k) r += red[k][c];
+    const float r = fold_groups(red, c);
     out[j] = accumulate ? out[j] + r : r;
   }
 }
@@ -276,25 +296,83 @@
   float* o = which == 0 ? o0 : (which == 1 ? o1 : o2);
   const int acc = which == 0 ? a0 : (which == 1 ? a1 : a2);
   const bool live = (j < 3 * n) && o;
-  float s0 = 0.f, s1 = 0.f, s2 = 0.f, s3 = 0.f;
-  if (live) {
-    int b = g;
-    for (; b + 24 < nblk; b += 32) {
-      s0 += partial[(size_t)b * stride + j];
-      s1 += partial[(size_t)(b + 8) * stride + j];
-      s2 += partial[(size_t)(b + 16) * stride + j];
-      s3 += partial[(size_t)(b + 24) * stride + j];
-    }
-    for (; b < nblk; b += 8) s0 += partial[(size_t)b * stride + j];
-  }
-  red[g][c] = (s0 + s1) + (s2 + s3);
+  red[g][c] = live ? fold_rows_x4(partial, nblk, stride, j, g) : 0.f;
   __syncthreads();
   if (g == 0 && live) {
-    float r = 0.f;
-#pragma unroll
-    for (int k = 0; k < 8; ++k) r += red[k][c];
+    const float r = fold_groups(red, c);
     o[jj] = acc ? o[jj] + r : r;
   }
+}
+
+__global__ __launch_bounds__(256) void fold_jobs_kernel(FoldJobs jobs) {
+  __shared__ float red[8][33];
+  int blk = blockIdx.x;
+  int ji = 0;
+#pragma unroll
+  for (int k = 1; k < 4; ++k) ji += (k < jobs.njobs && blk >= jobs.j[k].block0) ? 1 : 0;
+  const FoldJob& jb = jobs.j[ji];
+  blk -= jb.block0;
+  if (blk >= jb.colblocks) {
+    const int i = (blk - jb.colblocks) * 256 + (int)threadIdx.x;
+    if (i < jb.nzero) jb.zero[i] = 0.f;
+    return;
+  }
+  const int c = threadIdx.x & 31, g = threadIdx.x >> 5;
+  const int j = blk * 32 + c;
+  const int n = jb.n, nout = jb.nout;
+  const int which = (nout == 1) ? 0 : j / n, jj = j - which * n;
+  float* o = which == 0 ? jb.out[0] : (which == 1 ? jb.out[1] : jb.out[2]);
+  const int acc = which == 0 ? jb.acc[0] : (which == 1 ? jb.acc[1] : jb.acc[2]);
+  const bool live = (j < nout * n) && o;
+  float s = 0.f;
+  if (live) s = (nout == 1) ? fold_rows_x2(jb.partial, jb.nblk, jb.stride, j, g) : fold_rows_x4(jb.partial, jb.nblk, jb.stride, j, g);
+  red[g][c] = s;
+  __syncthreads();
+  if (g == 0 && live) {
+    const float r = fold_groups(red, c);
+    const bool last = which == nout - 1;
+    if (last && jb.prev) {
+      const float old = 0.f + o[jj];
+      jb.prev[jj] = jb.prev_acc ? jb.prev[jj] + old : old;
+    }
+    const float v = acc ? o[jj] + r : r;
+    o[jj] = v;
+    if (last) {
+#pragma unroll
+      for (int e = 0; e < 2; ++e)
+        if (jb.extra[e]) {
+          const float x = 0.f + v;
+          jb.extra[e][jj] = jb.extra_acc[e] ? jb.extra[e][jj] + x : x;
+        }
+    }
+  }
+}
+
+bool fold_jobs_add(FoldJobs& jobs, const FoldJob& job) {
+  FoldJob jb = job;
+  bool live = false;
+  for (int k = 0; k < jb.nout; ++k) live = live || jb.out[k];
+  if (!jb.partial || jb.n <= 0 || !live) {
+    jb.partial = nullptr;
+    live = false;
+  }
+  if (!jb.zero || jb.nzero <= 0) {
+    jb.zero = nullptr;
+    jb.nzero = 0;
+  }
+  if (!live && !jb.zero) return true;
+  if (jobs.njobs >= 4) return false;
+  jb.colblocks = live ? (jb.nout * jb.n + 31) / 32 : 0;
+  jb.block0 = jobs.nblocks;
+  jobs.nblocks += jb.colblocks + (jb.nzero + 255) / 256;
+  jobs.j[jobs.njobs++] = jb;
+  return true;
+}
+
+hipError_t fold_jobs_run(const FoldJobs& jobs, hipStream_t s) {
+  if (jobs.nblocks == 0) return hipSuccess;
+  hipLaunchKernelGGL(fold_jobs_kernel, dim3((unsigned)jobs.nblocks), dim3(256), 0, s, jobs);
+  return hipGetLastError();
 }
 
 hipError_t reduce_partials3(const float* partial, int nblk, int stride, float* o0, float* o1, float* o2, int n, int a0,
diff --git a/deepfake-detection-using-clip-based-siglip-2-vision-transformers_amd/lib.py b/deepfake-detection-using-clip-based-siglip-2-vision-transformers_amd/lib.py
--- a/deepfake-detection-using-clip-based-siglip-2-vision-transformers_amd/lib.py
+++ b/deepfake-detection-using-clip-based-siglip-2-vision-transformers_amd/lib.py
@@ -64,6 +64,12 @@
 
 class SglCastVec(C.Structure):
     _fields_ = [("src", _fp), ("dst", _fp), ("n", C.c_int), ("np", C.c_int)]
+
+
+class SglFoldJob(C.Structure):
+    _fields_ = [("partial", _fp), ("nblk", C.c_int), ("stride", C.c_int), ("n", C.c_int), ("nout", C.c_int),
+                ("out", _fp * 3), ("acc", C.c_int * 3), ("prev", _fp), ("extra", _fp * 2), ("prev_acc", C.c_int),
+                ("extra_acc", C.c_int * 2), ("zero", _fp), ("nzero", C.c_int)]
 
 
 class SglView(C.Structure):
@@ -142,6 +148,9 @@
     _sig(lib, "sgl_op_gemm_tn_ws", i, [i, _fp, i, _fp, i, i, i, i, i, _fp, i, i, _fp, sz, _fp])
     _sig(lib, "sgl_op_attn_fwd", i, [i, _fp, _fp, _fp, _fp, _fp, i, i, i, i, i, i, _fp])
     _sig(lib, "sgl_op_attn_bwd", i, [i, _fp, _fp, _fp, _fp, _fp, _fp, _fp, _fp, i, i, i, i, i, i, _fp])
+    _sig(lib, "sgl_op_attn_bwd_qsum", i, [i, _fp, _fp, _fp, _fp, _fp, _fp, _fp, _fp, i, i, i, i, i, i, _fp, i, _fp])
+    _sig(lib, "sgl_debug_qsum_counts", None, [C.POINTER(C.c_ulonglong), C.POINTER(C.c_ulonglong)])
+    _sig(lib, "sgl_op_fold_jobs", i, [C.POINTER(SglFoldJob), i, _fp])
     _sig(lib, "sgl_op_colsum", i, [i, _fp, i, i, i, _fp, i, _fp, sz, _fp])
     _sig(lib, "sgl_op_im2col", i, [_fp, i, _fp, i, i, i, i, i, i, _fp])
     _sig(lib, "sgl_op_col2im", i, [_fp, i, i, i, i, i, _fp, i, _fp])
diff --git a/include/siglip_hip.h b/include/siglip_hip.h
--- a/include/siglip_hip.h
+++ b/include/siglip_hip.h
@@ -150,6 +150,10 @@
 int sgl_op_attn_bwd(int dtype, const void* q, const void* k, const void* v, const void* out, const void* dout,
                     const float* lse, void* dqkv, float* delta_scratch, int B, int H, int N, int head_dim,
                     int head_dim_pad, int ld_qkv, sgl_stream stream);
+int sgl_op_attn_bwd_qsum(int dtype, const void* q, const void* k, const void* v, const void* out, const void* dout,
+                         const float* lse, void* dqkv, float* delta_scratch, int B, int H, int N, int head_dim,
+                         int head_dim_pad, int ld_qkv, float* qsum, int qsum_ld, sgl_stream stream);
+void sgl_debug_qsum_counts(unsigned long long* fused, unsigned long long* fallback);
 int sgl_op_colsum(int dtype, const void* in, int ld, int M, int N, float* out, int accumulate, float* scratch,
                   size_t scratch_bytes, sgl_stream stream);
 int sgl_op_im2col(const float* pixels, int channels_last, void* out, int out_dtype, int B, int H, int W, int P, int Kp,
@@ -187,6 +191,18 @@
                            sgl_stream stream);
 int sgl_op_reduce_partials3(const float* partial, int nblk, int stride, float* out0, float* out1, float* out2, int n,
                             int accumulate0, int accumulate1, int accumulate2, sgl_stream stream);
+typedef struct {
+  const float* partial;
+  int nblk, stride, n, nout;
+  float* out[3];
+  int acc[3];
+  float* prev;
+  float* extra[2];
+  int prev_acc, extra_acc[2];
+  float* zero;
+  int nzero;
+} sgl_fold_job;
+int sgl_op_fold_jobs(const sgl_fold_job* jobs, int njobs, sgl_stream stream);
 int sgl_op_reduce_splits(const float* ws, int splits, size_t stride, int N1, int N2, float* out, int ldo, int accumulate,
                          sgl_stream stream);
 int sgl_op_add_f32(const float* a, const float* b, float* out, size_t n, sgl_stream stream);
```
